# zdebruine/MMVAE

Measured on AMD Instinct MI355X. Metric: cells/sec per MMVAE train step, higher is better.
Workload: dtype f32; 1 GPU; c2: 2-modality MMVAE train step, 20000 genes each, latent 128, K=1, batch 512/GPU, adversarial=False; global_batch=512, parallelism=dp1, exchange=none

## Files before the change

include/mmvae_hip.h:

```cpp
#ifndef MMVAE_HIP_H
#define MMVAE_HIP_H

#include <stddef.h>
#include <stdint.h>

#ifdef __cplusplus
extern "C" {
#endif

typedef void* mmvae_stream_t;

#define MMVAE_OK 0
#define MMVAE_ERR_ARG 1
#define MMVAE_ERR_LAUNCH 2
#define MMVAE_ERR_WORKSPACE 3

#define MMVAE_ABI_VERSION 16
int mmvae_abi_version(void);
const char* mmvae_build_arch(void);

#define MMVAE_GEMM_NT 0
#define MMVAE_GEMM_NN 1
#define MMVAE_GEMM_TN 2

#define MMVAE_GEMM_RELU 1u
#define MMVAE_GEMM_ACCUMULATE 2u
#define MMVAE_GEMM_RAW_SLABS 4u
#define MMVAE_GEMM_OPERAND_SLACK 8u

#define MMVAE_GEMM_PRECISION_F32 0
#define MMVAE_GEMM_PRECISION_BF16X3 1
int mmvae_gemm_set_precision(int mode);
int mmvae_gemm_set_workgroup_cap(int max_workgroups);
int mmvae_gemm_set_x3w(int mode);
int mmvae_gemm_get_x3w(void);
int mmvae_gemm_get_precision(void);

int mmvae_gemm_plan(int layout, int M, int N, int K, int* tile_out, int* splitk_out);
size_t mmvae_gemm_workspace_bytes(int layout, int M, int N, int K, int splitk);

int mmvae_gemm_f32(int layout, int M, int N, int K, float alpha, const float* A, int64_t lda, const float* B,
                   int64_t ldb, float* C, int64_t ldc, const float* bias, unsigned flags, int splitk,
                   float* workspace, size_t workspace_bytes, mmvae_stream_t stream);

typedef struct mmvae_planes {
    uint16_t* p;
    int64_t ld, plane_stride;
} mmvae_planes;
#define MMVAE_RECON_H_KPAD 1u
typedef struct mmvae_recon_args {
    int32_t rows, x_rows, G, H;
    uint32_t flags, reserved;
    const float *h, *W, *bias, *x;
    int64_t ldh, ldw, ldx;
    float *xhat, *dP, *se_part, *col_part;
    int64_t ldxhat, lddp;
    mmvae_planes h_planes, W_planes, dP_planes;
} mmvae_recon_args;
int mmvae_recon_tiles(int G);
int mmvae_recon_row_tiles(int rows);
int mmvae_decoder_recon(const mmvae_recon_args* args, mmvae_stream_t stream);
size_t mmvae_sizeof_planes(void);
size_t mmvae_sizeof_recon_args(void);
size_t mmvae_sizeof_split_job(void);

typedef struct mmvae_bn_params {
    const float* gamma;
    const float* beta;
    float* running_mean;
    float* running_var;
    int64_t* num_batches_tracked;
    float momentum;
    float eps;
} mmvae_bn_params;

size_t mmvae_fc_workspace_bytes(int B, int N);

typedef struct mmvae_split_job {
    int32_t rows, cols;
    const float* src;
    int64_t ld_src;
    mmvae_planes planes;
} mmvae_split_job;

int mmvae_fc_epilogue_fwd(int B, int N, const float* in, int64_t ld_in, int n_slabs, const float* bias,
                          const mmvae_bn_params* bn , int training, int relu,
                          const uint8_t* keep_mask , float dropout_p, float* z_out,
                          float* a_out, float* d_out, int64_t ld_out, float* save_mean, float* save_invstd,
                          float* workspace, size_t workspace_bytes, const mmvae_planes* d_planes ,
                          const mmvae_split_job* split , mmvae_stream_t stream);

int mmvae_fc_epilogue_bwd(int B, int N, const float* din, int64_t ld_in, int n_slabs, const float* addend,
                          const float* addend_a, const float* row_scale, const uint8_t* keep_mask, float dropout_p, int relu,
                          const float* a, const float* z, const float* gamma, const float* save_mean,
                          const float* save_invstd, int has_bn, float* dz_out, int64_t ld_out, float* dbias,
                          float* dgamma, float* dbeta, float* workspace, size_t workspace_bytes,
                          const mmvae_planes* dz_planes , mmvae_stream_t stream);

int mmvae_layernorm_fwd(int B, int N, const float* x, int64_t ldx, float eps, float* y, int64_t ldy, float* save_mean,
                        float* save_invstd, mmvae_stream_t stream);
int mmvae_layernorm_bwd(int B, int N, const float* dy, int64_t lddy, const float* y, int64_t ldy,
                        const float* save_invstd, float* dx, int64_t lddx, mmvae_stream_t stream);

int mmvae_fc_rowtail_fwd(int B, int N, const float* in, int64_t ld_in, int n_slabs, const float* bias ,
                         float eps, int training, int relu, const uint8_t* keep_mask , float dropout_p,
                         float* y_out, float* a_out, float* d_out, int64_t ld_out, float* save_invstd,
                         mmvae_stream_t stream);

int mmvae_fc_rowtail_bwd(int B, int N, const float* din, int64_t ld_in, int n_slabs, const float* addend,
                         const float* row_scale, const uint8_t* keep_mask, float dropout_p, int relu, const float* act,
                         const float* y, const float* save_invstd, float* dz_out, int64_t ld_out, float* dbias,
                         float* workspace, size_t workspace_bytes, mmvae_stream_t stream);

int mmvae_reparam_kl_fwd(int B, int Z, int K, const float* mu, const float* a_raw, const float* eps, float var_eps,
                         float* std_out, float* z_out, float* kl_row, float* stat_row, mmvae_stream_t stream);

int mmvae_reparam_kl_bwd(int B, int Z, int K, const float* mu, const float* std, const float* eps, const float* dz,
                         const float* dmu_extra, const float* dstd_extra, const float* dkl_row,
                         const float* kl_scale_dev, float kl_scale_host, float var_eps, float* dmu, float* da_raw,
                         mmvae_stream_t stream);

int mmvae_mse_sum_fwd_bwd(int B, int G, const float* xhat, int64_t ldxhat, const float* x, int64_t ldx, float* se_row,
                          float* dxhat, int64_t lddx, const float* gscale_dev, float gscale_host,
                          mmvae_stream_t stream);

int mmvae_elbo_finalize(int B, int K, int T, const float* se_part, const float* kl_row, const float* stat_row, int Z,
                        const float* kl_weight_dev, float kl_weight_host, float* out6, float* w_out,
                        float* recon_row , mmvae_stream_t stream);

int mmvae_iwae_logratio(int B, int Z, int K, const float* std, const float* eps, const float* z, float* out,
                        mmvae_stream_t stream);
int mmvae_elbo_finalize_iwae(int B, int K, int T, const float* se_part, const float* logratio, const float* stat_row,
                             int Z, const float* kl_weight_dev, float kl_weight_host, float* out6, float* w_out,
                             float* rows3, mmvae_stream_t stream);
int mmvae_iwae_bwd_terms(int B, int Z, int K, const float* kl_weight_dev, float kl_weight_host, const float* w,
                         const float* z, const float* std, float* dz, float* dstd_extra, mmvae_stream_t stream);

int mmvae_cross_entropy_sum(int B, int C, const float* logits, int64_t ld, const int64_t* labels, float* loss_rows,
                            float* dlogits, int64_t ldd, const float* gscale_dev, float gscale_host,
                            mmvae_stream_t stream);
int mmvae_cross_entropy_heads(int B, int H, int max_classes, const int32_t* col_dev, const int32_t* classes_dev,
                              const float* logits, int64_t ld, const int64_t* labels, float* loss_rows, float* dlogits,
                              int64_t ldd, float gscale, mmvae_stream_t stream);
int mmvae_sum_f32(int64_t n, const float* v, float* out, int accumulate, mmvae_stream_t stream);
int mmvae_sum_rows_f32(int H, int64_t n, const float* v, int64_t ld, float* out_each, float* out_total,
                       mmvae_stream_t stream);

#define MMVAE_ADAM_STATE_FLOATS 8
#define MMVAE_PREPARE_NORM 1u
#define MMVAE_PREPARE_ADVANCE 2u
int64_t mmvae_sqnorm_partials(int64_t n);
int mmvae_grad_sqnorm(int64_t n, const float* grad, float* partials, mmvae_stream_t stream);
int mmvae_adam_prepare(int64_t n_partials, const float* partials, float max_norm, float grad_scale, float beta1,
                       float beta2, float* state, unsigned flags, mmvae_stream_t stream);
int mmvae_adam_set_workgroups(int workgroups);
int mmvae_adam_get_workgroups(void);
int mmvae_grad_sqnorm_ranges_prepare(int n_ranges, const float* const* grads, const int64_t* lens, float* partials,
                                     unsigned* ticket, int64_t n_partials_all, const float* partials_all, float max_norm,
                                     float grad_scale, float beta1, float beta2, float* state, unsigned flags,
                                     mmvae_stream_t stream);
#define MMVAE_ADAM_HYPER_FLOATS 4
int mmvae_adam_step_hp(int64_t n, float* param, const float* grad, float* exp_avg, float* exp_avg_sq, const float* state,
                       const float* hyper, float beta1, float beta2, float eps, float grad_scale, mmvae_stream_t stream);
int mmvae_adam_step_copy_hp(int64_t n, float* param, const float* grad, float* exp_avg, float* exp_avg_sq,
                            const float* state, const float* hyper, float beta1, float beta2, float eps, float grad_scale,
                            int copy_n, const float* copy_src, float* copy_dst, mmvae_stream_t stream);

#define MMVAE_ADAM_JOB_ELEMS 16384
typedef struct {
    int64_t offset;
    int32_t len;
    float bc1, bc2;
    int32_t reserved;
} mmvae_adam_job;
int mmvae_adam_step_jobs_hp(int n_jobs, const mmvae_adam_job* jobs_dev, float* param, const float* grad, float* exp_avg,
                            float* exp_avg_sq, const float* state, const float* hyper, float beta1, float beta2, float eps,
                            float grad_scale, mmvae_stream_t stream);
int mmvae_grad_sqnorm_jobs(int n_jobs, const mmvae_adam_job* jobs_dev, const float* grad, float* partials,
                           mmvae_stream_t stream);
int mmvae_grad_zero_flagged_jobs(int n_jobs, const mmvae_adam_job* jobs_dev, float* grad, mmvae_stream_t stream);
int mmvae_jobs_pack(int n_jobs, const mmvae_adam_job* jobs_dev, const float* arena, float* staging, mmvae_stream_t stream);
int mmvae_jobs_unpack(int n_jobs, const mmvae_adam_job* jobs_dev, float* arena, const float* staging, mmvae_stream_t stream);

int mmvae_philox_keep_mask(int64_t n, float p_drop, uint8_t* mask, uint64_t* rng_state, uint64_t stream_id,
                           int advance, mmvae_stream_t stream);
int mmvae_philox_normal(int64_t n, float* out, uint64_t* rng_state, uint64_t stream_id, int advance,
                        mmvae_stream_t stream);
typedef struct {
    void* out;
    int64_t n;
    uint64_t stream_id;
    float p_drop;
    int32_t kind;
} mmvae_philox_job;
int mmvae_philox_fill_jobs(int n_jobs, const mmvae_philox_job* jobs_dev, int64_t max_n, uint64_t* rng_state,
                           mmvae_stream_t stream);
int mmvae_philox_fill_jobs_advance(int n_jobs, const mmvae_philox_job* jobs_dev, int64_t max_n, uint64_t* rng_state,
                                   uint64_t advance_by, unsigned* ticket, mmvae_stream_t stream);
int mmvae_philox_advance(uint64_t* rng_state, uint64_t by, mmvae_stream_t stream);

typedef struct {
    const float* src;
    float* dst;
    int64_t part_stride, ld_src, ld_dst;
    int32_t n_parts, rows, cols;
    float alpha;
    uint32_t flags;
    uint32_t reserved;
} mmvae_sum_job;
int mmvae_sum_parts_batch(int n_jobs, const mmvae_sum_job* jobs, int64_t max_elems , mmvae_stream_t stream);

int mmvae_gemm_sq_partials(int layout, int M, int N, int K, int operands_regular);

int mmvae_split_planes_f32(int rows, int cols, const float* src, int64_t ld_src, uint16_t* planes,
                           int64_t ld, int64_t plane_stride, mmvae_stream_t stream);
int mmvae_gemm_planes_f32(int layout, int M, int N, int K, float alpha, const float* A, int64_t lda, const uint16_t* Ap,
                          int64_t ldap, int64_t a_plane_stride, const float* B, int64_t ldb, const uint16_t* Bp,
                          int64_t ldbp, int64_t b_plane_stride, float* C, int64_t ldc, const float* bias, unsigned flags,
                          int splitk, float* workspace, size_t workspace_bytes, float* sq_partials, int64_t sq_capacity,
                          mmvae_stream_t stream);
int mmvae_gemm_planes_supported(int layout, int M, int N, int K, int splitk, int a_planes, int b_planes);
typedef struct {
    const float* A;
    const float* B;
    float* C;
    const float* bias;
    int64_t lda, ldb, ldc;
    int32_t layout, M, N, K;
    float alpha;
    uint32_t flags;
    int32_t first_block;
    int32_t n_blocks;
} mmvae_gemm_job;
int mmvae_gemm_batch_job_ok(const mmvae_gemm_job* job);
int mmvae_gemm_batch_prepare(int n_jobs, mmvae_gemm_job* jobs, int* total_blocks);
int mmvae_gemm_batch_f32(int n_jobs, const mmvae_gemm_job* jobs_dev, int total_blocks, mmvae_stream_t stream);

int mmvae_csr_to_dense_f32(int B, int G, int64_t nnz, const int64_t* crow_indices, const int64_t* col_indices,
                           const float* values, float* out, int64_t ldo, mmvae_stream_t stream);
int mmvae_csr_to_dense_i32_f32(int B, int G, int64_t nnz, const int32_t* crow_indices, const int32_t* col_indices,
                               const float* values, float* out, int64_t ldo, mmvae_stream_t stream);

int mmvae_csr_gather_rows_i64(int B, int64_t n_src_rows, int64_t src_nnz, const int64_t* src_crow, const int64_t* src_col,
                              const float* src_val, const int64_t* rows, const int64_t* out_crow, int64_t out_nnz,
                              int64_t* out_col, float* out_val, mmvae_stream_t stream);
int mmvae_csr_gather_rows_i32(int B, int64_t n_src_rows, int64_t src_nnz, const int32_t* src_crow, const int32_t* src_col,
                              const float* src_val, const int64_t* rows, const int32_t* out_crow, int64_t out_nnz,
                              int32_t* out_col, float* out_val, mmvae_stream_t stream);
int mmvae_csr_gather_rows_dense_i64(int B, int G, int64_t n_src_rows, int64_t src_nnz, const int64_t* src_crow,
                                    const int64_t* src_col, const float* src_val, const int64_t* rows, float* out,
                                    int64_t ldo, mmvae_stream_t stream);
int mmvae_csr_gather_rows_dense_i32(int B, int G, int64_t n_src_rows, int64_t src_nnz, const int32_t* src_crow,
                                    const int32_t* src_col, const float* src_val, const int64_t* rows, float* out,
                                    int64_t ldo, mmvae_stream_t stream);

int mmvae_csr_spmm_wt_i32_f32(int B, int N, int G, int64_t nnz, const int32_t* crow_indices, const int32_t* col_indices,
                              const float* values, const float* Wt, int64_t ldwt, const float* bias, float* y,
                              int64_t ldy, mmvae_stream_t stream);

#define MMVAE_COND_DW_CHUNK 32
int mmvae_cond_linear_fwd(int B, int n_in, int n_out, const float* x, int64_t ldx, const float* params,
                          const int64_t* w_off, const int64_t* b_off, const int32_t* cond, const int32_t* rows, float* y,
                          int64_t ldy, mmvae_stream_t stream);
int mmvae_cond_linear_bwd_dx(int B, int n_in, int n_out, const float* dy, int64_t lddy, const float* params,
                             const int64_t* w_off, const int32_t* cond, const int32_t* rows, float* dx, int64_t lddx,
                             int accumulate, mmvae_stream_t stream);
int mmvae_cond_linear_bwd_dw(int n_chunks, const int32_t* chunk_dst, const int32_t* chunk_beg, const int32_t* chunk_end,
                             const int32_t* rows, int n_in, int n_out, const float* dy, int64_t lddy, const float* x,
                             int64_t ldx, float* grads, const int64_t* w_off, const int64_t* b_off, int n_red,
                             const int32_t* red_cond, const int32_t* red_slot, const int32_t* red_n, float* partials,
                             mmvae_stream_t stream);
int mmvae_cond_linear_fwd_multi(int n_pos, int B, int n_in, int n_out, const float* x, int64_t ldx, int64_t x_pos_stride,
                                const float* params, const int64_t* w_off, const int64_t* b_off, const int32_t* cond,
// ... 110 lines not shown
```

mmvae_amd/_lib.py:

```python
from __future__ import annotations

import ctypes as C
import os
from typing import Optional

_HERE = os.path.dirname(os.path.abspath(__file__))
LIB_PATH = os.path.join(_HERE, "csrc", "libmmvae_hip.so")
if os.environ.get("MMVAE_LIB"):
    LIB_PATH = os.environ["MMVAE_LIB"]

OK, ERR_ARG, ERR_LAUNCH, ERR_WORKSPACE = 0, 1, 2, 3
_ERR_NAMES = {1: "MMVAE_ERR_ARG", 2: "MMVAE_ERR_LAUNCH", 3: "MMVAE_ERR_WORKSPACE"}

GEMM_NT, GEMM_NN, GEMM_TN = 0, 1, 2
GEMM_RELU, GEMM_ACCUMULATE, GEMM_RAW_SLABS, GEMM_OPERAND_SLACK = 1, 2, 4, 8
GEMM_PRECISION_F32, GEMM_PRECISION_BF16X3 = 0, 1
ADAM_STATE_FLOATS = 8
ADAM_HYPER_FLOATS = 4
PREPARE_NORM, PREPARE_ADVANCE = 1, 2

_p = C.c_void_p
_i = C.c_int
_l = C.c_int64
_f = C.c_float
_u = C.c_uint
_z = C.c_size_t
_u64 = C.c_uint64


class BnParams(C.Structure):

    _fields_ = [
        ("gamma", _p),
        ("beta", _p),
        ("running_mean", _p),
        ("running_var", _p),
        ("num_batches_tracked", _p),
        ("momentum", _f),
        ("eps", _f),
    ]


class Planes(C.Structure):
    _fields_ = [("p", _p), ("ld", _l), ("plane_stride", _l)]


class ReconArgs(C.Structure):
    _fields_ = [("rows", C.c_int32), ("x_rows", C.c_int32), ("G", C.c_int32), ("H", C.c_int32), ("flags", C.c_uint32),
                ("reserved", C.c_uint32), ("h", _p), ("W", _p), ("bias", _p), ("x", _p), ("ldh", _l), ("ldw", _l),
                ("ldx", _l), ("xhat", _p), ("dP", _p), ("se_part", _p), ("col_part", _p), ("ldxhat", _l), ("lddp", _l),
                ("h_planes", Planes), ("W_planes", Planes), ("dP_planes", Planes)]


class SplitJob(C.Structure):
    _fields_ = [("rows", C.c_int32), ("cols", C.c_int32), ("src", _p), ("ld_src", _l), ("planes", Planes)]


RECON_H_KPAD = 1


PROTOTYPES = {
    "mmvae_abi_version": (_i, []),
    "mmvae_build_arch": (C.c_char_p, []),
    "mmvae_gemm_set_precision": (_i, [_i]),
    "mmvae_gemm_set_workgroup_cap": (_i, [_i]),
    "mmvae_adam_set_workgroups": (_i, [_i]),
    "mmvae_adam_get_workgroups": (_i, []),
    "mmvae_gemm_set_x3w": (_i, [_i]),
    "mmvae_gemm_get_x3w": (_i, []),
    "mmvae_gemm_get_precision": (_i, []),
    "mmvae_gemm_plan": (_i, [_i, _i, _i, _i, C.POINTER(_i), C.POINTER(_i)]),
    "mmvae_gemm_workspace_bytes": (_z, [_i, _i, _i, _i, _i]),
    "mmvae_gemm_f32": (_i, [_i, _i, _i, _i, _f, _p, _l, _p, _l, _p, _l, _p, _u, _i, _p, _z, _p]),
    "mmvae_recon_tiles": (_i, [_i]),
    "mmvae_recon_row_tiles": (_i, [_i]),
    "mmvae_decoder_recon": (_i, [C.POINTER(ReconArgs), _p]),
    "mmvae_sizeof_planes": (_z, []),
    "mmvae_sizeof_recon_args": (_z, []),
    "mmvae_sizeof_split_job": (_z, []),
    "mmvae_fc_workspace_bytes": (_z, [_i, _i]),
    "mmvae_fc_epilogue_fwd": (
        _i,
        [_i, _i, _p, _l, _i, _p, C.POINTER(BnParams), _i, _i, _p, _f, _p, _p, _p, _l, _p, _p, _p, _z,
         C.POINTER(Planes), C.POINTER(SplitJob), _p],
    ),
    "mmvae_fc_epilogue_bwd": (
        _i,
        [_i, _i, _p, _l, _i, _p, _p, _p, _p, _f, _i, _p, _p, _p, _p, _p, _i, _p, _l, _p, _p, _p, _p, _z,
         C.POINTER(Planes), _p],
    ),
    "mmvae_layernorm_fwd": (_i, [_i, _i, _p, _l, _f, _p, _l, _p, _p, _p]),
    "mmvae_layernorm_bwd": (_i, [_i, _i, _p, _l, _p, _l, _p, _p, _l, _p]),
    "mmvae_fc_rowtail_fwd": (_i, [_i, _i, _p, _l, _i, _p, _f, _i, _i, _p, _f, _p, _p, _p, _l, _p, _p]),
    "mmvae_fc_rowtail_bwd": (_i, [_i, _i, _p, _l, _i, _p, _p, _p, _f, _i, _p, _p, _p, _p, _l, _p, _p, _z, _p]),
    "mmvae_reparam_kl_fwd": (_i, [_i, _i, _i, _p, _p, _p, _f, _p, _p, _p, _p, _p]),
    "mmvae_reparam_kl_bwd": (_i, [_i, _i, _i, _p, _p, _p, _p, _p, _p, _p, _p, _f, _f, _p, _p, _p]),
    "mmvae_mse_sum_fwd_bwd": (_i, [_i, _i, _p, _l, _p, _l, _p, _p, _l, _p, _f, _p]),
    "mmvae_elbo_finalize": (_i, [_i, _i, _i, _p, _p, _p, _i, _p, _f, _p, _p, _p, _p]),
    "mmvae_iwae_logratio": (_i, [_i, _i, _i, _p, _p, _p, _p, _p]),
    "mmvae_elbo_finalize_iwae": (_i, [_i, _i, _i, _p, _p, _p, _i, _p, _f, _p, _p, _p, _p]),
    "mmvae_iwae_bwd_terms": (_i, [_i, _i, _i, _p, _f, _p, _p, _p, _p, _p, _p]),
    "mmvae_cross_entropy_sum": (_i, [_i, _i, _p, _l, _p, _p, _p, _l, _p, _f, _p]),
    "mmvae_cross_entropy_heads": (_i, [_i, _i, _i, _p, _p, _p, _l, _p, _p, _p, _l, _f, _p]),
    "mmvae_sum_f32": (_i, [_l, _p, _p, _i, _p]),
    "mmvae_debug_occupy": (_i, [_i, _i, _i, _p, _p]),
    "mmvae_sum_rows_f32": (_i, [_i, _l, _p, _l, _p, _p, _p]),
    "mmvae_sqnorm_partials": (_l, [_l]),
    "mmvae_grad_sqnorm": (_i, [_l, _p, _p, _p]),
    "mmvae_adam_prepare": (_i, [_l, _p, _f, _f, _f, _f, _p, _u, _p]),
    "mmvae_grad_sqnorm_ranges_prepare": (_i, [_i, _p, _p, _p, _p, _l, _p, _f, _f, _f, _f, _p, _u, _p]),
    "mmvae_adam_step_hp": (_i, [_l, _p, _p, _p, _p, _p, _p, _f, _f, _f, _f, _p]),
    "mmvae_adam_step_copy_hp": (_i, [_l, _p, _p, _p, _p, _p, _p, _f, _f, _f, _f, _i, _p, _p, _p]),
    "mmvae_adam_step_jobs_hp": (_i, [_i, _p, _p, _p, _p, _p, _p, _p, _f, _f, _f, _f, _p]),
    "mmvae_grad_sqnorm_jobs": (_i, [_i, _p, _p, _p, _p]),
    "mmvae_grad_zero_flagged_jobs": (_i, [_i, _p, _p, _p]),
    "mmvae_jobs_pack": (_i, [_i, _p, _p, _p, _p]),
    "mmvae_jobs_unpack": (_i, [_i, _p, _p, _p, _p]),
    "mmvae_philox_keep_mask": (_i, [_l, _f, _p, _p, _u64, _i, _p]),
    "mmvae_philox_normal": (_i, [_l, _p, _p, _u64, _i, _p]),
    "mmvae_philox_advance": (_i, [_p, _u64, _p]),
    "mmvae_philox_fill_jobs": (_i, [_i, _p, _l, _p, _p]),
    "mmvae_philox_fill_jobs_advance": (_i, [_i, _p, _l, _p, C.c_uint64, _p, _p]),
    "mmvae_axpby": (_i, [_l, _f, _p, _f, _p, _p]),
    "mmvae_upload_words": (_i, [_l, _p, _p, _p]),
    "mmvae_scale_rows": (_i, [_i, _i, _p, _l, _p, _p, _l, _p]),
    "mmvae_debug_stamp": (_i, [_p, _i, _p]),
    "mmvae_weighted_colsum_chunks": (_i, [_i]),
    "mmvae_weighted_colsum_f32": (_i, [_i, _i, _p, _l, _p, _p, _p]),
    "mmvae_sum_parts_batch": (_i, [_i, _p, _l, _p]),
    "mmvae_gemm_sq_partials": (_i, [_i, _i, _i, _i, _i]),
    "mmvae_split_planes_f32": (_i, [_i, _i, _p, _l, _p, _l, _l, _p]),
    "mmvae_gemm_planes_f32": (
        _i,
        [_i, _i, _i, _i, _f, _p, _l, _p, _l, _l, _p, _l, _p, _l, _l, _p, _l, _p, _u, _i, _p, _z, _p, _l, _p],
    ),
    "mmvae_gemm_planes_supported": (_i, [_i, _i, _i, _i, _i, _i, _i]),
    "mmvae_csr_to_dense_f32": (_i, [_i, _i, _l, _p, _p, _p, _p, _l, _p]),
    "mmvae_csr_to_dense_i32_f32": (_i, [_i, _i, _l, _p, _p, _p, _p, _l, _p]),
    "mmvae_csr_gather_rows_i64": (_i, [_i, _l, _l, _p, _p, _p, _p, _p, _l, _p, _p, _p]),
    "mmvae_csr_gather_rows_i32": (_i, [_i, _l, _l, _p, _p, _p, _p, _p, _l, _p, _p, _p]),
    "mmvae_csr_gather_rows_dense_i64": (_i, [_i, _i, _l, _l, _p, _p, _p, _p, _p, _l, _p]),
    "mmvae_csr_gather_rows_dense_i32": (_i, [_i, _i, _l, _l, _p, _p, _p, _p, _p, _l, _p]),
    "mmvae_csr_spmm_wt_i32_f32": (_i, [_i, _i, _i, _l, _p, _p, _p, _p, _l, _p, _p, _l, _p]),
    "mmvae_cond_linear_fwd": (_i, [_i, _i, _i, _p, _l, _p, _p, _p, _p, _p, _p, _l, _p]),
    "mmvae_cond_linear_bwd_dx": (_i, [_i, _i, _i, _p, _l, _p, _p, _p, _p, _p, _l, _i, _p]),
    "mmvae_cond_linear_bwd_dw": (_i, [_i, _p, _p, _p, _p, _i, _i, _p, _l, _p, _l, _p, _p, _p, _i, _p, _p, _p, _p, _p]),
    "mmvae_cond_linear_fwd_multi": (_i, [_i, _i, _i, _i, _p, _l, _l, _p, _p, _p, _p, _p, _l, _p, _l, _l, _p]),
    "mmvae_cond_linear_bwd_dx_multi": (_i, [_i, _i, _i, _i, _p, _l, _l, _p, _p, _p, _l, _p, _l, _i, _p]),
    "mmvae_cond_linear_bwd_dw_multi": (_i, [_i, _i, _p, _p, _p, _p, _l, _i, _i, _p, _l, _l, _p, _l, _l, _p, _p, _p, _i, _p,
                                            _p, _p, _p, _l, _p]),
    "mmvae_gemm_batch_job_ok": (_i, [_p]),
    "mmvae_gemm_batch_prepare": (_i, [_i, _p, C.POINTER(_i)]),
    "mmvae_gemm_batch_f32": (_i, [_i, _p, _i, _p]),
    "mmvae_adv_pass_plan": (_i, [_p, _i, C.POINTER(_i), C.POINTER(_z), C.POINTER(_l), C.POINTER(_i)]),
    "mmvae_adv_pass_f32": (_i, [_i, _p, _i, _i, _i, _i, _z, _p]),
    "mmvae_adv_dw_prepare": (_i, [_i, _p, C.POINTER(_i), C.POINTER(_i)]),
    "mmvae_adv_dw_f32": (_i, [_i, _p, _i, _i, _p, _p, _p, _i, _p, _i, _p]),
    "mmvae_adam_step_multi_hp": (_i, [_i, _p, _l, _p]),
    "mmvae_ell_from_dense_f32": (_i, [_i, _i, _p, _l, _i, _p, _p, _p, _p]),
    "mmvae_dw_sparse_ell_f32": (_i, [_i, _i, _i, _p, _l, _p, _p, _p, _i, _p, _l, _p]),
    "mmvae_col_pearson_workspace_bytes": (_z, [_i, _i]),
    "mmvae_col_pearson_f32": (_i, [_i, _i, _p, _l, _p, _l, _p, _p, _z, _p]),
}


class SumJob(C.Structure):
    _fields_ = [("src", C.c_void_p), ("dst", C.c_void_p), ("part_stride", C.c_int64), ("ld_src", C.c_int64),
                ("ld_dst", C.c_int64), ("n_parts", C.c_int32), ("rows", C.c_int32), ("cols", C.c_int32),
                ("alpha", C.c_float), ("flags", C.c_uint32), ("reserved", C.c_uint32)]


class PhiloxJob(C.Structure):
    _fields_ = [("out", C.c_void_p), ("n", C.c_int64), ("stream_id", C.c_uint64), ("p_drop", C.c_float),
                ("kind", C.c_int32)]


class GemmJob(C.Structure):
    _fields_ = [("A", C.c_void_p), ("B", C.c_void_p), ("C", C.c_void_p), ("bias", C.c_void_p), ("lda", C.c_int64),
                ("ldb", C.c_int64), ("ldc", C.c_int64), ("layout", C.c_int32), ("M", C.c_int32), ("N", C.c_int32),
                ("K", C.c_int32), ("alpha", C.c_float), ("flags", C.c_uint32), ("first_block", C.c_int32),
                ("n_blocks", C.c_int32)]


ADV_MAX_LAYERS, ADV_MAX_HEADS = 4, 8


class AdvJob(C.Structure):
    _fields_ = [("x", _p), ("ldx", _l), ("W", _p * ADV_MAX_LAYERS), ("b", _p * ADV_MAX_LAYERS),
                ("mask", _p * ADV_MAX_LAYERS), ("act", _p * ADV_MAX_LAYERS), ("dz", _p * ADV_MAX_LAYERS), ("Wh", _p),
                ("bh", _p), ("labels", _p), ("logits", _p), ("lse", _p), ("loss_rows", _p), ("gx", _p), ("partials", _p),
                ("loss_each", _p), ("loss_total", _p), ("total_loss", _p), ("total_scale", _f),
                ("gscale", _f), ("p_drop", _f * ADV_MAX_LAYERS), ("relu", C.c_int32 * ADV_MAX_LAYERS),
                ("width", C.c_int32 * (ADV_MAX_LAYERS + 1)), ("n_layers", C.c_int32), ("H", C.c_int32),
                ("Ct", C.c_int32), ("B", C.c_int32), ("col", C.c_int32 * ADV_MAX_HEADS),
                ("classes", C.c_int32 * ADV_MAX_HEADS), ("seg_lo", (C.c_int16 * ADV_MAX_HEADS) * 8),
                ("seg_hi", (C.c_int16 * ADV_MAX_HEADS) * 8)]


class AdvDwJob(C.Structure):
    _fields_ = [("dz", _p), ("ld_dz", _l), ("inp", _p), ("ld_inp", _l), ("gW", _p), ("gb", _p), ("lse", _p),
                ("labels", _p), ("gscale", _f), ("M", C.c_int32), ("N", C.c_int32), ("B", C.c_int32), ("H", C.c_int32),
                ("opt", C.c_int32), ("col", C.c_int32 * ADV_MAX_HEADS), ("classes", C.c_int32 * ADV_MAX_HEADS),
                ("first_block", C.c_int32), ("n_blocks", C.c_int32)]


class AdvOpt(C.Structure):
    _fields_ = [("state", _p), ("norm_out", _p), ("max_norm", _f), ("grad_scale", _f), ("beta1", _f), ("beta2", _f),
                ("flags", C.c_uint32), ("reserved", C.c_uint32)]


class AdamArenaHp(C.Structure):
    _fields_ = [("p", _p), ("g", _p), ("m", _p), ("v", _p), ("state", _p), ("hyper", _p), ("n", _l), ("beta1", _f),
                ("beta2", _f), ("eps", _f), ("grad_scale", _f)]


class HipLibraryError(RuntimeError):
    pass


_lib: Optional[C.CDLL] = None


def load() -> C.CDLL:
    global _lib
    if _lib is not None:
        return _lib
    import torch

    if not os.path.exists(LIB_PATH):
        raise HipLibraryError(
            f"{LIB_PATH} not found: build it with `make -C mmvae_amd/csrc` (or __graft_entry__.build()). "
            "mmvae_amd has no non-HIP execution path for device tensors."
        )
    try:
        lib = C.CDLL(LIB_PATH)
    except OSError as e:
        raise HipLibraryError(f"could not load {LIB_PATH}: {e}") from e
    for name, (res, args) in PROTOTYPES.items():
        try:
            fn = getattr(lib, name)
        except AttributeError as e:
            raise HipLibraryError(f"{LIB_PATH} does not export {name}") from e
        fn.restype = res
        fn.argtypes = args
    _lib = lib
    return lib


def check(rc: int, what: str) -> None:
# ... 3 lines not shown
```

mmvae_amd/csrc/elbo_optim.hip:

```cpp
#include "common.h"

namespace {

__global__ __launch_bounds__(256) void reparam_kl_fwd_kernel(int B, int Z, int K, const float* __restrict__ mu,
                                                             const float* __restrict__ a_raw,
                                                             const float* __restrict__ eps, float var_eps,
                                                             float* __restrict__ std_out, float* __restrict__ z_out,
                                                             float* __restrict__ kl_row, float* __restrict__ stat_row) {
    const int lane = threadIdx.x & 63;
    const int b = blockIdx.x * 4 + (threadIdx.x >> 6);
    if (b >= B) return;
    float kl = 0.f, smu = 0.f, svar = 0.f;
    for (int j = lane; j < Z; j += 64) {
        const int64_t o = (int64_t)b * Z + j;
        const float m = mu[o];
        const float v = expf(a_raw[o]) + var_eps;
        const float s = sqrtf(v);
        if (std_out) std_out[o] = s;
        const float vr = s * s;
        kl += 0.5f * (vr + m * m - 1.f - logf(vr));
        smu += m;
        svar += vr;
        if (z_out)
            for (int k = 0; k < K; ++k) {
                const int64_t ok = ((int64_t)k * B + b) * Z + j;
                z_out[ok] = m + s * eps[ok];
            }
    }
    kl = wave_sum(kl);
    smu = wave_sum(smu);
    svar = wave_sum(svar);
    if (lane == 0) {
        if (kl_row) kl_row[b] = kl;
        if (stat_row) {
            stat_row[b] = smu;
            stat_row[B + b] = svar;
        }
    }
}

__global__ __launch_bounds__(256) void reparam_kl_bwd_kernel(int B, int Z, int K, const float* __restrict__ mu,
                                                             const float* __restrict__ sd,
                                                             const float* __restrict__ eps, const float* __restrict__ dz,
                                                             const float* __restrict__ dmu_extra,
                                                             const float* __restrict__ dstd_extra,
                                                             const float* __restrict__ dkl_row,
                                                             const float* __restrict__ kl_scale_dev, float kl_scale_host,
                                                             float var_eps, float* __restrict__ dmu,
                                                             float* __restrict__ da_raw) {
    const int64_t n = (int64_t)B * Z;
    const float cs = (kl_scale_dev ? *kl_scale_dev : 1.f) * kl_scale_host;
    for (int64_t o = (int64_t)blockIdx.x * blockDim.x + threadIdx.x; o < n; o += (int64_t)gridDim.x * blockDim.x) {
        const int b = (int)(o / Z);
        const float c = cs * (dkl_row ? dkl_row[b] : 1.f);
        const float m = mu[o], s = sd[o];
        const float v = s * s;
        float gm = dmu_extra ? dmu_extra[o] : 0.f;
        float gs = dstd_extra ? dstd_extra[o] : 0.f;
        if (dz)
            for (int k = 0; k < K; ++k) {
                const int64_t ok = (int64_t)k * n + o;
                const float g = dz[ok];
                gm += g;
                gs += g * eps[ok];
            }
        dmu[o] = gm + c * m;
        da_raw[o] = (gs / (2.f * s) + c * 0.5f * (1.f - 1.f / v)) * (v - var_eps);
    }
}

__global__ __launch_bounds__(256) void mse_rows_kernel(int B, int G, const float* __restrict__ xhat, int64_t ldxhat,
                                                       const float* __restrict__ x, int64_t ldx,
                                                       float* __restrict__ se_row, float* __restrict__ dxhat,
                                                       int64_t lddx, const float* __restrict__ gscale_dev,
                                                       float gscale_host) {
    __shared__ float red[4];
    const int b = blockIdx.x;
    const float gs = 2.f * gscale_host * (gscale_dev ? *gscale_dev : 1.f);
    const float* xh = xhat + (int64_t)b * ldxhat;
    const float* xr = x + (int64_t)b * ldx;
    float* dr = dxhat ? dxhat + (int64_t)b * lddx : nullptr;
    float s = 0.f;
    for (int j = threadIdx.x; j < G; j += 256) {
        const float d = xh[j] - xr[j];
        s += d * d;
        if (dr) dr[j] = gs * d;
    }
    s = wave_sum(s);
    if ((threadIdx.x & 63) == 0) red[threadIdx.x >> 6] = s;
    __syncthreads();
    if (threadIdx.x == 0 && se_row) se_row[b] = (red[0] + red[1]) + (red[2] + red[3]);
}

constexpr int ELBO_MAXK = 64;
__global__ __launch_bounds__(256) void elbo_rows_kernel(int B, int K, int T, const float* __restrict__ se_part,
                                                        float* __restrict__ recon_row, float* __restrict__ w_out) {
    __shared__ float se_s[4][ELBO_MAXK];
    const int lane = threadIdx.x & 63, wv = threadIdx.x >> 6;
    const int b = blockIdx.x * 4 + wv;
    if (b >= B) return;
    const int64_t KB = (int64_t)K * B;
    if (K == 1) {
        float s = 0.f;
        for (int t = lane; t < T; t += 64) s += se_part[(int64_t)t * KB + b];
        s = wave_sum(s);
        if (lane == 0) {
            recon_row[b] = s;
            if (w_out) w_out[b] = 1.f;
        }
        return;
    }
    for (int k = 0; k < K; ++k) {
        float s = 0.f;
        for (int t = lane; t < T; t += 64) s += se_part[(int64_t)t * KB + (int64_t)k * B + b];
        s = wave_sum(s);
        if (lane == 0) se_s[wv][k] = s;
    }
    __builtin_amdgcn_wave_barrier();
    float v = (lane < K) ? -se_s[wv][lane] : -INFINITY;
    const float mx = wave_max(v);
    const float ex = (lane < K) ? expf(v - mx) : 0.f;
    const float sum = wave_sum(ex);
    const float lse = mx + logf(sum);
    if (lane == 0) recon_row[b] = -(lse - logf((float)K));
    if (w_out && lane < K) w_out[(int64_t)lane * B + b] = ex / sum;
}

__global__ __launch_bounds__(256) void iwae_logratio_kernel(int B, int Z, int K, const float* __restrict__ std,
                                                            const float* __restrict__ eps, const float* __restrict__ z,
                                                            float* __restrict__ out) {
    const int lane = threadIdx.x & 63, row = blockIdx.x * 4 + (threadIdx.x >> 6);
    if (row >= K * B) return;
    const int b = row % B;
    const float* sr = std + (int64_t)b * Z;
    const float* er = eps + (int64_t)row * Z;
    const float* zr = z + (int64_t)row * Z;
    float s = 0.f;
    for (int j = lane; j < Z; j += 64) s += -logf(sr[j]) - 0.5f * er[j] * er[j] + 0.5f * zr[j] * zr[j];
    s = wave_sum(s);
    if (lane == 0) out[row] = s;
}

__global__ __launch_bounds__(256) void elbo_rows_iwae_kernel(int B, int K, int T, const float* __restrict__ se_part,
                                                             const float* __restrict__ logratio,
                                                             const float* __restrict__ klw_dev, float c_host,
                                                             float* __restrict__ rows3, float* __restrict__ w_out) {
    __shared__ float se_s[4][ELBO_MAXK];
    const int lane = threadIdx.x & 63, wv = threadIdx.x >> 6;
    const int b = blockIdx.x * 4 + wv;
    if (b >= B) return;
    const int64_t KB = (int64_t)K * B;
    const float c = (klw_dev ? *klw_dev : 1.f) * c_host;
    for (int k = 0; k < K; ++k) {
        float s = 0.f;
        for (int t = lane; t < T; t += 64) s += se_part[(int64_t)t * KB + (int64_t)k * B + b];
        s = wave_sum(s);
        if (lane == 0) se_s[wv][k] = s;
    }
    __builtin_amdgcn_wave_barrier();
    const float se = (lane < K) ? se_s[wv][lane] : 0.f;
    const float r = (lane < K) ? logratio[(int64_t)lane * B + b] : 0.f;
    const float v = (lane < K) ? -se - c * r : -INFINITY;
    const float mx = wave_max(v);
    const float ex = (lane < K) ? expf(v - mx) : 0.f;
    const float sum = wave_sum(ex);
    const float lse = mx + logf(sum);
    const float w = ex / sum;
    const float wse = wave_sum(w * se), wr = wave_sum(w * r);
    if (lane == 0) {
        rows3[b] = -(lse - logf((float)K));
        rows3[B + b] = wse;
        rows3[2 * (int64_t)B + b] = wr;
    }
    if (w_out && lane < K) w_out[(int64_t)lane * B + b] = w;
}

__global__ __launch_bounds__(256) void elbo_reduce_iwae_kernel(int B, const float* __restrict__ rows3,
                                                               const float* __restrict__ stat_row, int Z,
                                                               const float* __restrict__ klw_dev, float klw_host,
                                                               float* __restrict__ out6) {
    __shared__ double red[5][256];
    const int tid = threadIdx.x;
    double a0 = 0.0, a1 = 0.0, a2 = 0.0, smu = 0.0, svar = 0.0;
    for (int b = tid; b < B; b += 256) {
        a0 += (double)rows3[b];
        a1 += (double)rows3[B + b];
        a2 += (double)rows3[2 * (int64_t)B + b];
        if (stat_row) {
            smu += (double)stat_row[b];
            svar += (double)stat_row[B + b];
        }
    }
    red[0][tid] = a0;
    red[1][tid] = a1;
    red[2][tid] = a2;
    red[3][tid] = smu;
    red[4][tid] = svar;
    __syncthreads();
    if (tid == 0) {
        double t[5] = {0, 0, 0, 0, 0};
        for (int i = 0; i < 256; ++i)
            for (int q = 0; q < 5; ++q) t[q] += red[q][i];
// ... 426 lines not shown
                   nullptr, nullptr);
}

inline int grid_for(int64_t n, int per_block, int cap);
constexpr int STREAM_GRID_CAP = 1 << 22;
static int g_adam_workgroups = 0;

extern "C" int mmvae_adam_set_workgroups(int workgroups) {
    if (workgroups < 0 || workgroups > 256) return MMVAE_ERR_ARG;
    g_adam_workgroups = workgroups;
    return MMVAE_OK;
}

extern "C" int mmvae_adam_get_workgroups(void) { return g_adam_workgroups; }

static int launch_adam_step(int64_t n, float* param, const float* grad, float* exp_avg, float* exp_avg_sq,
                            const float* state, const float* hyper, float beta1, float beta2, float eps,
                            float grad_scale, int copy_n, const float* copy_src, float* copy_dst, hipStream_t stream) {
    const int vec = aligned16(param) && aligned16(grad) && aligned16(exp_avg) && aligned16(exp_avg_sq);
    if (g_adam_workgroups > 0) {
        static bool attr = false;
        if (!attr) {
            if (hipFuncSetAttribute(reinterpret_cast<const void*>(adam_step_wide_hp_kernel),
                                    hipFuncAttributeMaxDynamicSharedMemorySize, ADAM_WIDE_LDS) != hipSuccess)
                return MMVAE_ERR_LAUNCH;
            attr = true;
        }
        MMVAE_LAUNCH(adam_step_wide_hp_kernel, dim3(g_adam_workgroups), dim3(1024), (size_t)ADAM_WIDE_LDS, stream, n, param,
                     grad, exp_avg, exp_avg_sq, state, hyper, beta1, beta2, eps, grad_scale, vec, copy_n, copy_src,
                     copy_dst);
    } else {
        MMVAE_LAUNCH(adam_step_hp_kernel, dim3(grid_for(n, 1024, STREAM_GRID_CAP)), dim3(256), 0, stream, n, param, grad,
                     exp_avg, exp_avg_sq, state, hyper, beta1, beta2, eps, grad_scale, vec, copy_n, copy_src, copy_dst);
    }
    MMVAE_LAUNCH_CHECK();
    return MMVAE_OK;
}

__device__ __forceinline__ void adam_step_jobs_body(const mmvae_adam_job* __restrict__ jobs, float* __restrict__ p,
                                                    const float* __restrict__ g, float* __restrict__ m,
                                                    float* __restrict__ v, const float* __restrict__ state,
                                                    const float* __restrict__ hyper, float b1, float b2, float eps,
                                                    float grad_scale) {
    const mmvae_adam_job job = jobs[blockIdx.x];
    if ((job.reserved & 3) == 2) return;
    float lr, wd, decay;
    adam_hyper(hyper, lr, wd, decay);
    const float gmul = state[2] * grad_scale;
    const float step_size = lr / job.bc1;
    const float inv_bc2_sqrt = 1.f / sqrtf(job.bc2);
    const float cv = state[5];
    const int64_t o = job.offset;
    const int n = job.len;
    if ((o & 3) == 0) {
        const int nv = n >> 2;
        f32x4* pv = reinterpret_cast<f32x4*>(p + o);
        const f32x4* gv = reinterpret_cast<const f32x4*>(g + o);
        f32x4* mv = reinterpret_cast<f32x4*>(m + o);
        f32x4* vv = reinterpret_cast<f32x4*>(v + o);
        for (int i = threadIdx.x; i < nv; i += 256) {
            f32x4 pp = pv[i], gg = gv[i], mm = mv[i], vw = vv[i];
#pragma unroll
            for (int e = 0; e < 4; ++e) {
                float pe = pp[e], me = mm[e], ve = vw[e];
                adam_elem(pe, gg[e], me, ve, gmul, wd, decay, b1, b2, step_size, inv_bc2_sqrt, eps, cv);
                pp[e] = pe;
                mm[e] = me;
                vw[e] = ve;
            }
            pv[i] = pp;
            mv[i] = mm;
            vv[i] = vw;
        }
        for (int i = 4 * nv + threadIdx.x; i < n; i += 256)
            adam_elem(p[o + i], g[o + i], m[o + i], v[o + i], gmul, wd, decay, b1, b2, step_size, inv_bc2_sqrt, eps, cv);
    } else {
        for (int i = threadIdx.x; i < n; i += 256)
            adam_elem(p[o + i], g[o + i], m[o + i], v[o + i], gmul, wd, decay, b1, b2, step_size, inv_bc2_sqrt, eps, cv);
    }
}

__global__ __launch_bounds__(256) void adam_step_jobs_hp_kernel(const mmvae_adam_job* __restrict__ jobs,
                                                                float* __restrict__ p, const float* __restrict__ g,
                                                                float* __restrict__ m, float* __restrict__ v,
                                                                const float* __restrict__ state,
                                                                const float* __restrict__ hyper, float b1, float b2,
                                                                float eps, float grad_scale) {
    adam_step_jobs_body(jobs, p, g, m, v, state, hyper, b1, b2, eps, grad_scale);
}

__global__ __launch_bounds__(256) void sqnorm_jobs_kernel(const mmvae_adam_job* __restrict__ jobs,
                                                          const float* __restrict__ g, float* __restrict__ partials) {
    __shared__ float red[4];
    const mmvae_adam_job job = jobs[blockIdx.x];
    const int64_t o = job.offset;
    const int n = (job.reserved & 3) == 2 ? 0 : job.len;
    float s = 0.f;
    if ((o & 3) == 0) {
        const int nv = n >> 2;
        const f32x4* gv = reinterpret_cast<const f32x4*>(g + o);
        float s0 = 0.f, s1 = 0.f, s2 = 0.f, s3 = 0.f;
        for (int i = threadIdx.x; i < nv; i += 256) {
            const f32x4 v = gv[i];
            s0 += v.x * v.x;
            s1 += v.y * v.y;
            s2 += v.z * v.z;
            s3 += v.w * v.w;
        }
        s = (s0 + s1) + (s2 + s3);
        for (int i = 4 * nv + threadIdx.x; i < n; i += 256) s += g[o + i] * g[o + i];
    } else {
        for (int i = threadIdx.x; i < n; i += 256) s += g[o + i] * g[o + i];
    }
    s = wave_sum(s);
    if ((threadIdx.x & 63) == 0) red[threadIdx.x >> 6] = s;
    __syncthreads();
    if (threadIdx.x == 0) partials[blockIdx.x] = (red[0] + red[1]) + (red[2] + red[3]);
}

__global__ __launch_bounds__(256) void zero_flagged_jobs_kernel(const mmvae_adam_job* __restrict__ jobs,
                                                                float* __restrict__ g) {
    const mmvae_adam_job job = jobs[blockIdx.x];
    if ((job.reserved & 3) != 1 && (job.reserved & 3) != 2) return;
    for (int i = threadIdx.x; i < job.len; i += 256) g[job.offset + i] = 0.f;
}

template <bool PACK>
__global__ __launch_bounds__(256) void jobs_pack_kernel(const mmvae_adam_job* __restrict__ jobs, float* __restrict__ arena,
                                                        float* __restrict__ staging) {
    const mmvae_adam_job job = jobs[blockIdx.x];
    float* a = arena + job.offset;
    float* s = staging + (int64_t)((unsigned)job.reserved >> 2) * 128;
    const int n = job.len, padded = (n + 127) & ~127;
    for (int i = threadIdx.x; i < n; i += 256) {
        if (PACK)
            s[i] = a[i];
        else
            a[i] = s[i];
    }
    if (PACK)
        for (int i = n + threadIdx.x; i < padded; i += 256) s[i] = 0.f;
}

__global__ __launch_bounds__(256) void occupy_kernel(long long ticks, float* __restrict__ sink) {
    extern __shared__ float hold[];
    hold[threadIdx.x] = (float)threadIdx.x;
    __syncthreads();
    const long long t0 = wall_clock64();
    float acc = hold[(threadIdx.x + 1) & 255];
    while (wall_clock64() - t0 < ticks) acc = acc * 1.0000001f + 1e-7f;
    if (acc == -1.f && sink) sink[0] = acc;
}

struct u32x4 {
    uint32_t x, y, z, w;
};
__device__ __forceinline__ u32x4 philox4x32_10(uint64_t counter, uint64_t stream_id, uint64_t seed) {
    uint32_t c0 = (uint32_t)counter, c1 = (uint32_t)(counter >> 32), c2 = (uint32_t)stream_id,
             c3 = (uint32_t)(stream_id >> 32);
    uint32_t k0 = (uint32_t)seed, k1 = (uint32_t)(seed >> 32);
#pragma unroll
    for (int i = 0; i < 10; ++i) {
        const uint64_t p0 = (uint64_t)0xD2511F53u * c0;
        const uint64_t p1 = (uint64_t)0xCD9E8D57u * c2;
        const uint32_t n0 = (uint32_t)(p1 >> 32) ^ c1 ^ k0;
        const uint32_t n1 = (uint32_t)p1;
        const uint32_t n2 = (uint32_t)(p0 >> 32) ^ c3 ^ k1;
        const uint32_t n3 = (uint32_t)p0;
        c0 = n0;
        c1 = n1;
        c2 = n2;
        c3 = n3;
        k0 += 0x9E3779B9u;
        k1 += 0xBB67AE85u;
    }
    return {c0, c1, c2, c3};
}
__device__ __forceinline__ float u01(uint32_t x) { return ((float)(x >> 8) + 0.5f) * (1.0f / 16777216.0f); }

__global__ __launch_bounds__(256) void philox_mask_kernel(int64_t n, float p_drop, uint8_t* __restrict__ mask,
                                                          const uint64_t* __restrict__ rng, uint64_t stream_id) {
    const uint64_t seed = rng[0], off = rng[1];
    const int64_t nq = (n + 3) / 4;
    for (int64_t q = (int64_t)blockIdx.x * blockDim.x + threadIdx.x; q < nq; q += (int64_t)gridDim.x * blockDim.x) {
        const u32x4 r = philox4x32_10(off + (uint64_t)q, stream_id, seed);
        const uint32_t rv[4] = {r.x, r.y, r.z, r.w};
#pragma unroll
        for (int j = 0; j < 4; ++j) {
            const int64_t i = q * 4 + j;
            if (i < n) mask[i] = (u01(rv[j]) >= p_drop) ? 1 : 0;
        }
    }
}

__global__ __launch_bounds__(256) void philox_normal_kernel(int64_t n, float* __restrict__ out,
                                                            const uint64_t* __restrict__ rng, uint64_t stream_id) {
    const uint64_t seed = rng[0], off = rng[1];
    const int64_t nq = (n + 3) / 4;
    for (int64_t q = (int64_t)blockIdx.x * blockDim.x + threadIdx.x; q < nq; q += (int64_t)gridDim.x * blockDim.x) {
        const u32x4 r = philox4x32_10(off + (uint64_t)q, stream_id, seed);
        const float u0 = u01(r.x), u1 = u01(r.y), u2 = u01(r.z), u3 = u01(r.w);
        const float r0 = sqrtf(-2.f * logf(u0)), r1 = sqrtf(-2.f * logf(u2));
        float s0, c0, s1, c1;
        sincosf(6.283185307179586f * u1, &s0, &c0);
        sincosf(6.283185307179586f * u3, &s1, &c1);
        const float nv[4] = {r0 * c0, r0 * s0, r1 * c1, r1 * s1};
#pragma unroll
        for (int j = 0; j < 4; ++j) {
            const int64_t i = q * 4 + j;
            if (i < n) out[i] = nv[j];
        }
    }
}

__global__ void philox_advance_kernel(uint64_t* rng, uint64_t by) { rng[1] += by; }

__global__ __launch_bounds__(256) void philox_fill_jobs_kernel(const mmvae_philox_job* __restrict__ jobs, uint64_t* rng,
                                                               uint64_t advance_by, unsigned* ticket) {
    const mmvae_philox_job job = jobs[blockIdx.y];
    const uint64_t seed = rng[0], off = rng[1];
    const int64_t n = job.n, nq = (n + 3) / 4;
    for (int64_t q = (int64_t)blockIdx.x * blockDim.x + threadIdx.x; q < nq; q += (int64_t)gridDim.x * blockDim.x) {
        const u32x4 r = philox4x32_10(off + (uint64_t)q, job.stream_id, seed);
        if (job.kind == 0) {
            uint8_t* mask = static_cast<uint8_t*>(job.out);
            const uint32_t rv[4] = {r.x, r.y, r.z, r.w};
#pragma unroll
            for (int j = 0; j < 4; ++j) {
                const int64_t i = q * 4 + j;
                if (i < n) mask[i] = (u01(rv[j]) >= job.p_drop) ? 1 : 0;
            }
        } else {
            float* out = static_cast<float*>(job.out);
            const float u0 = u01(r.x), u1 = u01(r.y), u2 = u01(r.z), u3 = u01(r.w);
            const float r0 = sqrtf(-2.f * logf(u0)), r1 = sqrtf(-2.f * logf(u2));
            float s0, c0, s1, c1;
            sincosf(6.283185307179586f * u1, &s0, &c0);
            sincosf(6.283185307179586f * u3, &s1, &c1);
            const float nv[4] = {r0 * c0, r0 * s0, r1 * c1, r1 * s1};
#pragma unroll
            for (int j = 0; j < 4; ++j) {
                const int64_t i = q * 4 + j;
                if (i < n) out[i] = nv[j];
            }
        }
    }
    if (advance_by && ticket) {
        __syncthreads();
        if (threadIdx.x == 0 && atomicAdd(ticket, 1u) == gridDim.x * gridDim.y - 1) {
            *ticket = 0u;
            rng[1] = off + advance_by;
        }
    }
}

__global__ __launch_bounds__(256) void axpby_kernel(int64_t n, float alpha, const float* __restrict__ x, float beta,
                                                    float* __restrict__ y) {
    for (int64_t i = (int64_t)blockIdx.x * blockDim.x + threadIdx.x; i < n; i += (int64_t)gridDim.x * blockDim.x)
        y[i] = alpha * x[i] + (beta != 0.f ? beta * y[i] : 0.f);
}

__global__ __launch_bounds__(256) void axpby4_kernel(int64_t n4, float alpha, const float4* __restrict__ x, float beta,
                                                     float4* __restrict__ y) {
    for (int64_t i = (int64_t)blockIdx.x * blockDim.x + threadIdx.x; i < n4; i += (int64_t)gridDim.x * blockDim.x) {
        const float4 a = x[i];
        float4 r = make_float4(alpha * a.x, alpha * a.y, alpha * a.z, alpha * a.w);
        if (beta != 0.f) {
            const float4 b = y[i];
            r.x += beta * b.x, r.y += beta * b.y, r.z += beta * b.z, r.w += beta * b.w;
        }
        y[i] = r;
    }
}

__global__ __launch_bounds__(256) void sum_parts_batch_kernel(const mmvae_sum_job* __restrict__ jobs) {
    const mmvae_sum_job j = jobs[blockIdx.y];
    const bool acc = j.flags & MMVAE_GEMM_ACCUMULATE;
    const bool vec = j.cols % 4 == 0;
    if (vec) {
        const int c4n = j.cols / 4;
        const int64_t total = (int64_t)j.rows * c4n;
        for (int64_t i = (int64_t)blockIdx.x * blockDim.x + threadIdx.x; i < total; i += (int64_t)gridDim.x * blockDim.x) {
            const int r = (int)(i / c4n), c = (int)(i - (int64_t)r * c4n) * 4;
            const float* sp = j.src + (int64_t)r * j.ld_src + c;
            f32x4 s = {0.f, 0.f, 0.f, 0.f};
            int p = 0;
            for (; p + 8 <= j.n_parts; p += 8) {
                f32x4 t[8];
#pragma unroll
                for (int u = 0; u < 8; ++u) t[u] = *reinterpret_cast<const f32x4*>(sp + (int64_t)(p + u) * j.part_stride);
#pragma unroll
                for (int u = 0; u < 8; ++u) s += t[u];
            }
            for (; p < j.n_parts; ++p) s += *reinterpret_cast<const f32x4*>(sp + (int64_t)p * j.part_stride);
            f32x4 v = s * j.alpha;
            float* dp = j.dst + (int64_t)r * j.ld_dst + c;
            if (acc) v += *reinterpret_cast<const f32x4*>(dp);
            *reinterpret_cast<f32x4*>(dp) = v;
        }
    } else {
        const int64_t total = (int64_t)j.rows * j.cols;
        for (int64_t i = (int64_t)blockIdx.x * blockDim.x + threadIdx.x; i < total; i += (int64_t)gridDim.x * blockDim.x) {
            const int r = (int)(i / j.cols), c = (int)(i - (int64_t)r * j.cols);
            const float* sp = j.src + (int64_t)r * j.ld_src + c;
            float s = 0.f;
            for (int p = 0; p < j.n_parts; ++p) s += sp[(int64_t)p * j.part_stride];
            float v = s * j.alpha;
            float* dp = j.dst + (int64_t)r * j.ld_dst + c;
            if (acc) v += *dp;
            *dp = v;
        }
    }
}

__global__ __launch_bounds__(256) void scale_rows_kernel(int B, int N, const float* __restrict__ x, int64_t ldx,
                                                         const float* __restrict__ rs, float* __restrict__ y,
                                                         int64_t ldy) {
    const int64_t total = (int64_t)B * N;
    for (int64_t i = (int64_t)blockIdx.x * blockDim.x + threadIdx.x; i < total; i += (int64_t)gridDim.x * blockDim.x) {
        const int b = (int)(i / N), j = (int)(i - (int64_t)b * N);
        y[(int64_t)b * ldy + j] = x[(int64_t)b * ldx + j] * rs[b];
    }
}

inline int grid_for(int64_t n, int per_block, int cap) {
    int64_t b = (n + per_block - 1) / per_block;
    if (b < 1) b = 1;
    if (b > cap) b = cap;
    return (int)b;
}

}

extern "C" int mmvae_abi_version(void) { return MMVAE_ABI_VERSION; }
extern "C" const char* mmvae_build_arch(void) { return "gfx950"; }

extern "C" int mmvae_reparam_kl_fwd(int B, int Z, int K, const float* mu, const float* a_raw, const float* eps,
                                    float var_eps, float* std_out, float* z_out, float* kl_row, float* stat_row,
                                    mmvae_stream_t stream) {
    if (B <= 0 || Z <= 0 || K < 1 || !mu || !a_raw) return MMVAE_ERR_ARG;
    if (z_out && !eps) return MMVAE_ERR_ARG;
    MMVAE_LAUNCH(reparam_kl_fwd_kernel, dim3(ceil_div_i(B, 4)), dim3(256), 0, (hipStream_t)stream, B, Z, K, mu,
                       a_raw, eps, var_eps, std_out, z_out, kl_row, stat_row);
    MMVAE_LAUNCH_CHECK();
    return MMVAE_OK;
}

extern "C" int mmvae_reparam_kl_bwd(int B, int Z, int K, const float* mu, const float* sd, const float* eps,
                                    const float* dz, const float* dmu_extra, const float* dstd_extra,
                                    const float* dkl_row, const float* kl_scale_dev, float kl_scale_host, float var_eps,
                                    float* dmu, float* da_raw, mmvae_stream_t stream) {
    if (B <= 0 || Z <= 0 || K < 1 || !mu || !sd || !dmu || !da_raw) return MMVAE_ERR_ARG;
    if (dz && !eps) return MMVAE_ERR_ARG;
    const int64_t n = (int64_t)B * Z;
    MMVAE_LAUNCH(reparam_kl_bwd_kernel, dim3(grid_for(n, 256, 2048)), dim3(256), 0, (hipStream_t)stream, B, Z, K,
                       mu, sd, eps, dz, dmu_extra, dstd_extra, dkl_row, kl_scale_dev, kl_scale_host, var_eps, dmu,
                       da_raw);
    MMVAE_LAUNCH_CHECK();
    return MMVAE_OK;
}

extern "C" int mmvae_mse_sum_fwd_bwd(int B, int G, const float* xhat, int64_t ldxhat, const float* x, int64_t ldx,
                                     float* se_row, float* dxhat, int64_t lddx, const float* gscale_dev,
                                     float gscale_host, mmvae_stream_t stream) {
    if (B <= 0 || G <= 0 || !xhat || !x || ldxhat < G || ldx < G) return MMVAE_ERR_ARG;
    if (!se_row && !dxhat) return MMVAE_ERR_ARG;
    if (dxhat && lddx < G) return MMVAE_ERR_ARG;
    MMVAE_LAUNCH(mse_rows_kernel, dim3(B), dim3(256), 0, (hipStream_t)stream, B, G, xhat, ldxhat, x, ldx, se_row,
                       dxhat, lddx, gscale_dev, gscale_host);
    MMVAE_LAUNCH_CHECK();
    return MMVAE_OK;
}

extern "C" int mmvae_elbo_finalize(int B, int K, int T, const float* se_part, const float* kl_row,
                                   const float* stat_row, int Z, const float* kl_weight_dev, float kl_weight_host,
                                   float* out6, float* w_out, float* recon_row, mmvae_stream_t stream) {
    if (B <= 0 || K < 1 || K > ELBO_MAXK || T < 1 || !se_part || !out6 || !recon_row) return MMVAE_ERR_ARG;
    MMVAE_LAUNCH(elbo_rows_kernel, dim3(ceil_div_i(B, 4)), dim3(256), 0, (hipStream_t)stream, B, K, T, se_part,
                       recon_row, w_out);
    MMVAE_LAUNCH_CHECK();
    MMVAE_LAUNCH(elbo_reduce_kernel, dim3(1), dim3(256), 0, (hipStream_t)stream, B, recon_row, kl_row, stat_row, Z,
                       kl_weight_dev, kl_weight_host, out6);
    MMVAE_LAUNCH_CHECK();
    return MMVAE_OK;
}

extern "C" int mmvae_iwae_logratio(int B, int Z, int K, const float* std, const float* eps, const float* z, float* out,
                                   mmvae_stream_t stream) {
    if (B <= 0 || Z <= 0 || K < 1 || K > ELBO_MAXK || !std || !eps || !z || !out) return MMVAE_ERR_ARG;
    MMVAE_LAUNCH(iwae_logratio_kernel, dim3(ceil_div_i(K * B, 4)), dim3(256), 0, (hipStream_t)stream, B, Z, K, std, eps, z,
                 out);
    MMVAE_LAUNCH_CHECK();
    return MMVAE_OK;
}

extern "C" int mmvae_elbo_finalize_iwae(int B, int K, int T, const float* se_part, const float* logratio,
                                        const float* stat_row, int Z, const float* kl_weight_dev, float kl_weight_host,
                                        float* out6, float* w_out, float* rows3, mmvae_stream_t stream) {
    if (B <= 0 || K < 1 || K > ELBO_MAXK || T < 1 || !se_part || !logratio || !out6 || !rows3) return MMVAE_ERR_ARG;
    MMVAE_LAUNCH(elbo_rows_iwae_kernel, dim3(ceil_div_i(B, 4)), dim3(256), 0, (hipStream_t)stream, B, K, T, se_part,
                 logratio, kl_weight_dev, kl_weight_host / (float)B, rows3, w_out);
    MMVAE_LAUNCH_CHECK();
    MMVAE_LAUNCH(elbo_reduce_iwae_kernel, dim3(1), dim3(256), 0, (hipStream_t)stream, B, rows3, stat_row, Z,
                 kl_weight_dev, kl_weight_host, out6);
    MMVAE_LAUNCH_CHECK();
    return MMVAE_OK;
}

extern "C" int mmvae_iwae_bwd_terms(int B, int Z, int K, const float* kl_weight_dev, float kl_weight_host, const float* w,
                                    const float* z, const float* std, float* dz, float* dstd_extra,
                                    mmvae_stream_t stream) {
    if (B <= 0 || Z <= 0 || K < 1 || !w || !z || !std || !dz || !dstd_extra) return MMVAE_ERR_ARG;
    MMVAE_LAUNCH(iwae_bwd_terms_kernel, dim3(grid_for((int64_t)K * B * Z, 256, 2048)), dim3(256), 0, (hipStream_t)stream,
                 B, Z, K, kl_weight_dev, kl_weight_host / (float)B, w, z, std, dz, dstd_extra);
    MMVAE_LAUNCH_CHECK();
    return MMVAE_OK;
}

extern "C" int mmvae_cross_entropy_sum(int B, int C, const float* logits, int64_t ld, const int64_t* labels,
                                       float* loss_rows, float* dlogits, int64_t ldd, const float* gscale_dev,
                                       float gscale_host, mmvae_stream_t stream) {
    if (B <= 0 || C <= 0 || !logits || !labels || ld < C) return MMVAE_ERR_ARG;
    if (!loss_rows && !dlogits) return MMVAE_ERR_ARG;
    if (dlogits && ldd < C) return MMVAE_ERR_ARG;
    if (C >= 1024 && C <= 256 * 4 * 8)
        MMVAE_LAUNCH(ce_rows_block_kernel<8>, dim3(B), dim3(256), 0, (hipStream_t)stream, B, C, logits, ld, labels,
                     loss_rows, dlogits, ldd, gscale_dev, gscale_host);
    else
        MMVAE_LAUNCH(ce_rows_kernel, dim3(ceil_div_i(B, 4)), dim3(256), 0, (hipStream_t)stream, B, C, logits, ld,
                     labels, loss_rows, dlogits, ldd, gscale_dev, gscale_host);
    MMVAE_LAUNCH_CHECK();
    return MMVAE_OK;
}

extern "C" int mmvae_cross_entropy_heads(int B, int H, int max_classes, const int32_t* col_dev, const int32_t* classes_dev,
                                         const float* logits, int64_t ld, const int64_t* labels, float* loss_rows,
                                         float* dlogits, int64_t ldd, float gscale, mmvae_stream_t stream) {
    if (B <= 0 || H <= 0 || H > 65535 || max_classes <= 0 || max_classes > 256 * 4 * 8 || !col_dev || !classes_dev ||
        !logits || !labels || (!loss_rows && !dlogits))
        return MMVAE_ERR_ARG;
    MMVAE_LAUNCH(ce_heads_kernel<8>, dim3(B, H), dim3(256), 0, (hipStream_t)stream, B, col_dev, classes_dev, logits, ld,
                 labels, loss_rows, dlogits, ldd, gscale);
    MMVAE_LAUNCH_CHECK();
    return MMVAE_OK;
}

__global__ void debug_stamp_kernel(long long* __restrict__ buf, int slot) { buf[slot] = wall_clock64(); }
extern "C" int mmvae_debug_stamp(long long* buf, int slot, mmvae_stream_t stream) {
    if (!buf || slot < 0) return MMVAE_ERR_ARG;
    MMVAE_LAUNCH(debug_stamp_kernel, dim3(1), dim3(1), 0, (hipStream_t)stream, buf, slot);
    MMVAE_LAUNCH_CHECK();
    return MMVAE_OK;
}

extern "C" int mmvae_debug_occupy(int workgroups, int lds_bytes, int micros, float* sink, mmvae_stream_t stream) {
    if (workgroups <= 0 || workgroups > 256 || lds_bytes < 1024 || lds_bytes > 160 * 1024 || micros <= 0 ||
        micros > 20000)
        return MMVAE_ERR_ARG;
    if (lds_bytes > 64 * 1024 &&
        hipFuncSetAttribute(reinterpret_cast<const void*>(occupy_kernel), hipFuncAttributeMaxDynamicSharedMemorySize,
                            lds_bytes) != hipSuccess)
        return MMVAE_ERR_LAUNCH;
    MMVAE_LAUNCH(occupy_kernel, dim3(workgroups), dim3(256), (size_t)lds_bytes, (hipStream_t)stream,
                 (long long)micros * 100, sink);
    MMVAE_LAUNCH_CHECK();
    return MMVAE_OK;
}

extern "C" int mmvae_sum_f32(int64_t n, const float* v, float* out, int accumulate, mmvae_stream_t stream) {
    if (n < 0 || (n > 0 && !v) || !out) return MMVAE_ERR_ARG;
    MMVAE_LAUNCH(sum_kernel, dim3(1), dim3(1024), 0, (hipStream_t)stream, n, v, out, accumulate);
    MMVAE_LAUNCH_CHECK();
    return MMVAE_OK;
}

extern "C" int mmvae_sum_rows_f32(int H, int64_t n, const float* v, int64_t ld, float* out_each, float* out_total,
                                  mmvae_stream_t stream) {
    if (H <= 0 || n < 0 || (n > 0 && !v) || ld < n || (!out_each && !out_total)) return MMVAE_ERR_ARG;
    MMVAE_LAUNCH(sum_rows_kernel, dim3(1), dim3(1024), 0, (hipStream_t)stream, H, n, v, ld, out_each, out_total);
    MMVAE_LAUNCH_CHECK();
    return MMVAE_OK;
}

extern "C" int64_t mmvae_sqnorm_partials(int64_t n) { return n > 0 ? ceil_div_l(n, SQN_CHUNK) : 0; }

extern "C" int mmvae_grad_sqnorm(int64_t n, const float* grad, float* partials, mmvae_stream_t stream) {
    if (n <= 0 || !grad || !partials) return MMVAE_ERR_ARG;
    MMVAE_LAUNCH(sqnorm_kernel, dim3((unsigned)mmvae_sqnorm_partials(n)), dim3(256), 0, (hipStream_t)stream, n,
                       grad, partials);
    MMVAE_LAUNCH_CHECK();
    return MMVAE_OK;
}

extern "C" int mmvae_adam_prepare(int64_t n_partials, const float* partials, float max_norm, float grad_scale,
                                  float beta1, float beta2, float* state, unsigned flags, mmvae_stream_t stream) {
    if (n_partials < 0 || !state) return MMVAE_ERR_ARG;
    if ((flags & MMVAE_PREPARE_NORM) && n_partials > 0 && !partials) return MMVAE_ERR_ARG;
    MMVAE_LAUNCH(adam_prepare_kernel, dim3(1), dim3(256), 0, (hipStream_t)stream, n_partials, partials, max_norm,
                       grad_scale, beta1, beta2, state, flags);
    MMVAE_LAUNCH_CHECK();
    return MMVAE_OK;
}

extern "C" int mmvae_grad_sqnorm_ranges_prepare(int n_ranges, const float* const* grads, const int64_t* lens,
                                                float* partials, unsigned* ticket, int64_t n_partials_all,
                                                const float* partials_all, float max_norm, float grad_scale,
                                                float beta1, float beta2, float* state, unsigned flags,
                                                mmvae_stream_t stream) {
    if (n_ranges < 1 || n_ranges > 4 || !grads || !lens || !partials || !ticket || !partials_all || !state ||
        n_partials_all <= 0)
// ... 482 lines not shown
```

mmvae_amd/csrc/fc_epilogue.hip:

```cpp
#include "common.h"

namespace {

constexpr int CW = 64;
constexpr int RPC = 32;
constexpr int RPW = 8;
constexpr int CT = 256;

struct FwdArgs {
    const float* in;
    int64_t ld_in, slab_stride;
    int n_slabs;
    const float* bias;
    const float* gamma;
    const float* beta;
    float* running_mean;
    float* running_var;
    int64_t* nbt;
    float momentum, eps;
    int training, relu;
    const uint8_t* mask;
    float keep_scale;
    float* z_out;
    float* a_out;
    float* d_out;
    int64_t ld_out;
    float* save_mean;
    float* save_invstd;
    float* ws;
    int B, N, RC;
    unsigned short* d_planes;
    int64_t ldp, pstride;
    const float* sp_src;
    unsigned short* sp_planes;
    int64_t sp_ld_src, sp_ld, sp_pstride;
    int sp_rows, sp_groups, sp_cols;
};

__device__ __forceinline__ void split_rows_job(const FwdArgs& a, int wg, int nwg) {
    const int64_t total = (int64_t)a.sp_rows * a.sp_groups;
    for (int64_t idx = (int64_t)wg * CT + threadIdx.x; idx < total; idx += (int64_t)nwg * CT) {
        const int row = (int)(idx / a.sp_groups), gq = (int)(idx - (int64_t)row * a.sp_groups);
        const float* sp = a.sp_src + (int64_t)row * a.sp_ld_src + 8 * gq;
        f32x4 v0, v1;
        if (8 * gq + 8 <= a.sp_cols) {
            v0 = *reinterpret_cast<const f32x4*>(sp);
            v1 = *reinterpret_cast<const f32x4*>(sp + 4);
        } else {
            const int left = a.sp_cols - 8 * gq;
#pragma unroll
            for (int j = 0; j < 4; ++j) {
                v0[j] = j < left ? sp[j] : 0.f;
                v1[j] = 4 + j < left ? sp[4 + j] : 0.f;
            }
        }
        unsigned q[8][3];
#pragma unroll
        for (int j = 0; j < 4; ++j) {
            x3_split(v0[j], q[j][0], q[j][1], q[j][2]);
            x3_split(v1[j], q[4 + j][0], q[4 + j][1], q[4 + j][2]);
        }
        unsigned short* dp = a.sp_planes + (int64_t)row * a.sp_ld + 8 * gq;
#pragma unroll
        for (int p = 0; p < 3; ++p)
            *reinterpret_cast<uint4*>(dp + p * a.sp_pstride) =
                make_uint4((q[0][p] >> 16) | (q[1][p] & 0xFFFF0000u), (q[2][p] >> 16) | (q[3][p] & 0xFFFF0000u),
                           (q[4][p] >> 16) | (q[5][p] & 0xFFFF0000u), (q[6][p] >> 16) | (q[7][p] & 0xFFFF0000u));
    }
}

__device__ __forceinline__ float block_colsum(float v, float (*red)[CW], int w, int lane) {
    __syncthreads();
    red[w][lane] = v;
    __syncthreads();
    return (red[0][lane] + red[1][lane]) + (red[2][lane] + red[3][lane]);
}

__device__ __forceinline__ void slab_sum_rows(float (&acc)[RPW], const float* __restrict__ in, int64_t ld,
                                              int64_t slab_stride, int n_slabs, int r0, int B, int c) {
    const float* p[RPW];
#pragma unroll
    for (int i = 0; i < RPW; ++i) p[i] = in + (int64_t)min(r0 + i, B - 1) * ld + c;
    int s = 0;
    for (; s + 4 <= n_slabs; s += 4) {
        float t[4][RPW];
#pragma unroll
        for (int u = 0; u < 4; ++u)
#pragma unroll
            for (int i = 0; i < RPW; ++i) t[u][i] = p[i][(int64_t)(s + u) * slab_stride];
#pragma unroll
        for (int u = 0; u < 4; ++u)
#pragma unroll
            for (int i = 0; i < RPW; ++i) acc[i] += t[u][i];
    }
    for (; s < n_slabs; ++s) {
        float t[RPW];
#pragma unroll
        for (int i = 0; i < RPW; ++i) t[i] = p[i][(int64_t)s * slab_stride];
#pragma unroll
        for (int i = 0; i < RPW; ++i) acc[i] += t[i];
    }
}

__global__ __launch_bounds__(CT) void fc_fwd_stats_kernel(const FwdArgs a) {
    __shared__ float red[4][CW];
    const int lane = threadIdx.x & 63, w = threadIdx.x >> 6;
    const int c = blockIdx.x * CW + lane;
    const int chunk = blockIdx.y;
    const bool cv = c < a.N;
    const float bias = (cv && a.bias) ? a.bias[c] : 0.f;
    const int r0 = chunk * RPC + w * RPW;
    float zv[RPW];
    float s = 0.f;
#pragma unroll
    for (int i = 0; i < RPW; ++i) zv[i] = bias;
    slab_sum_rows(zv, a.in, a.ld_in, a.slab_stride, a.n_slabs, r0, a.B, cv ? c : a.N - 1);
#pragma unroll
    for (int i = 0; i < RPW; ++i) {
        const int r = r0 + i;
        if (cv && r < a.B) {
            a.z_out[(int64_t)r * a.ld_out + c] = zv[i];
            s += zv[i];
        } else {
            zv[i] = 0.f;
        }
    }
    const int nb = min(RPC, a.B - chunk * RPC);
    const float mean = block_colsum(s, red, w, lane) / (float)nb;
    float m2 = 0.f;
#pragma unroll
    for (int i = 0; i < RPW; ++i)
        if (r0 + i < a.B) {
            const float d = zv[i] - mean;
            m2 += d * d;
        }
    m2 = block_colsum(m2, red, w, lane);
    if (w == 0 && cv) {
        a.ws[(int64_t)chunk * a.N + c] = mean;
        a.ws[(int64_t)(a.RC + chunk) * a.N + c] = m2;
    }
}

template <bool HAS_BN>
__global__ __launch_bounds__(CT) void fc_fwd_apply_kernel(const FwdArgs a) {
    if ((int)blockIdx.y >= a.RC) {
        split_rows_job(a, ((int)blockIdx.y - a.RC) * gridDim.x + blockIdx.x, ((int)gridDim.y - a.RC) * gridDim.x);
        return;
    }
    const int lane = threadIdx.x & 63, w = threadIdx.x >> 6;
    const int c = blockIdx.x * CW + lane;
    const int chunk = blockIdx.y;
    if (c >= a.N) return;
    const float bias = a.bias ? a.bias[c] : 0.f;
    float mean = 0.f, invstd = 1.f, gam = 1.f, bet = 0.f;
    const bool stats = HAS_BN && a.training;
    const int r0 = chunk * RPC + w * RPW;
    float zs[RPW];
    unsigned char mk[RPW];
    if (stats || a.mask) {
#pragma unroll
        for (int i = 0; i < RPW; ++i) {
            const int rc = min(r0 + i, a.B - 1);
            if (stats) zs[i] = a.z_out[(int64_t)rc * a.ld_out + c];
            mk[i] = a.mask ? a.mask[(int64_t)rc * a.N + c] : (unsigned char)1;
        }
    }
    if (HAS_BN) {
        gam = a.gamma ? a.gamma[c] : 1.f;
        bet = a.beta ? a.beta[c] : 0.f;
        if (stats) {
            float n = 0.f, M2 = 0.f;
            for (int ch0 = 0; ch0 < a.RC; ch0 += 8) {
                float mb[8], m2b[8];
#pragma unroll
                for (int u = 0; u < 8; ++u) {
                    const int ch = min(ch0 + u, a.RC - 1);
                    mb[u] = a.ws[(int64_t)ch * a.N + c];
                    m2b[u] = a.ws[(int64_t)(a.RC + ch) * a.N + c];
                }
#pragma unroll
                for (int u = 0; u < 8; ++u) {
                    const int ch = ch0 + u;
                    if (ch < a.RC) {
                        const float nb = (float)min(RPC, a.B - ch * RPC);
                        const float delta = mb[u] - mean;
                        const float nn = n + nb;
                        mean += delta * (nb / nn);
                        M2 += m2b[u] + delta * delta * (n * nb / nn);
                        n = nn;
                    }
                }
            }
            const float var = M2 / (float)a.B;
            invstd = 1.0f / sqrtf(var + a.eps);
            if (chunk == 0 && w == 0) {
                if (a.save_mean) a.save_mean[c] = mean;
                if (a.save_invstd) a.save_invstd[c] = invstd;
                if (a.running_mean) a.running_mean[c] = (1.f - a.momentum) * a.running_mean[c] + a.momentum * mean;
                if (a.running_var) {
                    const float unb = a.B > 1 ? var * ((float)a.B / (float)(a.B - 1)) : var;
                    a.running_var[c] = (1.f - a.momentum) * a.running_var[c] + a.momentum * unb;
                }
                if (blockIdx.x == 0 && lane == 0 && a.nbt) *a.nbt += 1;
            }
        } else {
            mean = a.running_mean[c];
            invstd = 1.0f / sqrtf(a.running_var[c] + a.eps);
        }
    }
    if (!stats) {
#pragma unroll
        for (int i = 0; i < RPW; ++i) zs[i] = bias;
        slab_sum_rows(zs, a.in, a.ld_in, a.slab_stride, a.n_slabs, r0, a.B, c);
    }
#pragma unroll
    for (int i = 0; i < RPW; ++i) {
        const int r = r0 + i;
        if (r >= a.B) break;
        const int64_t o = (int64_t)r * a.ld_out + c;
        const float z = zs[i];
        if (!stats && a.z_out) a.z_out[o] = z;
        float y = z;
        if (HAS_BN) y = (z - mean) * invstd * gam + bet;
        if (a.relu) y = fmaxf(y, 0.f);
        if (a.a_out) a.a_out[o] = y;
        if (a.d_out) {
            float d = y;
            if (a.mask) d = mk[i] ? y * a.keep_scale : 0.f;
            a.d_out[o] = d;
            if (a.d_planes) store_planes_lanepair(a.d_planes, a.ldp, a.pstride, r, c, d, lane);
        }
    }
}

struct BwdArgs {
    const float* din;
    int64_t ld_in, slab_stride;
    int n_slabs;
    const float* addend;
    const float* addend_a;
    const float* row_scale;
    const uint8_t* mask;
    float keep_scale;
    int relu;
    const float* a;
    const float* z;
    const float* gamma;
    const float* save_mean;
    const float* save_invstd;
    float* dz_out;
    int64_t ld_out;
    float* dbias;
    float* dgamma;
    float* dbeta;
    float* ws;
    int B, N, RC;
    unsigned short* dz_planes;
    int64_t ldp, pstride;
};

struct BwdRowOps {
    float addend[RPW], row_scale[RPW], addend_a[RPW], act[RPW], z[RPW];
    unsigned char mask[RPW];
};
template <bool HAS_BN>
__device__ __forceinline__ void bwd_load_rows(const BwdArgs& a, int r0, int c, BwdRowOps& o) {
#pragma unroll
    for (int i = 0; i < RPW; ++i) {
        const int r = min(r0 + i, a.B - 1);
        const int64_t oo = (int64_t)r * a.ld_out + c;
        o.addend[i] = a.addend ? a.addend[oo] : 0.f;
        o.row_scale[i] = a.row_scale ? a.row_scale[r] : 1.f;
        o.mask[i] = a.mask ? a.mask[(int64_t)r * a.N + c] : (unsigned char)1;
        o.addend_a[i] = a.addend_a ? a.addend_a[oo] : 0.f;
        o.act[i] = a.relu ? a.a[oo] : 1.f;
        o.z[i] = HAS_BN ? a.z[oo] : 0.f;
    }
}
__device__ __forceinline__ float bwd_dy(const BwdArgs& a, const BwdRowOps& o, int i, float g) {
    if (a.addend) g += o.addend[i];
    if (a.row_scale) g *= o.row_scale[i];
    if (a.mask) g = o.mask[i] ? g * a.keep_scale : 0.f;
    if (a.addend_a) g += o.addend_a[i];
    if (a.relu) g = (o.act[i] > 0.f) ? g : 0.f;
    return g;
}

template <bool HAS_BN>
__global__ __launch_bounds__(CT) void fc_bwd_stats_kernel(const BwdArgs a) {
    __shared__ float red[4][CW];
    const int lane = threadIdx.x & 63, w = threadIdx.x >> 6;
    const int c = blockIdx.x * CW + lane;
    const int chunk = blockIdx.y;
    const bool cv = c < a.N;
    float mean = 0.f, invstd = 1.f;
    if (HAS_BN && cv) {
        mean = a.save_mean[c];
        invstd = a.save_invstd[c];
    }
    const int r0 = chunk * RPC + w * RPW;
    float s1 = 0.f, s2 = 0.f, s3 = 0.f;
    float gs[RPW];
#pragma unroll
    for (int i = 0; i < RPW; ++i) gs[i] = 0.f;
    BwdRowOps ops;
    bwd_load_rows<HAS_BN>(a, r0, cv ? c : a.N - 1, ops);
    slab_sum_rows(gs, a.din, a.ld_in, a.slab_stride, a.n_slabs, r0, a.B, cv ? c : a.N - 1);
#pragma unroll
    for (int i = 0; i < RPW; ++i) {
        const int r = r0 + i;
        if (cv && r < a.B) {
            const float dy = bwd_dy(a, ops, i, gs[i]);
            const int64_t oo = (int64_t)r * a.ld_out + c;
            if (a.dz_out) a.dz_out[oo] = dy;
            if (!HAS_BN && a.dz_planes) store_planes_lanepair(a.dz_planes, a.ldp, a.pstride, r, c, dy, lane);
            s1 += dy;
            if (HAS_BN) {
                const float xh = (ops.z[i] - mean) * invstd;
                s2 += dy * xh;
                s3 += xh;
            }
        }
    }
    if (!a.ws) return;
    s1 = block_colsum(s1, red, w, lane);
    if (HAS_BN) {
        s2 = block_colsum(s2, red, w, lane);
        s3 = block_colsum(s3, red, w, lane);
    }
    if (w == 0 && cv) {
        a.ws[(int64_t)chunk * a.N + c] = s1;
        if (HAS_BN) {
            a.ws[(int64_t)(a.RC + chunk) * a.N + c] = s2;
            a.ws[(int64_t)(2 * a.RC + chunk) * a.N + c] = s3;
        }
    }
}

__global__ __launch_bounds__(CT) void fc_bwd_apply_kernel(const BwdArgs a) {
    const int lane = threadIdx.x & 63, w = threadIdx.x >> 6;
    const int c = blockIdx.x * CW + lane;
    const int chunk = blockIdx.y;
    if (c >= a.N) return;
    const int r0 = chunk * RPC + w * RPW;
    float dys[RPW], zsv[RPW];
#pragma unroll
    for (int i = 0; i < RPW; ++i) {
        const int64_t oc = (int64_t)min(r0 + i, a.B - 1) * a.ld_out + c;
        dys[i] = a.dz_out[oc];
        zsv[i] = a.z[oc];
    }
    float S1 = 0.f, S2 = 0.f, S3 = 0.f;
    for (int ch0 = 0; ch0 < a.RC; ch0 += 8) {
        float t1[8], t2[8], t3[8];
#pragma unroll
        for (int u = 0; u < 8; ++u) {
            const int ch = min(ch0 + u, a.RC - 1);
            t1[u] = a.ws[(int64_t)ch * a.N + c];
            t2[u] = a.ws[(int64_t)(a.RC + ch) * a.N + c];
            t3[u] = a.ws[(int64_t)(2 * a.RC + ch) * a.N + c];
        }
#pragma unroll
        for (int u = 0; u < 8; ++u)
            if (ch0 + u < a.RC) {
                S1 += t1[u];
                S2 += t2[u];
                S3 += t3[u];
            }
    }
    const float mean = a.save_mean[c], invstd = a.save_invstd[c];
    const float gam = a.gamma ? a.gamma[c] : 1.f;
    const float invB = 1.f / (float)a.B;
    const float m1 = S1 * invB, m2 = S2 * invB;
    if (chunk == 0 && w == 0) {
        if (a.dbeta) a.dbeta[c] = S1;
        if (a.dgamma) a.dgamma[c] = S2;
        if (a.dbias) a.dbias[c] = -gam * invstd * m2 * S3;
    }
#pragma unroll
    for (int i = 0; i < RPW; ++i) {
        const int r = r0 + i;
// ... 105 lines not shown
        v[k] = (c < a.N && a.bias) ? a.bias[c] : 0.f;
    }
    for (int s = 0; s < a.n_slabs; ++s) {
        const float* xs = xr + (int64_t)s * a.slab_stride;
#pragma unroll
        for (int k = 0; k < NV; ++k) {
            const int c = lane + 64 * k;
            if (c < a.N) v[k] += xs[c];
        }
    }
    float s1 = 0.f;
#pragma unroll
    for (int k = 0; k < NV; ++k) s1 += v[k];
    const float mean = wave_sum(s1) / (float)a.N;
    float s2 = 0.f;
#pragma unroll
    for (int k = 0; k < NV; ++k) {
        v[k] = (lane + 64 * k < a.N) ? v[k] - mean : 0.f;
        s2 += v[k] * v[k];
    }
    const float invstd = 1.0f / sqrtf(wave_sum(s2) / (float)a.N + a.eps);
#pragma unroll
    for (int k = 0; k < NV; ++k) {
        const int c = lane + 64 * k;
        if (c < a.N) rowtail_store(a, row, c, v[k] * invstd);
    }
    if (lane == 0 && a.save_invstd) a.save_invstd[row] = invstd;
}

__global__ __launch_bounds__(256) void fc_rowtail_fwd_loop_kernel(const RowFwdArgs a) {
    const int lane = threadIdx.x & 63;
    const int row = blockIdx.x * 4 + (threadIdx.x >> 6);
    if (row >= a.B) return;
    const float* xr = a.in + (int64_t)row * a.ld_in;
    float* dr = a.d_out + (int64_t)row * a.ld_out;
    float s1 = 0.f;
    for (int c = lane; c < a.N; c += 64) {
        float v = a.bias ? a.bias[c] : 0.f;
        for (int s = 0; s < a.n_slabs; ++s) v += xr[(int64_t)s * a.slab_stride + c];
        dr[c] = v;
        s1 += v;
    }
    const float mean = wave_sum(s1) / (float)a.N;
    float s2 = 0.f;
    for (int c = lane; c < a.N; c += 64) {
        const float d = dr[c] - mean;
        s2 += d * d;
    }
    const float invstd = 1.0f / sqrtf(wave_sum(s2) / (float)a.N + a.eps);
    for (int c = lane; c < a.N; c += 64) rowtail_store(a, row, c, (dr[c] - mean) * invstd);
    if (lane == 0 && a.save_invstd) a.save_invstd[row] = invstd;
}

struct RowBwdArgs {
    const float* din;
    int64_t ld_in, slab_stride;
    int n_slabs;
    const float* addend;
    const float* row_scale;
    const uint8_t* mask;
    float keep_scale;
    int relu;
    const float* act;
    const float* y;
    const float* save_invstd;
    float* dz_out;
    int64_t ld_out;
    float* ws;
    int B, N;
};

__device__ __forceinline__ float rowtail_dy(const RowBwdArgs& a, int row, int c, float rs) {
    const float* gp = a.din + (int64_t)row * a.ld_in + c;
    float g = 0.f;
    for (int s = 0; s < a.n_slabs; ++s) g += gp[(int64_t)s * a.slab_stride];
    const int64_t o = (int64_t)row * a.ld_out + c;
    g *= rs;
    if (a.mask) g = a.mask[(int64_t)row * a.N + c] ? g * a.keep_scale : 0.f;
    if (a.addend) g += a.addend[o];
    if (a.relu) g = (a.act[o] > 0.f) ? g : 0.f;
    return g;
}

template <int NV>
__global__ __launch_bounds__(256) void fc_rowtail_bwd_kernel(const RowBwdArgs a) {
    __shared__ float red[4][64 * NV];
    const int lane = threadIdx.x & 63, w = threadIdx.x >> 6;
    const int chunk = blockIdx.x;
    float col[NV];
#pragma unroll
    for (int k = 0; k < NV; ++k) col[k] = 0.f;
#pragma unroll 2
    for (int i = 0; i < RPW; ++i) {
        const int row = chunk * RPC + w * RPW + i;
        if (row >= a.B) break;
        const float rs = a.row_scale ? a.row_scale[row] : 1.f;
        float g[NV], yv[NV];
        float s1 = 0.f, s2 = 0.f;
#pragma unroll
        for (int k = 0; k < NV; ++k) {
            const int c = lane + 64 * k;
            const bool cv = c < a.N;
            g[k] = cv ? rowtail_dy(a, row, c, rs) : 0.f;
            yv[k] = cv ? a.y[(int64_t)row * a.ld_out + c] : 0.f;
            s1 += g[k];
            s2 += g[k] * yv[k];
        }
        const float m1 = wave_sum(s1) / (float)a.N, m2 = wave_sum(s2) / (float)a.N;
        const float invstd = a.save_invstd[row];
#pragma unroll
        for (int k = 0; k < NV; ++k) {
            const int c = lane + 64 * k;
            if (c < a.N) {
                const float dz = invstd * (g[k] - m1 - yv[k] * m2);
                a.dz_out[(int64_t)row * a.ld_out + c] = dz;
                col[k] += dz;
            }
        }
    }
    if (!a.ws) return;
#pragma unroll
    for (int k = 0; k < NV; ++k) red[w][lane + 64 * k] = col[k];
    __syncthreads();
    for (int c = threadIdx.x; c < a.N; c += 256)
        a.ws[(int64_t)chunk * a.N + c] = (red[0][c] + red[1][c]) + (red[2][c] + red[3][c]);
}

__global__ __launch_bounds__(256) void fc_rowtail_bwd_loop_kernel(const RowBwdArgs a) {
    const int lane = threadIdx.x & 63;
    const int row = blockIdx.x * 4 + (threadIdx.x >> 6);
    if (row >= a.B) return;
    const float rs = a.row_scale ? a.row_scale[row] : 1.f;
    const float* yr = a.y + (int64_t)row * a.ld_out;
    float* dr = a.dz_out + (int64_t)row * a.ld_out;
    float s1 = 0.f, s2 = 0.f;
    for (int c = lane; c < a.N; c += 64) {
        const float g = rowtail_dy(a, row, c, rs);
        dr[c] = g;
        s1 += g;
        s2 += g * yr[c];
    }
    const float m1 = wave_sum(s1) / (float)a.N, m2 = wave_sum(s2) / (float)a.N;
    const float invstd = a.save_invstd[row];
    for (int c = lane; c < a.N; c += 64) dr[c] = invstd * (dr[c] - m1 - yr[c] * m2);
}

}

extern "C" size_t mmvae_fc_workspace_bytes(int B, int N) {
    if (B <= 0 || N <= 0) return 0;
    return (size_t)3 * (size_t)ceil_div_i(B, RPC) * (size_t)N * sizeof(float);
}

extern "C" int mmvae_fc_epilogue_fwd(int B, int N, const float* in, int64_t ld_in, int n_slabs, const float* bias,
                                     const mmvae_bn_params* bn, int training, int relu, const uint8_t* keep_mask,
                                     float dropout_p, float* z_out, float* a_out, float* d_out, int64_t ld_out,
                                     float* save_mean, float* save_invstd, float* workspace, size_t workspace_bytes,
                                     const mmvae_planes* d_pl, const mmvae_split_job* split, mmvae_stream_t stream) {
    if ((d_pl && d_pl->p && split) || (split && !split->planes.p)) return MMVAE_ERR_ARG;
    static const mmvae_planes no_planes = {nullptr, 0, 0};
    const mmvae_planes dp = d_pl ? *d_pl : no_planes, sp = split ? split->planes : no_planes;
    uint16_t *const d_planes = dp.p, *const sp_planes = sp.p;
    const int64_t ldp = dp.ld, pstride = dp.plane_stride, sp_ld = sp.ld, sp_pstride = sp.plane_stride;
    const int sp_rows = split ? split->rows : 0, sp_cols = split ? split->cols : 0;
    const float* sp_src = split ? split->src : nullptr;
    const int64_t sp_ld_src = split ? split->ld_src : 0;
    if (d_planes && (!d_out || N % 2 != 0 || ldp < N || ldp % 2 != 0 || pstride < (int64_t)B * ldp)) return MMVAE_ERR_ARG;
    if (sp_planes && (sp_rows <= 0 || sp_cols <= 0 || !sp_src || sp_ld_src < sp_cols || sp_ld < (sp_cols + 7) / 8 * 8 ||
                      sp_ld % 8 != 0 || sp_pstride % 8 != 0 || sp_pstride < (int64_t)sp_rows * sp_ld ||
                      (reinterpret_cast<uintptr_t>(sp_planes) & 15u)))
        return MMVAE_ERR_ARG;
    if (B <= 0 || N <= 0 || !in || n_slabs < 1 || ld_in < N || ld_out < N) return MMVAE_ERR_ARG;
    if (!a_out && !d_out) return MMVAE_ERR_ARG;
    if (keep_mask && (dropout_p < 0.f || dropout_p >= 1.f || !d_out)) return MMVAE_ERR_ARG;
    if (bn && training && (!z_out || !save_mean || !save_invstd)) return MMVAE_ERR_ARG;
    if (bn && !training && (!bn->running_mean || !bn->running_var)) return MMVAE_ERR_ARG;
    const bool stats = bn && training;
    if (stats && (!workspace || workspace_bytes < mmvae_fc_workspace_bytes(B, N))) return MMVAE_ERR_WORKSPACE;
    FwdArgs a = {};
    a.in = in;
    a.ld_in = ld_in;
    a.slab_stride = (int64_t)B * ld_in;
    a.n_slabs = n_slabs;
    a.bias = bias;
    if (bn) {
        a.gamma = bn->gamma;
        a.beta = bn->beta;
        a.running_mean = bn->running_mean;
        a.running_var = bn->running_var;
        a.nbt = bn->num_batches_tracked;
        a.momentum = bn->momentum;
        a.eps = bn->eps;
    }
    a.training = training;
    a.relu = relu;
    a.mask = keep_mask;
    a.keep_scale = keep_mask ? 1.0f / (1.0f - dropout_p) : 1.f;
    a.z_out = z_out;
    a.a_out = a_out;
    a.d_out = d_out;
    a.ld_out = ld_out;
    a.save_mean = save_mean;
    a.save_invstd = save_invstd;
    a.ws = workspace;
    a.B = B;
    a.N = N;
    a.RC = ceil_div_i(B, RPC);
    a.d_planes = reinterpret_cast<unsigned short*>(d_planes);
    a.ldp = ldp;
    a.pstride = pstride;
    const dim3 grid(ceil_div_i(N, CW), a.RC);
    dim3 grid_apply = grid;
    if (sp_planes) {
        a.sp_src = sp_src;
        a.sp_planes = reinterpret_cast<unsigned short*>(sp_planes);
        a.sp_ld_src = sp_ld_src;
        a.sp_ld = sp_ld;
        a.sp_pstride = sp_pstride;
        a.sp_rows = sp_rows;
        a.sp_groups = (sp_cols + 7) / 8;
        a.sp_cols = sp_cols;
        grid_apply.y = a.RC + ceil_div_i(768, (int)grid.x);
    }
    hipStream_t s = (hipStream_t)stream;
    if (stats) {
        MMVAE_LAUNCH(fc_fwd_stats_kernel, grid, dim3(CT), 0, s, a);
        MMVAE_LAUNCH_CHECK();
    }
    if (bn)
        MMVAE_LAUNCH(fc_fwd_apply_kernel<true>, grid_apply, dim3(CT), 0, s, a);
    else
        MMVAE_LAUNCH(fc_fwd_apply_kernel<false>, grid_apply, dim3(CT), 0, s, a);
    MMVAE_LAUNCH_CHECK();
    return MMVAE_OK;
}

extern "C" int mmvae_fc_epilogue_bwd(int B, int N, const float* din, int64_t ld_in, int n_slabs, const float* addend,
                                     const float* addend_a, const float* row_scale, const uint8_t* keep_mask,
                                     float dropout_p, int relu, const float* a_act, const float* z, const float* gamma,
                                     const float* save_mean, const float* save_invstd, int has_bn, float* dz_out,
                                     int64_t ld_out, float* dbias, float* dgamma, float* dbeta, float* workspace,
                                     size_t workspace_bytes, const mmvae_planes* dz_pl, mmvae_stream_t stream) {
    uint16_t* const dz_planes = dz_pl ? dz_pl->p : nullptr;
    const int64_t ldp = dz_pl ? dz_pl->ld : 0, pstride = dz_pl ? dz_pl->plane_stride : 0;
    if (dz_planes && (!dz_out || N % 2 != 0 || ldp < N || ldp % 2 != 0 || pstride < (int64_t)B * ldp)) return MMVAE_ERR_ARG;
    if (B <= 0 || N <= 0 || !din || n_slabs < 1 || ld_in < N || ld_out < N) return MMVAE_ERR_ARG;
    if (relu && !a_act) return MMVAE_ERR_ARG;
    if (keep_mask && (dropout_p < 0.f || dropout_p >= 1.f)) return MMVAE_ERR_ARG;
    if (has_bn && (!z || !save_mean || !save_invstd || !dz_out)) return MMVAE_ERR_ARG;
    if (!dz_out && !dbias && !workspace) return MMVAE_ERR_ARG;
    const bool need_ws = has_bn || dbias || workspace;
    if (need_ws && (!workspace || workspace_bytes < mmvae_fc_workspace_bytes(B, N))) return MMVAE_ERR_WORKSPACE;
    BwdArgs a = {};
    a.din = din;
    a.ld_in = ld_in;
    a.slab_stride = (int64_t)B * ld_in;
    a.n_slabs = n_slabs;
    a.addend = addend;
    a.addend_a = addend_a;
    a.row_scale = row_scale;
    a.mask = keep_mask;
    a.keep_scale = keep_mask ? 1.0f / (1.0f - dropout_p) : 1.f;
    a.relu = relu;
    a.a = a_act;
    a.z = z;
    a.gamma = gamma;
    a.save_mean = save_mean;
    a.save_invstd = save_invstd;
    a.dz_out = dz_out;
    a.ld_out = ld_out;
    a.dbias = dbias;
    a.dgamma = dgamma;
    a.dbeta = dbeta;
    a.ws = need_ws ? workspace : nullptr;
    a.B = B;
    a.N = N;
    a.RC = ceil_div_i(B, RPC);
    a.dz_planes = reinterpret_cast<unsigned short*>(dz_planes);
    a.ldp = ldp;
    a.pstride = pstride;
    const dim3 grid(ceil_div_i(N, CW), a.RC);
    hipStream_t s = (hipStream_t)stream;
    if (has_bn) {
        MMVAE_LAUNCH(fc_bwd_stats_kernel<true>, grid, dim3(CT), 0, s, a);
        MMVAE_LAUNCH_CHECK();
        MMVAE_LAUNCH(fc_bwd_apply_kernel, grid, dim3(CT), 0, s, a);
    } else {
        MMVAE_LAUNCH(fc_bwd_stats_kernel<false>, grid, dim3(CT), 0, s, a);
        MMVAE_LAUNCH_CHECK();
        if (dbias)
            MMVAE_LAUNCH(fc_colsum_finish_kernel, dim3(ceil_div_i(N, 256)), dim3(256), 0, s, workspace, a.RC, N,
                               dbias);
    }
    MMVAE_LAUNCH_CHECK();
    return MMVAE_OK;
}

extern "C" int mmvae_layernorm_fwd(int B, int N, const float* x, int64_t ldx, float eps, float* y, int64_t ldy,
                                   float* save_mean, float* save_invstd, mmvae_stream_t stream) {
    if (B <= 0 || N <= 0 || !x || !y || ldx < N || ldy < N) return MMVAE_ERR_ARG;
    MMVAE_LAUNCH(layernorm_fwd_kernel, dim3(ceil_div_i(B, 4)), dim3(256), 0, (hipStream_t)stream, B, N, x, ldx,
                       eps, y, ldy, save_mean, save_invstd);
    MMVAE_LAUNCH_CHECK();
    return MMVAE_OK;
}

extern "C" int mmvae_layernorm_bwd(int B, int N, const float* dy, int64_t lddy, const float* y, int64_t ldy,
                                   const float* save_invstd, float* dx, int64_t lddx, mmvae_stream_t stream) {
    if (B <= 0 || N <= 0 || !dy || !y || !save_invstd || !dx || lddy < N || ldy < N || lddx < N) return MMVAE_ERR_ARG;
    MMVAE_LAUNCH(layernorm_bwd_kernel, dim3(ceil_div_i(B, 4)), dim3(256), 0, (hipStream_t)stream, B, N, dy,
                       lddy, y, ldy, save_invstd, dx, lddx);
    MMVAE_LAUNCH_CHECK();
    return MMVAE_OK;
}

extern "C" int mmvae_fc_rowtail_fwd(int B, int N, const float* in, int64_t ld_in, int n_slabs, const float* bias, float eps,
                                    int training, int relu, const uint8_t* keep_mask, float dropout_p, float* y_out,
                                    float* a_out, float* d_out, int64_t ld_out, float* save_invstd,
                                    mmvae_stream_t stream) {
    if (B <= 0 || N <= 0 || !in || !d_out || n_slabs < 1 || ld_in < N || ld_out < N || !(eps >= 0.f)) return MMVAE_ERR_ARG;
    if (keep_mask && (!training || dropout_p < 0.f || dropout_p >= 1.f)) return MMVAE_ERR_ARG;
    if (training && !save_invstd) return MMVAE_ERR_ARG;
    RowFwdArgs a = {};
    a.in = in;
    a.ld_in = ld_in;
    a.slab_stride = (int64_t)B * ld_in;
    a.n_slabs = n_slabs;
    a.bias = bias;
    a.eps = eps;
    a.relu = relu;
    a.mask = keep_mask;
    a.keep_scale = keep_mask ? 1.0f / (1.0f - dropout_p) : 1.f;
    a.y_out = training ? y_out : nullptr;
    a.a_out = training ? a_out : nullptr;
    a.d_out = d_out;
    a.ld_out = ld_out;
    a.save_invstd = training ? save_invstd : nullptr;
    a.B = B;
    a.N = N;
    const dim3 grid(ceil_div_i(B, 4)), block(256);
    hipStream_t s = (hipStream_t)stream;
    if (N <= 256)
        MMVAE_LAUNCH(fc_rowtail_fwd_kernel<4>, grid, block, 0, s, a);
    else if (N <= 512)
        MMVAE_LAUNCH(fc_rowtail_fwd_kernel<8>, grid, block, 0, s, a);
    else if (N <= 768)
        MMVAE_LAUNCH(fc_rowtail_fwd_kernel<12>, grid, block, 0, s, a);
    else if (N <= 1024)
        MMVAE_LAUNCH(fc_rowtail_fwd_kernel<16>, grid, block, 0, s, a);
    else
        MMVAE_LAUNCH(fc_rowtail_fwd_loop_kernel, grid, block, 0, s, a);
    MMVAE_LAUNCH_CHECK();
    return MMVAE_OK;
}

extern "C" int mmvae_fc_rowtail_bwd(int B, int N, const float* din, int64_t ld_in, int n_slabs, const float* addend,
                                    const float* row_scale, const uint8_t* keep_mask, float dropout_p, int relu,
                                    const float* act, const float* y, const float* save_invstd, float* dz_out,
                                    int64_t ld_out, float* dbias, float* workspace, size_t workspace_bytes,
                                    mmvae_stream_t stream) {
    if (B <= 0 || N <= 0 || !din || !y || !save_invstd || !dz_out || n_slabs < 1 || ld_in < N || ld_out < N)
        return MMVAE_ERR_ARG;
    if (relu && !act) return MMVAE_ERR_ARG;
    if (keep_mask && (dropout_p < 0.f || dropout_p >= 1.f)) return MMVAE_ERR_ARG;
    const int RC = ceil_div_i(B, RPC);
    if (dbias && !workspace) return MMVAE_ERR_WORKSPACE;
    if (workspace && workspace_bytes < (size_t)RC * (size_t)N * sizeof(float)) return MMVAE_ERR_WORKSPACE;
    RowBwdArgs a = {};
    a.din = din;
    a.ld_in = ld_in;
    a.slab_stride = (int64_t)B * ld_in;
    a.n_slabs = n_slabs;
    a.addend = addend;
    a.row_scale = row_scale;
    a.mask = keep_mask;
    a.keep_scale = keep_mask ? 1.0f / (1.0f - dropout_p) : 1.f;
    a.relu = relu;
    a.act = act;
    a.y = y;
    a.save_invstd = save_invstd;
    a.dz_out = dz_out;
    a.ld_out = ld_out;
    a.ws = workspace;
    a.B = B;
    a.N = N;
    const dim3 grid(RC), block(256);
    hipStream_t s = (hipStream_t)stream;
// ... 34 lines not shown
```

mmvae_amd/engine.py:

```python
from __future__ import annotations

import os
from dataclasses import dataclass
from typing import Dict, List, Optional

import torch

from . import _lib, dist as mdist, rng
from .constants import REGISTRY_KEYS as RK
from .engine_adv import PlanAdversaries
from .engine_common import ACC, NN, NT, RELU, SQ_FUSED_SLOTS, TN, _LayerRef, _PlaneBuf, _block_decline, _p
from .engine_cond import CondProgram
from .engine_emit import PlanEmit
from .engine_run import PlanRun
from .modules.base.components import Adversarial, FCBlock, _identity
from .optim import HipAdam

MAX_POINTER_PLANS = 8
SIDE_MAX_ROWS = 640
ADV_DW_CAP = 170


@dataclass(frozen=True)
class EngineSettings:
    conditionals: bool = True
    graphs: bool = True
    planes: bool = True
    side_dw: int = 125
    side_dw2: int = 185
    side_dw_dp: int = 125
    side_dw_any: bool = False
    prefetch_adv: int = 86
    cond_batched: bool = True
    prefetch: int = 128
    adv_fused: bool = True
    adv_aside: int = 2
    dp_overlap: Optional[bool] = None
    dp_shard: bool = True
    dp_kernels: str = "auto"
    dp_sim_world: int = 0
    dp_autotune_force: bool = False
    stamps: bool = False

    @staticmethod
    def from_env() -> "EngineSettings":
        e = os.environ.get
        ov = e("MMVAE_DP_OVERLAP", "")
        kernels = e("MMVAE_DP_KERNELS", "auto")
        if kernels not in ("auto", "dynamic", "persistent"):
            raise _lib.HipLibraryError(f"MMVAE_DP_KERNELS={kernels!r}: dynamic | persistent | auto")
        return EngineSettings(
            conditionals=e("MMVAE_ENGINE_CONDITIONALS", "1") != "0", graphs=e("MMVAE_NO_GRAPH", "0") == "0",
            planes=e("MMVAE_PLANES", "1") != "0", side_dw=int(e("MMVAE_SIDE_DW", "125")),
            side_dw2=int(e("MMVAE_SIDE_DW2", "185")), side_dw_dp=int(e("MMVAE_SIDE_DW_DP", "125")),
            side_dw_any=e("MMVAE_SIDE_DW_ANY", "0") != "0", prefetch=int(e("MMVAE_PREFETCH", "128")),
            cond_batched=e("MMVAE_COND_BATCHED", "1") != "0", prefetch_adv=int(e("MMVAE_PREFETCH_ADV", "86")),
            adv_fused=e("MMVAE_ADV_FUSED", "1") != "0",
            adv_aside=int(e("MMVAE_ADV_ASIDE", "2")),
            dp_overlap=None if ov == "" else ov != "0", dp_shard=e("MMVAE_DP_SHARD", "1") != "0", dp_kernels=kernels,
            dp_sim_world=int(e("MMVAE_DP_SIM_WORLD", "0")), dp_autotune_force=e("MMVAE_DP_AUTOTUNE_FORCE", "0") != "0",
            stamps=e("MMVAE_STAMPS", "0") == "1")


FORK_VALIDATED_RUNTIMES = ("7.0.",)


def concurrent_streams(device, n: int, pool: int = 12) -> list:
    main = torch.cuda.current_stream(device)
    spin = 400_000
    out = []
    for _ in range(pool):
        c = torch.cuda.Stream(device=device)
        torch.cuda.synchronize(device)
        t0, t1, m0, m1 = (torch.cuda.Event(enable_timing=True) for _ in range(4))
        ev = torch.cuda.Event()
        with torch.cuda.stream(c):
            t0.record()
        m0.record(main)
        torch.cuda._sleep(spin)
        ev.record(main)
        torch.cuda._sleep(spin)
        m1.record(main)
        with torch.cuda.stream(c):
            c.wait_event(ev)
            torch.cuda._sleep(2_000)
            t1.record()
        torch.cuda.synchronize(device)
        side_us, both_us = t0.elapsed_time(t1) * 1e3, m0.elapsed_time(m1) * 1e3
        if side_us < 0.8 * both_us:
            out.append(c)
            if len(out) == n:
                break
    return out


def forks_allowed(settings: "EngineSettings", runtime: Optional[str] = None) -> bool:
    v = (torch.version.hip or "") if runtime is None else runtime
    return bool(settings.side_dw_any) or any(v.startswith(p) for p in FORK_VALIDATED_RUNTIMES)


@dataclass(frozen=True)
class _Layout:
    big: bool
    side_dw: int
    early: bool
    late: bool
    late_cap: int
    adv_aside: bool
    adv_dw2: bool
    adv_lane: bool
    dp_dw: int
    prefetch: bool
    prefetch_cap: int
    prefetch_side2: bool


def plan_layout(st: EngineSettings, *, fork_ok: bool, side_stream: bool, side_stream2: bool, lane_stream: bool,
                overlap: bool, world: int, mode: str, B: int, K: int, R: int, G: int, n_in_last: int, iwae: bool,
                has_adv: bool, has_cond: bool, adv_reducer: bool) -> _Layout:
    train = mode == "train"
    dw_flops = 2.0 * G * n_in_last * R
    big = dw_flops >= 5e9
    measured = big and (0.75 * 2.1e10 <= dw_flops <= 1.25 * 2.1e10 or st.side_dw_any)
    in_order = not overlap and world == 1 and K == 1
    side_dw = st.side_dw if fork_ok else 0
    side_dw = side_dw if (train and side_stream and in_order and R <= SIDE_MAX_ROWS and not has_adv and measured) else 0
    late = bool(side_dw or (st.side_dw2 and side_stream and train and has_adv and in_order and R <= SIDE_MAX_ROWS
                            and measured and st.adv_aside))
    adv_fused = has_adv and train and st.adv_fused
    adv_dp = overlap or adv_reducer
    adv_aside = bool(adv_fused and not adv_dp and st.adv_aside and side_stream and in_order and measured and not has_cond)
    adv_forks = bool(adv_fused and st.adv_aside >= 2 and side_stream2 and in_order and measured and not has_cond
                     and not adv_reducer)
    dp_dw = st.side_dw_dp if fork_ok else 0
    dp_dw = dp_dw if (overlap and side_stream and train and K == 1 and not has_adv and measured and not has_cond) else 0
    return _Layout(
        big=big, side_dw=side_dw, early=bool(side_dw and not iwae), late=late, late_cap=st.side_dw2,
        adv_aside=adv_aside, adv_dw2=bool(adv_aside and side_stream2 and st.adv_aside >= 2),
        adv_lane=bool(adv_fused and adv_dp and st.adv_aside and lane_stream and K == 1 and not has_cond), dp_dw=dp_dw,
        prefetch=bool(train and (side_dw or adv_forks)),
        prefetch_cap=st.prefetch_adv if adv_forks else st.prefetch, prefetch_side2=adv_forks)


def _key_pointer(key: tuple) -> int:
    return key[-2]


def _key_target(key: tuple):
    t = key[6] if str(key[0]).startswith("train") else None
    return t if (t is not None and t[1] != 0) else None


class StepEngine:
    @staticmethod
    def decline_reason(model) -> Optional[str]:
        m = model.module
        if m.vae.encoder.z_transformation is not _identity:
            return ('the latent distribution is not "normal" (distribution="ln": a '
                    f"{type(m.vae.encoder.z_transformation).__name__} over the latent sample)")
        blocks = [("the shared VAE's encoder", m.vae.encoder.fc), ("the shared VAE's decoder", m.vae.decoder)]
        for eid, e in m.experts.items():
            blocks += [(f"the encoder of expert {eid!r}", e.encoder), (f"the decoder of expert {eid!r}", e.decoder)]
        for where, b in blocks:
            why = _block_decline(b)
            if why is not None:
                return f"{where}: {why}"
        for eid, e in m.experts.items():
            if hasattr(e.encoder.fc_layers[0], "ln"):
                return (f"the encoder of expert {eid!r}: LayerNorm on its first (gene-wide) layer, whose product is "
                        "pipelined across steps and whose weight gradient reads pre-split planes")
            if hasattr(e.decoder.fc_layers[-1], "ln"):
                return (f"the decoder of expert {eid!r}: LayerNorm on its last (gene-wide) layer, which is fused with the "
                        "reconstruction epilogue")
        for i, adv in enumerate(m.adversarials, start=1):
            why = _block_decline(adv.encoder, layer_norm=False)
            if why is not None:
                return f"the encoder of adversary {i}: {why} (the adversaries' programs have no row tail)"
            for c, h in adv.heads.items():
                if len(h.fc_layers) != 1 or len(list(h.fc_layers[0].children())) != 1:
                    return f"head {c!r} of adversary {i} is not a single Linear"
        cl = getattr(m.vae, "conditionals", None)
        if cl is not None and not EngineSettings.from_env().conditionals:
            return "conditional layers with MMVAE_ENGINE_CONDITIONALS=0"
        opts = model.optimizers()
        if not all(isinstance(o, HipAdam) and o._hip for o in opts):
            return ("an optimiser that is not the HIP Adam (mmvae_amd.optim.HipAdam on device arenas, coupled or "
                    "decoupled weight decay)")
        if cl is not None:
            if not CondProgram.supported(cl, model.get_optimizers()["vae"], m.vae.encoder.mean_encoder.out_features):
                return ("conditional blocks that are not one Linear (+ LayerNorm) of the latent width each, all in the "
                        "shared VAE's optimiser")
        return None

    @staticmethod
    def try_build(model, on_decline=None) -> Optional["StepEngine"]:
        why = StepEngine.decline_reason(model)
        if why is None:
            return StepEngine(model)
        if on_decline is not None:
            on_decline(why)
        return None

    def __init__(self, model, settings: Optional[EngineSettings] = None):
        self.model = model
        self.settings = settings if settings is not None else EngineSettings.from_env()
        self.lib = _lib.load()
        self.device = next(model.parameters()).device
        self.opts = model.get_optimizers()
        self._grad_of: Dict[int, torch.Tensor] = {}
        for opt in model.optimizers():
            for i, p in enumerate(opt.arena.params):
                self._grad_of[id(p)] = opt.arena.grad_view(i)
        self._pool: Dict[tuple, torch.Tensor] = {}
        self._plans: Dict[tuple, "_Plan"] = {}
        self._state_slot: Dict[int, int] = {}
        opts_list = list(model.optimizers())
        if len(opts_list) <= 8:
            metrics = self.buf("metrics", (256,))
            for i, opt in enumerate(opts_list):
                view = metrics[192 + 8 * i:200 + 8 * i]
                if opt.state_dev.data_ptr() != view.data_ptr():
                    view.copy_(opt.state_dev)
                    opt.state_dev = view
                self._state_slot[id(opt)] = 192 + 8 * i
        self._ptr_seen: Dict[tuple, int] = {}
        self.stamps = self.settings.stamps
        self.eager_only = False
        self.klw_dev = torch.ones(1, dtype=torch.float32, device=self.device)
        self._klw_host = None
        st = self.settings
        self.planes = st.planes
        self.side_dw = st.side_dw
        self.fork_ok = forks_allowed(st)
        if not self.fork_ok and (st.side_dw or st.side_dw_dp):
            import warnings

            warnings.warn(f"mmvae_amd.engine: HIP runtime {torch.version.hip} is not one the forked step programs were "
                          f"validated on {FORK_VALIDATED_RUNTIMES}: single-stream programs (MMVAE_SIDE_DW_ANY=1 overrides)")
            self.side_dw = 0
        self.side_dw_dp = st.side_dw_dp if self.fork_ok else 0
        self.side_stream = torch.cuda.Stream(device=self.device) if (self.side_dw or self.side_dw_dp) else None
        self.side_stream2 = torch.cuda.Stream(device=self.device) if (self.side_dw and st.adv_aside >= 2 and st.adv_fused) else None
        self.comm_stream = self.small_stream = self.lane_stream = None
        self._tune = None
        self.dp_tuned: Dict[str, float] = {}
        self._configure_parallel()
        self._sig = self._signature()
        self._sig_changes = 0
        self._cond_lookup: Dict[tuple, dict] = {}
        self._cond_prev_union = None
        self._pending: Dict[str, torch.cuda.Event] = {}
        import weakref

        me = weakref.ref(self)
        for opt in opts_list:
            opt.settle = lambda me=me: me() is not None and me().flush()
        self._prefetched: Optional[dict] = None
        self.prefetch_stats = {"issued": 0, "consumed": 0, "discarded": 0, "staged_ahead": 0}
        self._next_seen: Dict[tuple, int] = {}
        self._staged: Optional[tuple] = None
        self.last_forward_key: Optional[tuple] = None

    def _configure_parallel(self) -> None:
        self.world = mdist.world_size()
        st = self.settings
        self.overlap = mdist.collectives_active() if st.dp_overlap is None else bool(st.dp_overlap)
        self.shard = mdist.collectives_active() and st.dp_shard
        self.shard_sim_world = st.dp_sim_world if self.world == 1 else 0
        self.dp_kernels = st.dp_kernels
        if "MMVAE_X3W" not in os.environ:
            if not mdist.collectives_active():
                self.lib.mmvae_gemm_set_x3w(-1)
            else:
                choice = self.dp_kernels if self.dp_kernels != "auto" else (self.dp_tuned.get("choice") or "dynamic")
                tune = (self.dp_kernels == "auto" and "choice" not in self.dp_tuned
                        and (mdist.world_size() > 1 or st.dp_autotune_force))
                if tune and self._tune is None:
                    self._tune = dict(kind="dynamic", step=0, ev=None)
                elif tune:
                    self._tune.update(step=0, ev=None)
                    choice = self._tune["kind"]
                self.lib.mmvae_gemm_set_x3w(1 if choice == "persistent" else 0)
        if self.overlap and self.comm_stream is None:
            got = concurrent_streams(self.device, 3)
            self.streams_probe = {"wanted": 3, "observed_concurrent": len(got)}
            self.comm_stream, self.small_stream, self.lane_stream = (got + [torch.cuda.Stream(device=self.device)
                                                                            for _ in range(3)])[:3]

    def _signature(self) -> tuple:
        ac = self.model.autograd_config
        clip = lambda c: (float(c.val), c.algorithm or "norm") if (c and c.val) else (0.0, "norm")
        per_opt = tuple((g["eps"], tuple(g["betas"]), o.reducer is not None, o.grad_scale)
                        for o in self.model.optimizers() for g in o.param_groups[:1])
        return (per_opt, clip(ac.vae_gradient_clip), clip(ac.expert_gradient_clip), clip(ac.adversarial_gradient_clip),
# ... 335 lines not shown
        self._check_signature()
        x_arg = x
        x = self._dense_f32(x)
        enc_mod = model.module.vae.encoder
        expert = model.module.experts[expert_id]
        explicit = enc_mod.explicit_eps is not None or expert.encoder.explicit_masks is not None
        K = int(enc_mod.n_samples)
        if enc_mod.explicit_eps is not None and enc_mod.explicit_eps.dim() == 3:
            K = enc_mod.explicit_eps.shape[0]
        B = x.shape[0]
        iwae = getattr(enc_mod, "elbo_mode", "analytic") == "iwae"
        l0 = expert.encoder.fc_layers[0]
        planes = self._enc_planes(l0.lin.in_features, l0.lin.out_features, hasattr(l0, "bn"), B, K, True, iwae)
        ahead = self._take_prefetched(expert_id, x) if x is x_arg else None
        if x is not x_arg:
            self._drop_lookahead()
        staged, self._staged = self._staged, None
        target = self._prefetch_target(expert_id, B, K, iwae, next_batch)
        hinted = target[1] if target else None
        key, x_in, x_t = self._select_input(x, ("train-iwae" if iwae else "train", expert_id, B, K, explicit,
                                                ahead.data_ptr() if ahead is not None else 0),
                                            needs_slack=not planes, target=target, staged=staged)
        if target is not None:
            target = (target[0], x_t)
        plan = self._plans.get(key)
        if plan is None:
            plan = _Plan(self, expert_id, B, K, explicit, x_in, iwae=iwae, slabs_ahead=ahead, prefetch=target)
            self._plans[key] = plan
        if target is not None and plan.prefetch_slabs is None:
            target = None
        self._set_kl_weight()
        if explicit:
            plan.load_explicit_noise(enc_mod, expert)
        if plan.has_adv:
            plan.load_labels(metadata)
        if plan.cond is not None:
            plan.cond.load(metadata)
        ev = self._pending.pop(expert_id, None)
        if ev is not None:
            torch.cuda.current_stream().wait_event(ev)
        self._sync_hyper(expert_id)
        self.last_plan = plan
        ev = plan.run()
        if ev is not None:
            self._pending[expert_id] = ev
        if target is not None:
            x_n = hinted
            w_n = model.module.experts[target[0]].encoder.fc_layers[0].lin.weight
            self._prefetched = dict(eid=target[0], x=x_n, sig=self._batch_sig(x_n), w_version=w_n._version,
                                    slabs=plan.prefetch_slabs)
            self.prefetch_stats["issued"] += 1
        if plan.cond is not None:
            plan.cond.commit()
        model.kl_annealing_fn.step()
        plan.log(model, expert_id)
        if self._tune is not None:
            self._dp_autotune(plan)


class _Plan(PlanEmit, PlanAdversaries, PlanRun):
    def __init__(self, eng: StepEngine, eid: str, B: int, K: int, explicit: bool, x: torch.Tensor, mode: str = "train",
                 iwae: bool = False, slabs_ahead: Optional[torch.Tensor] = None, prefetch=None, targets: tuple = ()):
        self.eng, self.eid, self.B, self.K, self.explicit = eng, eid, B, K, explicit
        self.mode = mode
        self.targets = tuple(targets)
        self.xhat: Dict[str, torch.Tensor] = {}
        self.slabs_ahead, self.prefetch, self.prefetch_slabs = slabs_ahead, prefetch, None
        self.iwae = bool(iwae) and mode == "train"
        self.x, self.ldx = x, x.stride(0) if x.shape[0] > 1 else x.shape[1]
        self.R = B * K
        model = eng.model
        m = model.module
        self.lib = eng.lib
        g = eng.grad_of
        exp = m.experts[eid]

        refs = self._layer_refs
        self.enc_layers = refs(exp.encoder) + refs(m.vae.encoder.fc)
        self.n_expert_enc = len(exp.encoder.fc_layers)
        self.dec_layers = refs(m.vae.decoder) + refs(exp.decoder)
        self.G = exp.decoder.config.layers[-1]
        self.Z = m.vae.encoder.mean_encoder.out_features
        self.var_eps = float(m.vae.encoder.var_eps)
        self.hidden_z = bool(m.vae.encoder.hidden_z)
        self.mean_enc, self.var_enc = m.vae.encoder.mean_encoder, m.vae.encoder.var_encoder
        self.advs = list(m.adversarials)
        self.has_adv = len(self.advs) > 0
        self.adv_weight = float(model.adv_weight)
        self.opt_vae = eng.opts["vae"]
        self.opt_exp = eng.opts["experts"][eid]
        self.opt_adv = list(eng.opts.get("adversarials", {}).values()) if self.has_adv else []
        ac = model.autograd_config
        def clip_rule(c):
            val = float(c.val) if (c and c.val) else 0.0
            if val and (c.algorithm or "norm") == "value":
                return 0.0, val
            if val and (c.algorithm or "norm") != "norm":
                raise _lib.HipLibraryError(f"engine: gradient_clip_algorithm {c.algorithm!r} (config.py:8 allows 'norm' / 'value')")
            return val, 0.0

        (self.clip_vae, cv_vae), (self.clip_exp, cv_exp), (self.clip_adv, cv_adv) = (
            clip_rule(ac.vae_gradient_clip), clip_rule(ac.expert_gradient_clip), clip_rule(ac.adversarial_gradient_clip))
        for opt, cv in [(self.opt_vae, cv_vae), (self.opt_exp, cv_exp)] + [(o, cv_adv) for o in self.opt_adv]:
            opt.set_clip_value(cv or None)
            if not cv:
                opt.state_dev[5] = 0.0
        self.conditions = list(Adversarial.labels.keys()) if self.has_adv else []
        self.metric_slots: Dict[str, int] = {}
        self.segments: List = []
        self._cur: List = []
        self.stamp_names: List[str] = []
        self._dirty: List = []
        self._sq_used: Dict[int, int] = {}
        self._sq_cover: Dict[int, list] = {}
        self._mask_layers: List = []
        self._gemm_jobs: List = []
        self._sum_jobs: List = []
        self._sum_keep: List = []
        self._job_tables: List = []
        self._ws_bytes = 0
        self._slab_floats = 0
        self._graphs: Optional[list] = None
        self._probe_next = None
        self.probe = None
        self.probe_meta: Dict[str, dict] = {}
        self._forked = False
        self._events: List = []
        self._runs = 0
        self.exp_norm_log = None
        self._x_split_jobs: List = []
        self._defer_next_dw = False
        self._deferred_dw = None
        self._fcws_bytes = 0
        self._defer_id = 0
        self.x_fp32_dw1 = False
        self.adv_grad_into: Dict[int, torch.Tensor] = {}
        self.n_adv = 0
        self._label_ring = None
        self._log_cache: Dict[tuple, list] = {}
        self.metrics = eng.buf("metrics", (256,))
        self.rng_state = rng.state(eng.device)
        cl = getattr(m.vae, "conditionals", None)
        self.cond = None
        if cl is not None and mode != "embed":
            if K != 1:
                raise _lib.HipLibraryError("engine: conditional layers with the K-sample extension are not supported")
            self.cond = CondProgram(self, cl, eid, train=(mode == "train"))
        self.layout = plan_layout(
            eng.settings, fork_ok=eng.fork_ok, side_stream=eng.side_stream is not None,
            side_stream2=eng.side_stream2 is not None, lane_stream=eng.lane_stream is not None, overlap=eng.overlap,
            world=eng.world, mode=mode, B=B, K=K, R=self.R, G=self.G, n_in_last=self.dec_layers[-1].n_in, iwae=self.iwae,
            has_adv=self.has_adv, has_cond=self.cond is not None,
            adv_reducer=any(o.reducer is not None for o in self.opt_adv))
        self._build()

    def _layer_refs(self, block: FCBlock) -> list:
        g = self.eng.grad_of
        return [_LayerRef(seq, g, block.config.return_hidden[i], block, i) for i, seq in enumerate(block.fc_layers)]

    def _build(self):
        self.eps = self.eng.buf("eps", (self.K, self.B, self.Z))
        self._mark("step begins (behind the noise fill)")
        self._plan_operand_planes()
        self._emit_encoder_forward()
        self._emit_heads()
        if self.mode == "embed":
            return self._finish_forward_only()
        if self.mode == "generate":
            self._emit_generate()
            return self._finish_forward_only()
        adv = self._emit_adversaries()
        loss_calls = self._emit_decoder_forward()
        if self.mode != "train":
            return self._finish_forward_only()
        self._emit_adversaries_inline(adv)
        self._emit_decoder_backward(adv, loss_calls)
        self._emit_encoder_backward()
        self._emit_optimisers()
        self._finish(self._mask_layers)

    def _plan_operand_planes(self):
        eng, lib = self.eng, self.lib
        B, R, G, train = self.B, self.R, self.G, self.mode == "train"
        x, ldx = self.x, self.ldx
        l0, lastl = self.enc_layers[0], self.dec_layers[-1]
        pl_on = bool(eng.planes and train and not self.iwae and lib.mmvae_gemm_get_precision() == 1)
        self.pl_enc = eng._enc_planes(l0.n_in, l0.n_out, l0.bn is not None, B, self.K, train, self.iwae)
        self.xp = _PlaneBuf(eng, f"xp.{l0.n_in}", B, l0.n_in) if self.pl_enc else None
        self.dYp = _PlaneBuf(eng, f"dYp.{l0.n_out}", B, l0.n_out) if self.pl_enc else None
        self.pl_dec_h = bool(pl_on and lastl.n_in % 8 == 0 and len(self.dec_layers) >= 2
                             and lib.mmvae_gemm_planes_supported(TN, G, lastl.n_in, self.kpad(R), 1, 0, 1))
        self.hp = _PlaneBuf(eng, f"hp.{lastl.n_in}", R, lastl.n_in) if self.pl_dec_h else None
        self.pl_dec_w = bool(pl_on and R >= 2048 and lastl.n_in % 8 == 0
                             and lib.mmvae_gemm_planes_supported(NN, R, lastl.n_in, (G + 31) // 32 * 32, 0, 0, 1))
        self.wp = _PlaneBuf(eng, f"wp.{G}.{lastl.n_in}", G, lastl.n_in) if self.pl_dec_w else None
        self.x_fp32_dw1 = bool(self.pl_enc and not eng._x_planes(l0.n_in, B))
        if self.x_fp32_dw1:
            self.xp = None
        if self.pl_enc and not self.x_fp32_dw1:
            per = (B + 2) // 3
            xpp, xld, xps = self.xp.args()
            self._x_split_jobs = [(min(per, B - r0), l0.n_in, _p(x) + 4 * r0 * ldx, ldx, xpp + 2 * r0 * xld, xld, xps)
                                  for r0 in range(0, B, per)]
        if self.pl_dec_w:
            per = (G + 2) // 3
            wpp, wld, wps = self.wp.args()
            self._x_split_jobs = [(min(per, G - r0), lastl.n_in, _p(lastl.W) + 4 * r0 * lastl.n_in, lastl.n_in,
                                   wpp + 2 * r0 * wld, wld, wps) for r0 in range(0, G, per)] + self._x_split_jobs

    def _emit_prefetch(self):
        L, eng = self.layout, self.eng
        if self.prefetch is None or not L.prefetch:
            return
        eid_n, x_n = self.prefetch
        ln = _LayerRef(eng.model.module.experts[eid_n].encoder.fc_layers[0], eng.grad_of, False)
        Bn = x_n.shape[0]
        sk_n = self._plan_gemm(NT, Bn, ln.n_out, ln.n_in)
        if ln.bn is None or 2.0 * Bn * ln.n_out * ln.n_in < 5e9:
            return
        self.prefetch_slabs = eng.buf(f"prefetch.slabs.{eid_n}", (sk_n, Bn, ln.n_out))
        self._probe_next = "enc_l1_fwd"
        self._gemm_launch(NT, Bn, ln.n_out, ln.n_in, 1.0, x_n, x_n.stride(0), ln.W, ln.n_in, self.prefetch_slabs, ln.n_out,
                          None, _lib.GEMM_RAW_SLABS, sk=sk_n, cap=L.prefetch_cap,
                          stream=eng.side_stream2 if L.prefetch_side2 else eng.side_stream)
        self._probe_next = None

    def _emit_encoder_forward(self):
        B, train = self.B, self.mode == "train"
        cur, ld = self.x, self.ldx
        if self.slabs_ahead is not None:
            self._emit_prefetch()
        for i, l in enumerate(self.enc_layers):
            ahead = self.slabs_ahead if i == 0 else None
            if ahead is not None and tuple(ahead.shape) != (self._plan_gemm(NT, B, l.n_out, l.n_in), B, l.n_out):
                raise _lib.HipLibraryError("engine: slabs computed ahead do not fit this step's first layer")
            self._probe_next = "enc_l1_fwd" if (i == 0 and ahead is None) else None
            cur = self.fwd_layer(f"{self.eid}.enc{i}" if i < self.n_expert_enc else f"vae.enc{i}", l, cur, ld, B,
                                 training=train, mask_stream=i, split_job=self._next_x_split_job(l, B), slabs_from=ahead)
            self._probe_next = None
            ld = l.n_out
            if i == 0:
                self._mark("enc L1 forward done")
                if self.slabs_ahead is None:
                    self._emit_prefetch()

    def _emit_heads(self):
        eng, lib = self.eng, self.lib
        B, K, Z = self.B, self.K, self.Z
        q, HV = self.enc_layers[-1].d, self.enc_layers[-1].n_out
        self.mu = eng.buf("mu", (B, Z))
        self.a_raw = eng.buf("a_raw", (B, Z))
        self.std = eng.buf("std", (B, Z))
        self.z = eng.buf("z", (K, B, Z))
        self.kl_row = eng.buf("kl_row", (B,))
        self.stat = eng.buf("stat", (2, B))
        if not self._gemm_group([
                (NT, B, Z, HV, q, HV, self.mean_enc.weight, HV, self.mu, Z, self.mean_enc.bias, 0, 1.0),
                (NT, B, Z, HV, q, HV, self.var_enc.weight, HV, self.a_raw, Z, self.var_enc.bias, 0, 1.0)]):
            self.gemm(NT, B, Z, HV, q, HV, self.mean_enc.weight, HV, self.mu, Z, bias=self.mean_enc.bias)
            self.gemm(NT, B, Z, HV, q, HV, self.var_enc.weight, HV, self.a_raw, Z, bias=self.var_enc.bias)
        self._emit(lib.mmvae_reparam_kl_fwd, B, Z, K, _p(self.mu), _p(self.a_raw), _p(self.eps), self.var_eps,
                   _p(self.std), _p(self.z), _p(self.kl_row), _p(self.stat))
        self._mark("reparameterised (fork point)")
        if self.iwae:
            self.logratio = eng.buf("iwae.logratio", (K, B))
            self._emit(lib.mmvae_iwae_logratio, B, Z, K, _p(self.std), _p(self.eps), _p(self.z), _p(self.logratio))

    def _emit_adversaries(self):
        L, eng = self.layout, self.eng
        hidden = [l.a if l.a is not None else l.d for l in self.enc_layers if l.return_hidden]
        if self.hidden_z:
            hidden.append(self.z)
        adv_calls, adv_aside, adv_lane = None, False, False
        if L.adv_lane:
            main_segments, main_cur = self.segments, self._cur
            self.segments, self._cur = [], []
            slot_before = dict(self.metric_slots)
            self._mark("adversaries' lane: first launch")
            built = self._build_adversaries_fused(hidden)
            self._mark("adversaries' lane: done")
            lane = [it for it in self.segments + [self._cur] if isinstance(it, tuple) or it]
            self.segments, self._cur = main_segments, main_cur
            if built:
                self._host_marker(("lane", eng.lane_stream, lane))
                adv_lane = True
            else:
                self.metric_slots = slot_before
        if self.has_adv and self.mode == "train" and eng.settings.adv_fused and not self._adv_dp():
            start = len(self._cur)
            if self._build_adversaries_fused(hidden):
                adv_calls = self._take(start)
                adv_calls = [c for c in [self._mark_call("adversaries: first launch")] if c] + adv_calls + \
                            [c for c in [self._mark_call("adversaries: done")] if c]
                adv_aside = L.adv_aside
                if adv_aside:
                    self._fork()
        return hidden, adv_calls, adv_aside, adv_lane

    def _adv_dp(self) -> bool:
        return self.eng.overlap or any(o.reducer is not None for o in self.opt_adv)

    def _emit_decoder_forward(self) -> list:
        eng, lib, L = self.eng, self.lib, self.layout
        B, K, R, Z, G, train = self.B, self.K, self.R, self.Z, self.G, self.mode == "train"
        cur, ld = self.z, Z
        if self.cond is not None:
            cur, ld = self.cond.emit_forward(self.z)
        for i, l in enumerate(self.dec_layers[:-1]):
            to_planes = self.hp is not None and K == 1 and i == len(self.dec_layers) - 2
            cur = self.fwd_layer(f"{self.eid}.dec{i}.K{K}", l, cur, ld, R, training=train,
                                 mask_stream=len(self.enc_layers) + i, planes_out=self.hp if to_planes else None,
                                 split_job=None if to_planes else self._next_x_split_job(l, R))
            ld = l.n_out
        for job in self._x_split_jobs:
            self._emit(lib.mmvae_split_planes_f32, *job)
        self._x_split_jobs = []
        last = self.dec_layers[-1]
        if not (last.relu and last.bn is None and last.ln is None and last.p == 0):
            raise _lib.HipLibraryError("engine: the last decoder layer must be Linear+ReLU (fused recon epilogue)")
        last.inp, last.ld_inp, last.rows = cur, ld, R
        T = lib.mmvae_recon_tiles(G)
        Gp = (G + 31) // 32 * 32
        if not (train and Gp != G and L.big and lib.mmvae_gemm_get_precision() == 1
                and (Gp - G) * last.n_in <= last.b.numel() + 32
                and last.b.data_ptr() == last.W.data_ptr() + 4 * last.W.numel()):
            Gp = G
        self.ldp = Gp
        self.dP = eng.buf(f"dP.{G}", (R, Gp))[:, :G] if train else None
        self.se_part = eng.buf(f"se_part.{G}", (T, R))
        self.w = eng.buf("w", (R,))
        self.dp_colpart = None
        if train and K == 1:
            nrt = lib.mmvae_recon_row_tiles(R)
            self.dp_colpart = eng.buf(f"dP.colpart.{G}", (nrt, G))
            self._defer_sum(self.dp_colpart, nrt, G, 1, G, G, last.gb, G)
        h_in, ld_h, kpad = cur, ld, False
        if last.n_in % 32 != 0 and lib.mmvae_gemm_get_precision() == 1:
            Kp = (last.n_in + 31) // 32 * 32
            hpad = eng.buf(f"hpad.{R}.{last.n_in}", (R, Kp))
            pending, self._sum_jobs, pending_g, self._gemm_jobs = self._sum_jobs, [], self._gemm_jobs, []
            self._defer_sum(cur, 1, 0, R, last.n_in, ld, hpad, Kp)
            self._flush_sums()
            self._sum_jobs, self._gemm_jobs = pending, pending_g
            h_in, ld_h, kpad = hpad, Kp, True
        self._recon_args = _lib.ReconArgs(
            rows=R, x_rows=B, G=G, H=last.n_in, flags=_lib.RECON_H_KPAD if kpad else 0, h=_p(h_in), ldh=ld_h,
            W=_p(last.W), ldw=last.n_in, bias=_p(last.b), x=_p(self.x), ldx=self.ldx, dP=_p(self.dP), lddp=self.ldp,
            se_part=_p(self.se_part), col_part=_p(self.dp_colpart))
        self._emit(lib.mmvae_decoder_recon, self._recon_args, probe=("dec_l2_recon", 2.0 * R * G * last.n_in))
        self.probe_meta["dec_l2_recon"].update(bound="mfma", cus=0, planes="",
                                               shape=f"NT {R}x{G}x{last.n_in} + reconstruction epilogue")
        self._mark("reconstruction done")
        self.recon_row = eng.buf("recon_row", (B,))
        if self.iwae:
            self.rows3 = eng.buf("iwae.rows3", (3, B))
            self._emit(lib.mmvae_elbo_finalize_iwae, B, K, T, _p(self.se_part), _p(self.logratio), _p(self.stat), Z,
                       _p(eng.klw_dev), 1.0, _p(self.metrics), _p(self.w), _p(self.rows3))
            return []
        start = len(self._cur)
        self._emit(lib.mmvae_elbo_finalize, B, K, T, _p(self.se_part), _p(self.kl_row), _p(self.stat), Z,
                   _p(eng.klw_dev), 1.0, _p(self.metrics), _p(self.w), _p(self.recon_row))
        return self._take(start) if (L.early and not self.has_adv) else []

    def _emit_generate(self):
        eng = self.eng
        m = eng.model.module
        R, Z = self.R, self.Z
        cur, ld = self.z, Z
        if self.cond is not None:
            cur, ld = self.cond.emit_forward(self.z)
        self.z_out = cur if self.cond is not None else self.z[0]

        n_shared = len(m.vae.decoder.fc_layers)
        for i, l in enumerate(self.dec_layers[:n_shared]):
            cur = self.fwd_layer(f"gen.vae.dec{i}", l, cur, ld, R, training=False)
            ld = l.n_out
        for t in self.targets:
            t_cur, t_ld = cur, ld
            layers = self.dec_layers[n_shared:] if t == self.eid else self._layer_refs(m.experts[t].decoder)
            for i, l in enumerate(layers[:-1]):
                t_cur = self.fwd_layer(f"gen.{t}.dec{i}", l, t_cur, t_ld, R, training=False)
                t_ld = l.n_out
            last = layers[-1]
            if not (last.relu and last.bn is None and last.ln is None and last.p == 0):
                raise _lib.HipLibraryError("engine: the last decoder layer must be Linear+ReLU (fused recon epilogue)")
            G = last.n_out
            ldx = (G + 3) // 4 * 4
            out = eng.buf(f"xhat.{t}", (R, ldx))
            self.gemm(NT, R, G, last.n_in, t_cur, t_ld, last.W, last.n_in, out, ldx, bias=last.b, flags=RELU)
            self.xhat[t] = out[:, :G]
        self._mark("generated")

    def _emit_adversaries_inline(self, adv):
        hidden, adv_calls, adv_aside, adv_lane = adv
        eng, lib = self.eng, self.lib
        total = lambda beta: self._emit(lib.mmvae_axpby, 1, 1.0, _p(self.metrics), beta, self.mptr("total_loss"))
        self.dz_lat = eng.buf("dz_lat", (self.R, self.Z))
        if not self.has_adv:
            self.metric_slots["total_loss"] = 0
        elif adv_lane:
            pass
        elif adv_calls is None and eng.settings.adv_fused and self._adv_dp() and self._build_adversaries_fused(hidden):
            total(1.0)
        elif adv_calls is None:
            total(0.0)
            self._build_adversaries(hidden)
        elif adv_aside:
            self._branch(eng.side_stream, adv_calls)
        else:
            self._cur.extend(adv_calls)
            total(1.0)

    def _emit_decoder_backward(self, adv, loss_calls):
        eng, lib, L = self.eng, self.lib, self.layout
        B, K, R, Z, G = self.B, self.K, self.R, self.Z, self.G
        _, _, adv_aside, adv_lane = adv
        last = self.dec_layers[-1]
        dw_inp, dw_ld, w_rows = last.inp, last.ld_inp, None
        if K > 1:
            w_rows = self.w
            nch = lib.mmvae_weighted_colsum_chunks(R)
            parts = eng.buf(f"wcolsum.{G}", (nch, G))
            self._emit(lib.mmvae_weighted_colsum_f32, R, G, _p(self.dP), self.ldp, _p(self.w), _p(parts))
            self._defer_sum(parts, nch, G, 1, G, G, last.gb, G)
            dw_inp = eng.buf(f"h_weighted.{last.n_in}", (R, last.n_in))
            dw_ld = last.n_in
            self._emit(lib.mmvae_scale_rows, R, last.n_in, _p(last.inp), last.ld_inp, _p(self.w), _p(dw_inp), dw_ld)
            if self.hp is not None:
                self._emit(lib.mmvae_split_planes_f32, R, last.n_in, _p(dw_inp), dw_ld, *self.hp.args())
        late_dw = adv_aside and L.adv_dw2
        if late_dw:
            S = self._emit_dec_dx()
            self._mark("decoder dX done")
        elif L.side_dw:
            S = self._emit_dec_dx()
            self._emit_dec_dw(last.inp, last.ld_inp, cap=L.side_dw)
            self._mark("decoder dX done")
            if L.early:
                self._fork()
                self._branch(eng.side_stream, loss_calls + [c for c in [self._mark_call("decoder dW + loss words done (branch)")] if c])
        elif L.dp_dw and self._plan_gemm(TN, G, last.n_in, self.kpad(R)) == 1:
            S = self._emit_dec_dx()
            self._emit_dec_dw(last.inp, last.ld_inp, cap=L.dp_dw, exchange=True)
        else:
            self._emit_dec_dw(dw_inp, dw_ld, probe=L.big)
            S = self._emit_dec_dx(probe=L.big, planes=(None, self.wp) if self.pl_dec_w else None)
        rest = self.dec_layers[:-1]
        for j in range(len(rest) - 1, -1, -1):
            l = rest[j]
            rs = w_rows if j == len(rest) - 1 else None
            if j > 0:
                S = self.bwd_layer(l, None, S, need_dx="raw", row_scale=rs)
            else:
                self.bwd_layer(l, None, S, need_dx="full", row_scale=rs,
                               dx_out=self.dz_lat if self.cond is None else self.cond.d_out)
        if self.cond is not None:
            self.cond.emit_backward(self.dz_lat)
            if mdist.collectives_active():
                self._emit(lib.mmvae_grad_zero_flagged_jobs, self.cond.max_jobs, self.cond.jobs_ptr,
                           _p(self.cond.opt.arena.grad))
        if not rest:
            raise _lib.HipLibraryError("engine: decoder needs at least two layers")
        if adv_lane or adv_aside:
            self._mark("chain reaches the adversaries' join")
            if adv_lane:
                self._host_marker(("lane_join", eng.lane_stream))
            else:
                self._join(only=eng.side_stream)
            self._mark("adversaries joined")
            if late_dw:
                self._emit_dec_dw(last.inp, last.ld_inp, cap=ADV_DW_CAP, stream=eng.side_stream2)
                c = self._mark_call("decoder dW done (second branch)")
                if c is not None:
                    self._branch(eng.side_stream2, [c])
            self._emit(lib.mmvae_axpby, 1, 1.0, _p(self.metrics), 1.0, self.mptr("total_loss"))
        zi = self.adv_grad_into.get(id(self.z))
        if zi is not None:
            self._emit(lib.mmvae_axpby, B * Z, 1.0, _p(zi), 1.0, _p(self.dz_lat))

    def _emit_dec_dx(self, probe: bool = True, planes=None) -> int:
        last = self.dec_layers[-1]
        self._probe_next = "dec_l2_dx" if probe else None
        S = self.gemm_raw(NN, self.R, last.n_in, self.ldp, self.dP, self.ldp, last.W, last.n_in, planes=planes)
        self._probe_next = None
        return S

    def _emit_dec_dw(self, inp, ld_inp, cap: int = 0, stream=None, exchange: bool = False, probe: bool = True):
        last = self.dec_layers[-1]
        args = (TN, self.G, last.n_in, self.kpad(self.R))
        ops = (self.dP, self.ldp, inp, ld_inp, last.gW, last.n_in)
        planes = (None, self.hp) if self.pl_dec_h else None
        self._probe_next = "dec_l2_dw" if probe else None
        if exchange:
            self._gemm_launch(*args, 1.0, *ops, None, 0, planes=planes, cap=cap, stream=self.eng.side_stream)
        elif not (cap and self._fuse_sqnorm(*args, 1.0, *ops, None, 0, side_cap=cap, planes=planes, stream=stream)):
            self.gemm(*args, *ops, side=True, planes=planes)
        self._probe_next = None

    def _emit_encoder_backward(self):
        eng, lib = self.eng, self.lib
        B, K, Z = self.B, self.K, self.Z
        q, HV = self.enc_layers[-1].d, self.enc_layers[-1].n_out
        dm = eng.buf("dmu_da", (2, B, Z))
        self.dmu, self.da = dm[0], dm[1]
        dq2 = eng.buf("dq", (2, B, HV))
        self.dq = dq2[0]
        if self.iwae:
            self.dstd_extra = eng.buf("iwae.dstd", (B, Z))
            self._emit(lib.mmvae_iwae_bwd_terms, B, Z, K, _p(eng.klw_dev), 1.0, _p(self.w), _p(self.z), _p(self.std),
                       _p(self.dz_lat), _p(self.dstd_extra))
            self._emit(lib.mmvae_reparam_kl_bwd, B, Z, K, _p(self.mu), _p(self.std), _p(self.eps), _p(self.dz_lat), None,
                       _p(self.dstd_extra), None, _p(eng.klw_dev), 0.0, self.var_eps, _p(self.dmu), _p(self.da))
        else:
            self._emit(lib.mmvae_reparam_kl_bwd, B, Z, K, _p(self.mu), _p(self.std), _p(self.eps), _p(self.dz_lat), None,
                       None, None, _p(eng.klw_dev), 1.0 / B, self.var_eps, _p(self.dmu), _p(self.da))
        if B % 32 == 0:
            self._emit_colsum_pair(B, Z, dm, eng.grad_of(self.mean_enc.bias), eng.grad_of(self.var_enc.bias))
        else:
            for dy, lin in ((self.dmu, self.mean_enc), (self.da, self.var_enc)):
                self._emit_fc_bwd(B, Z, dy, None, None, None, eng.grad_of(lin.bias))
        for dy, lin in ((self.dmu, self.mean_enc), (self.da, self.var_enc)):
            self.gemm(TN, Z, HV, self.kpad(B), dy, Z, q, HV, eng.grad_of(lin.weight), HV, side=True)
        if self._gemm_group([(NN, B, HV, Z, self.dmu, Z, self.mean_enc.weight, HV, dq2[0], HV, None, 0, 1.0),
                             (NN, B, HV, Z, self.da, Z, self.var_enc.weight, HV, dq2[1], HV, None, 0, 1.0)]):
            din, S = dq2, 2
        else:
            self.gemm(NN, B, HV, Z, self.dmu, Z, self.mean_enc.weight, HV, self.dq, HV)
            self.gemm(NN, B, HV, Z, self.da, Z, self.var_enc.weight, HV, self.dq, HV, flags=ACC)
            din, S = self.dq, 1
        early = eng.overlap
        if early and len(self.enc_layers) == self.n_expert_enc:
            self._begin_exchange(self.opt_vae)
        for j in range(len(self.enc_layers) - 1, -1, -1):
            l = self.enc_layers[j]
            hid = l.a if l.a is not None else l.d
            addend = self.adv_grad_into.get(id(hid)) if l.return_hidden else None
            if j == 0 and self.layout.late:
                self._defer_next_dw = True
            S_next = self.bwd_layer(l, din, S, addend=addend, need_dx="raw" if j > 0 else "none",
                                    dz_planes=self.dYp if (j == 0 and self.pl_enc) else None,
                                    inp_planes=self.xp if (j == 0 and self.pl_enc) else None)
            din, S = None, S_next
            if early and j == self.n_expert_enc:
                self._begin_exchange(self.opt_vae)
        self._mark("backward chain done")

    def _emit_optimisers(self):
        eng, lib, L = self.eng, self.lib, self.layout
        self.log_buf = torch.zeros(256, dtype=torch.float32, device=eng.device)

        def emit_log_copy():
            self._emit(lib.mmvae_axpby, 256, 1.0, _p(self.metrics), 0.0, _p(self.log_buf))

        early = eng.overlap
        deferred, self._deferred_dw = self._deferred_dw, None
        late_branch = bool(L.late and deferred is not None and self.cond is None)
        start = len(self._cur)
        self.optimizer(self.opt_vae, self.clip_vae, exchange="wait" if early else "inline", join=not late_branch)
        self.log_norm(self.opt_vae, "grad_norms/vae")
        if late_branch:
            calls = self._take(start)
            self._fork()
            (layout, M, N, Kk, A, lda, Bm, ldb, Cm, ldc), dwp = deferred
            self._probe_next = "enc_l1_dw"
            if not self._fuse_sqnorm(layout, M, N, Kk, 1.0, A, lda, Bm, ldb, Cm, ldc, None, 0, side_cap=L.late_cap,
                                     on_side=False, planes=dwp):
                self.gemm(*deferred[0], side=True, planes=dwp)
            self._probe_next = None
            self._branch(eng.side_stream, calls + [c for c in [self._mark_call("VAE optimiser done (branch)")] if c])
        elif deferred is not None:
            self._probe_next = "enc_l1_dw" if L.big else None
            self.gemm(*deferred[0], side=True, planes=deferred[1])
            self._probe_next = None
        if early:
            emit_log_copy()
        self._mark("encoder dW done / VAE optimiser branch emitted")
        ride = (not early and self.cond is None
                and eng._state_slot.get(id(self.opt_exp)) is not None
                and not (eng.shard and self.opt_exp.reducer is not None))
        self.optimizer(self.opt_exp, self.clip_exp, exchange="deferred" if early else "inline",
                       tail_copy=(256, self.metrics, self.log_buf) if ride else None)
        self._mark("expert optimiser done")
        if early:
            self.exp_norm_log = torch.zeros(1, dtype=torch.float32, device=eng.device)
        else:
            self.log_norm(self.opt_exp, "grad_norms/expert")
            if not ride:
                emit_log_copy()

    def _finish_forward_only(self):
        self.exp_norm_log = None
        self.has_adv = False
        self._finish([])

    def _finish(self, masks):
        eng, lib = self.eng, self.lib
        self.segments.append(self._cur)
        self._cur = []
        if not self.explicit:
            n_max = self.K * self.B * self.Z
            fills = []
            for l, stream in masks:
                n_max = max(n_max, l.mask.numel())
                fills.append(_lib.PhiloxJob(_p(l.mask), l.mask.numel(), rng.STREAM_DROPOUT + stream, l.p, 0))
            fills.append(_lib.PhiloxJob(_p(self.eps), self.K * self.B * self.Z, rng.STREAM_NORMAL, 0.0, 1))
            jobs = self._upload_table((_lib.PhiloxJob * len(fills))(*fills))
            ticket = eng.buf("philox.ticket", (1,), torch.int32)
            self._emit(lib.mmvae_philox_fill_jobs_advance, len(fills), jobs, n_max, _p(self.rng_state), (n_max + 3) // 4,
                       _p(ticket))
            self.segments[0] = self._cur + self.segments[0]
            self._cur = []
        self._size_workspaces()

    def _size_workspaces(self):
        eng = self.eng
        self.fcws = eng.buf("fc_ws", (max(self._fcws_bytes // 4, 1),))
        for key, t in eng._pool.items():
            if key[0] == "fc_ws" and t.numel() > self.fcws.numel():
                self.fcws = t
        self.ws = eng.buf("gemm_ws", (max(self._ws_bytes // 4, 1),))
        self.slab = eng.buf("gemm_slabs", (max(self._slab_floats, 1),))
        for key, t in eng._pool.items():
            if key[0] == "gemm_ws" and t.numel() > self.ws.numel():
                self.ws = t
            if key[0] == "gemm_slabs" and t.numel() > self.slab.numel():
                self.slab = t
```

mmvae_amd/engine_emit.py:

```python
from __future__ import annotations

import ctypes as C
from typing import Optional

import torch

from . import _lib, dist as mdist
from .engine_common import ACC, NN, NT, RAW, RELU, SLACK, SQ_FUSED_SLOTS, TN, _LayerRef, _NOPL, _PlaneBuf, _p, _planes_desc, _s
from .optim import HipAdam


class PlanEmit:
    def _emit(self, fn, *args, probe=None):
        lib_fn = fn

        def call():
            rc = lib_fn(*args, _s())
            if rc != 0:
                raise _lib.HipLibraryError(f"{lib_fn.__name__} failed with code {rc}")

        self._cur.append(self._probed(probe[0], probe[1], call) if probe else call)

    def _mark_call(self, name: str):
        if not self.eng.stamps:
            return None
        slot = len(self.stamp_names)
        self.stamp_names.append(name)
        buf = self.eng.buf("debug.stamps", (256,), torch.int64)
        lib = self.lib

        def call():
            lib.mmvae_debug_stamp(buf.data_ptr(), slot, _s())

        return call

    def _mark(self, name: str):
        c = self._mark_call(name)
        if c is not None:
            self._cur.append(c)

    def _probed(self, tag, work, call, **meta):
        if tag is None:
            return call
        plan = self
        self.probe_meta[tag] = dict(meta, work=work)

        def wrapped():
            pr = plan.probe
            if pr is None:
                return call()
            st = torch.cuda.current_stream()
            e0, e1, e2 = (torch.cuda.Event(enable_timing=True) for _ in range(3))
            e0.record(st)
            call()
            e1.record(st)
            e2.record(st)
            pr.setdefault(tag, []).append((e0, e1, work, e2))

        return wrapped

    def _cut(self, marker):
        self._join()
        self.segments.append(self._cur)
        self.segments.append(marker)
        self._cur = []

    def _host_marker(self, marker):
        self._join()
        if self._cur:
            self.segments.append(self._cur)
            self._cur = []
        self.segments.append(marker)

    def slot(self, name: str) -> int:
        if name not in self.metric_slots:
            self.metric_slots[name] = 8 + sum(1 for v in self.metric_slots.values() if 8 <= v < 192)
            assert self.metric_slots[name] < 192
        return self.metric_slots[name]

    def mptr(self, name: str) -> int:
        return self.metrics.data_ptr() + 4 * self.slot(name)

    @staticmethod
    def kpad(rows: int) -> int:
        return (rows + 31) // 32 * 32

    def _plan_tile(self, layout, M, N, K):
        tile, sk = C.c_int(0), C.c_int(0)
        self.lib.mmvae_gemm_plan(layout, M, N, K, C.byref(tile), C.byref(sk))
        return tile.value, sk.value

    def _plan_gemm(self, layout, M, N, K):
        return self._plan_tile(layout, M, N, K)[1]

    def _fuse_sqnorm(self, layout, M, N, K, alpha, A, lda, Bm, ldb, Cm, ldc, bias, flags, side_cap: int = 0,
                     on_side: bool = True, planes=None, stream=None) -> bool:
        eng = self.eng
        if eng.overlap or eng.world > 1 or ldc != N or (flags & ~ACC):
            return False
        regular = int(_p(A) % 16 == 0 and _p(Bm) % 16 == 0 and lda % 4 == 0 and ldb % 4 == 0)
        self.lib.mmvae_gemm_set_workgroup_cap(side_cap)
        n_part = self.lib.mmvae_gemm_sq_partials(layout, M, N, K, regular)
        self.lib.mmvae_gemm_set_workgroup_cap(0)
        if n_part <= 0:
            return False
        hit = eng.locate_grad(Cm)
        if hit is None:
            return False
        opt, off = hit
        if opt.reducer is not None or (self.cond is not None and opt is self.opt_vae):
            return False
        buf = eng.sq_buffer(opt)
        base = self._sq_used.get(id(opt), 0)
        if base + n_part > SQ_FUSED_SLOTS:
            return False
        self._sq_used[id(opt)] = base + n_part
        self._sq_cover.setdefault(id(opt), []).append((off, M * N))
        side = (stream if stream is not None else eng.side_stream) if on_side else None
        self._gemm_launch(layout, M, N, K, alpha, A, lda, Bm, ldb, Cm, ldc, bias, flags, planes=planes,
                          sq=(buf.data_ptr() + 4 * base, n_part), cap=side_cap, stream=side)
        return True

    def _gemm_launch(self, layout, M, N, K, alpha, A, lda, Bm, ldb, Cm, ldc, bias, flags, sk: int = 1, planes=None,
                     use_ws: bool = False, sq=None, cap: int = 0, stream=None) -> None:
        plan, lib = self, self.lib
        ap, bp = (planes[0].args() if planes and planes[0] else _NOPL), (planes[1].args() if planes and planes[1] else _NOPL)
        tag, self._probe_next = self._probe_next, None
        sq_args = sq if sq else (None, 0)

        def launch_gemm():
            ws = (plan.ws.data_ptr(), plan.ws.numel() * 4) if use_ws else (None, 0)
            c_ptr = _p(Cm) if Cm is not None else plan.slab.data_ptr()
            rc = lib.mmvae_gemm_planes_f32(layout, M, N, K, alpha, _p(A), lda, *ap, _p(Bm), ldb, *bp, c_ptr, ldc,
                                           _p(bias), flags | SLACK, sk, *ws, *sq_args, _s())
            if rc != 0:
                raise _lib.HipLibraryError(f"GEMM launch failed with code {rc} (layout {layout}, {M}x{N}x{K})")

        launch = self._probed(tag, 2.0 * M * N * K, launch_gemm, bound="mfma", cus=cap, planes=_planes_desc(planes),
                              shape=f"{('NT', 'NN', 'TN')[layout]} {M}x{N}x{K}" + (f" split-K {sk}" if sk > 1 else ""))
        if not cap:
            self._cur.append(launch)
            return
        if stream is not None:
            self._fork(stream)

        def call():
            lib.mmvae_gemm_set_workgroup_cap(cap)
            try:
                if stream is not None:
                    with torch.cuda.stream(stream):
                        launch()
                else:
                    launch()
            finally:
                lib.mmvae_gemm_set_workgroup_cap(0)

        self._cur.append(call)

    def _queue_gemm(self, layout, M, N, K, alpha, A, lda, Bm, ldb, Cm, ldc, bias, flags) -> bool:
        if self._plan_tile(layout, M, N, K)[0] != 2:
# ... 5 lines not shown
            n_sl = (K + 511) // 512
            slabs = self.eng.buf(f"dwslabs.{self._next_defer_id()}", (n_sl, M, N))
            ok = True
            sub = []
            for i in range(n_sl):
                k0 = 512 * i
                kk = min(512, K - k0)
                j = _lib.GemmJob(_p(A) + 4 * k0 * lda, _p(Bm) + 4 * k0 * ldb, _p(slabs[i]), None, lda, ldb, N, layout, M, N,
                                 kk, 1.0, 0, 0, 0)
                ok = ok and bool(self.lib.mmvae_gemm_batch_job_ok(C.addressof(j)))
                sub.append(j)
            if ok:
                self._gemm_jobs.extend(sub)
                self._sum_keep.append((A, Bm, Cm, slabs))
                self._defer_sum(slabs, n_sl, M * N, M, N, N, Cm, ldc, alpha, flags & ACC)
                return True
        self._gemm_jobs.append(job)
        self._sum_keep.append((A, Bm, Cm, bias))
        return True

    def _gemm_group(self, jobs) -> bool:
        arr = []
        for layout, M, N, K, A, lda, Bm, ldb, Cm, ldc, bias, flags, alpha in jobs:
            tile = self._plan_tile(layout, M, N, K)[0]
            job = _lib.GemmJob(_p(A), _p(Bm), _p(Cm), _p(bias), lda, ldb, ldc, layout, M, N, K, float(alpha), int(flags), 0, 0)
            if tile != 2 or not self.lib.mmvae_gemm_batch_job_ok(C.addressof(job)):
                return False
            arr.append(job)
            self._sum_keep.append((A, Bm, Cm, bias))
        self._emit_gemm_batch(arr)
        return True

    def _flush_gemms(self):
        if self._gemm_jobs:
            self._emit_gemm_batch(self._gemm_jobs)
            self._gemm_jobs = []

    def _emit_gemm_batch(self, jobs):
        table = (_lib.GemmJob * len(jobs))(*jobs)
        total = C.c_int(0)
        _lib.check(self.lib.mmvae_gemm_batch_prepare(len(jobs), C.addressof(table), C.byref(total)), "mmvae_gemm_batch_prepare")
        self._emit(self.lib.mmvae_gemm_batch_f32, len(jobs), self._upload_table(table), total.value)

    def _upload_table(self, table) -> int:
        t = torch.frombuffer(bytearray(bytes(table)), dtype=torch.uint8).to(self.eng.device)
        self._job_tables.append(t)
        return t.data_ptr()

    def gemm(self, layout, M, N, K, A, lda, Bm, ldb, Cm, ldc, bias=None, flags=0, alpha=1.0, side=False, planes=None):
        if side and self._queue_gemm(layout, M, N, K, alpha, A, lda, Bm, ldb, Cm, ldc, bias, flags):
            return
        sk = self._plan_gemm(layout, M, N, K)
        if side and sk > 1 and not (flags & ~ACC) and bias is None:
            slabs = self.eng.buf(f"dwslabs.{self._next_defer_id()}", (sk, M, N))
            self._gemm_launch(layout, M, N, K, 1.0, A, lda, Bm, ldb, slabs, N, None, RAW, sk=sk, planes=planes)
            self._defer_sum(slabs, sk, M * N, M, N, N, Cm, ldc, alpha, flags & ACC)
            return
        if side and sk == 1 and self._fuse_sqnorm(layout, M, N, K, alpha, A, lda, Bm, ldb, Cm, ldc, bias, flags, planes=planes):
            return
        nbytes = self.lib.mmvae_gemm_workspace_bytes(layout, M, N, K, sk)
        self._ws_bytes = max(self._ws_bytes, nbytes)
        self._gemm_launch(layout, M, N, K, alpha, A, lda, Bm, ldb, Cm, ldc, bias, flags, sk=sk, planes=planes, use_ws=True)

    def _edge(self, src, dst):
        ev = torch.cuda.Event()
        self._events.append(ev)

        def call():
            s = src if src is not None else torch.cuda.current_stream()
            d = dst if dst is not None else torch.cuda.current_stream()
            ev.record(s)
            d.wait_event(ev)

        self._cur.append(call)

    def _next_x_split_job(self, l: _LayerRef, rows: int):
        if not self._x_split_jobs:
            return None
        p_drop = l.p if self.mode == "train" else 0.0
        if l.ln is not None and l.bn is None:
            return None
        if l.bn is None and p_drop == 0 and self._plan_gemm(NT, rows, l.n_out, l.n_in) == 1:
            return None
        job = self._x_split_jobs.pop(0)
        return _lib.SplitJob(*job[:4], _lib.Planes(*job[4:]))

    def _fork(self, stream=None):
        side = stream if stream is not None else self.eng.side_stream
        self._edge(None, side)
        self._forked = True
        if side not in self._dirty:
            self._dirty.append(side)

    def _join(self, only=None):
        for side in self._dirty:
            if only is None or side is only:
                self._edge(side, None)
        self._dirty = [] if only is None else [s for s in self._dirty if s is not only]

    def _take(self, start: int) -> list:
        calls = self._cur[start:]
        del self._cur[start:]
        return calls

    def _branch(self, stream, calls):
        if not calls:
            return

        def call():
            with torch.cuda.stream(stream):
                for c in calls:
                    c()

        self._cur.append(call)
        if stream not in self._dirty:
            self._dirty.append(stream)

    def _next_defer_id(self) -> int:
        self._defer_id += 1
        return self._defer_id

    def _defer_sum(self, src, n_parts, part_stride, rows, cols, ld_src, dst, ld_dst, alpha=1.0, flags=0):
        self._sum_jobs.append(_lib.SumJob(_p(src), _p(dst), part_stride, ld_src, ld_dst, n_parts, rows, cols, float(alpha),
                                          int(flags), 0))
        self._sum_keep.append((src, dst))

    def _flush_sums(self):
        self._flush_gemms()
        if not self._sum_jobs:
            return
        arr = (_lib.SumJob * len(self._sum_jobs))(*self._sum_jobs)
        self._emit(self.lib.mmvae_sum_parts_batch, len(self._sum_jobs), self._upload_table(arr),
                   max(int(j.rows) * int(j.cols) for j in self._sum_jobs))
        self._sum_jobs = []

    def gemm_raw(self, layout, M, N, K, A, lda, Bm, ldb, planes=None) -> int:
        sk = self._plan_gemm(layout, M, N, K)
        self._slab_floats = max(self._slab_floats, sk * M * N)
        self._gemm_launch(layout, M, N, K, 1.0, A, lda, Bm, ldb, None, N, None, RAW, sk=sk, planes=planes)
        return sk

    def fwd_layer(self, tag: str, l: _LayerRef, cur: torch.Tensor, ld_cur: int, rows: int, training: bool = True,
                  mask_tag: Optional[str] = None, mask_stream: Optional[int] = None, planes_out: Optional[_PlaneBuf] = None,
                  split_job=None, slabs_from: Optional[torch.Tensor] = None):
        eng = self.eng
        l.inp, l.ld_inp, l.rows = cur, ld_cur, rows
        l.d = eng.buf(f"{tag}.d", (rows, l.n_out))
        l.z = eng.buf(f"{tag}.z", (rows, l.n_out)) if l.bn is not None else None
        l.mean = eng.buf(f"{tag}.mean", (l.n_out,)) if l.bn is not None else None
        l.invstd = eng.buf(f"{tag}.invstd", (l.n_out,)) if l.bn is not None else None
        l.mask = eng.buf(f"{mask_tag or tag}.mask", (rows, l.n_out), torch.uint8) if (l.p > 0 and training) else None
        if l.mask is not None:
            self._mask_layers.append((l, mask_stream if mask_stream is not None else len(self._mask_layers)))
        l.a = eng.buf(f"{tag}.a", (rows, l.n_out)) if (l.p > 0 and l.return_hidden and training) else None
        l.dz = eng.buf(f"{tag}.dz", (rows, l.n_out)) if training else None
        p_drop = l.p if training else 0.0
        self._fcws_bytes = max(self._fcws_bytes, self.lib.mmvae_fc_workspace_bytes(rows, l.n_out))
        sk = self._plan_gemm(NT, rows, l.n_out, l.n_in)
        l.y = l.ln_invstd = l.bn_out = l.dy = None
        if l.ln is not None:
            return self._fwd_layer_ln(tag, l, cur, ld_cur, rows, training, p_drop, sk, planes_out, split_job, slabs_from)
        if l.bn is None and p_drop == 0 and sk == 1:
            self.gemm(NT, rows, l.n_out, l.n_in, cur, ld_cur, l.W, l.n_in, l.d, l.n_out, bias=l.b,
                      flags=RELU if l.relu else 0)
            if planes_out is not None:
                self._emit(self.lib.mmvae_split_planes_f32, rows, l.n_out, _p(l.d), l.n_out, *planes_out.args())
            return l.d
        if slabs_from is not None:
            assert tuple(slabs_from.shape) == (sk, rows, l.n_out) and slabs_from.is_contiguous()
            S = sk
        else:
            S = self.gemm_raw(NT, rows, l.n_out, l.n_in, cur, ld_cur, l.W, l.n_in)
        self._emit_col_fwd(l, rows, S, slabs_from, training, l.relu, l.mask, p_drop, l.a, l.d, planes_out, split_job)
        return l.d

    def _emit_col_fwd(self, l: _LayerRef, rows: int, S: int, slabs_from, training: bool, relu: bool, mask, p_drop: float,
                      a_out, d_out, planes_out=None, split_job=None):
        bnp = None
        if l.bn is not None:
            bn = l.bn
            bnp = _lib.BnParams(_p(bn.weight), _p(bn.bias), _p(bn.running_mean), _p(bn.running_var),
                                _p(bn.num_batches_tracked), float(bn.momentum), float(bn.eps))
            l._bnp = bnp
        plan = self
        d_planes = _lib.Planes(*planes_out.args()) if planes_out is not None else None

        def call():
            rc = plan.lib.mmvae_fc_epilogue_fwd(
                rows, l.n_out, slabs_from.data_ptr() if slabs_from is not None else plan.slab.data_ptr(), l.n_out, S, _p(l.b),
                bnp, int(training), int(relu), _p(mask), p_drop, _p(l.z), _p(a_out), _p(d_out), l.n_out, _p(l.mean),
                _p(l.invstd), plan.fcws.data_ptr(), plan.fcws.numel() * 4, d_planes, split_job, _s())
            if rc != 0:
                raise _lib.HipLibraryError(f"mmvae_fc_epilogue_fwd failed with code {rc}")

        self._cur.append(call)

    def _fwd_layer_ln(self, tag: str, l: _LayerRef, cur, ld_cur: int, rows: int, training: bool, p_drop: float, sk: int,
                      planes_out, split_job, slabs_from):
        eng = self.eng
        if slabs_from is not None:
            assert tuple(slabs_from.shape) == (sk, rows, l.n_out) and slabs_from.is_contiguous()
            S = sk
        else:
            S = self.gemm_raw(NT, rows, l.n_out, l.n_in, cur, ld_cur, l.W, l.n_in)
        l.y = eng.buf(f"{tag}.y", (rows, l.n_out)) if (training and (l.relu or p_drop > 0)) else None
        l.ln_invstd = eng.buf(f"{tag}.invstd.rows", (rows,)) if training else None
        if l.bn is not None:
            l.bn_out = eng.buf(f"{tag}.bn", (rows, l.n_out))
            l.dy = eng.buf(f"{tag}.dy", (rows, l.n_out)) if training else None
            self._emit_col_fwd(l, rows, S, slabs_from, training, False, None, 0.0, None, l.bn_out, None, split_job)
            S = 1
        plan, src, bias = self, l.bn_out, (l.b if l.bn is None else None)

        def call():
            in_ptr = _p(src) if src is not None else (slabs_from.data_ptr() if slabs_from is not None else plan.slab.data_ptr())
            rc = plan.lib.mmvae_fc_rowtail_fwd(rows, l.n_out, in_ptr, l.n_out, S, _p(bias), l.ln, int(training), int(l.relu),
                                               _p(l.mask), p_drop, _p(l.y), _p(l.a), _p(l.d), l.n_out, _p(l.ln_invstd), _s())
            if rc != 0:
                raise _lib.HipLibraryError(f"mmvae_fc_rowtail_fwd failed with code {rc}")

        self._cur.append(call)
        if planes_out is not None:
            self._emit(self.lib.mmvae_split_planes_f32, rows, l.n_out, _p(l.d), l.n_out, *planes_out.args())
        return l.d

    def bwd_layer(self, l: _LayerRef, din, S_in: int, addend=None, need_dx: str = "raw", dx_out=None, dx_flags=0,
                  dx_alpha=1.0, dz_planes: Optional[_PlaneBuf] = None, inp_planes: Optional[_PlaneBuf] = None,
                  row_scale=None):
        rows = l.rows
        dw_planes = (dz_planes, inp_planes) if (dz_planes is not None and (inp_planes is not None or self.x_fp32_dw1)) else None
        dz_pl = _lib.Planes(*dz_planes.args()) if dw_planes is not None else None
        plan = self
        relu_src = l.a if l.a is not None else l.d
        has_bn = l.bn is not None

        own_ws = None
        if not has_bn and l.gb is not None:
            own_ws = self._bias_partials(rows, l.n_out, l.gb)
        after_ln = l.ln is not None
        if after_ln:
            din, S_in, addend, row_scale = self._bwd_layer_ln(l, din, S_in, addend, row_scale, own_ws)

        def call():
            din_ptr = _p(din) if din is not None else plan.slab.data_ptr()
            ws = own_ws if own_ws is not None else plan.fcws
            mask, relu = (None, False) if after_ln else (l.mask, l.relu)
            rc = plan.lib.mmvae_fc_epilogue_bwd(
                rows, l.n_out, din_ptr, l.n_out, S_in, None, _p(addend), _p(row_scale), _p(mask), l.p, int(relu),
                _p(relu_src) if relu else None, _p(l.z), _p(l.bn.weight) if has_bn else None, _p(l.mean),
                _p(l.invstd), int(has_bn), _p(l.dz), l.n_out, _p(l.gb) if own_ws is None else None,
                _p(l.ggamma) if has_bn else None, _p(l.gbeta) if has_bn else None, ws.data_ptr(), ws.numel() * 4,
                dz_pl, _s())
            if rc != 0:
                raise _lib.HipLibraryError(f"mmvae_fc_epilogue_bwd failed with code {rc}")

        if has_bn or not after_ln:
            self._cur.append(call)
        k_rows = rows if (self.K > 1 and l.inp is self.z and rows != self.R) else self.kpad(rows)
        if self._defer_next_dw:
            self._deferred_dw = ((TN, l.n_out, l.n_in, k_rows, l.dz, l.n_out, l.inp, l.ld_inp, l.gW, l.n_in), dw_planes)
            self._defer_next_dw = False
        else:
            big_first = l is self.enc_layers[0] and 2.0 * l.n_out * l.n_in * k_rows >= 5e9
            self._probe_next = "enc_l1_dw" if big_first else None
            self.gemm(TN, l.n_out, l.n_in, k_rows, l.dz, l.n_out, l.inp, l.ld_inp, l.gW, l.n_in, side=True, planes=dw_planes)
            self._probe_next = None
        if need_dx == "raw":
            return self.gemm_raw(NN, rows, l.n_in, l.n_out, l.dz, l.n_out, l.W, l.n_in)
        if need_dx == "full":
            if not self._gemm_group([(NN, rows, l.n_in, l.n_out, l.dz, l.n_out, l.W, l.n_in, dx_out, l.n_in, None,
                                      dx_flags, dx_alpha)]):
                self.gemm(NN, rows, l.n_in, l.n_out, l.dz, l.n_out, l.W, l.n_in, dx_out, l.n_in, flags=dx_flags,
                          alpha=dx_alpha)
        return 0

    def _bwd_layer_ln(self, l: _LayerRef, din, S_in: int, addend, row_scale, own_ws):
        plan, rows, has_bn = self, l.rows, l.bn is not None
        out = l.dy if has_bn else l.dz
        act = (l.a if l.a is not None else l.d) if l.relu else None
        y = l.y if l.y is not None else l.d

        def call():
            din_ptr = _p(din) if din is not None else plan.slab.data_ptr()
            rc = plan.lib.mmvae_fc_rowtail_bwd(
                rows, l.n_out, din_ptr, l.n_out, S_in, _p(addend), _p(row_scale), _p(l.mask), l.p, int(l.relu), _p(act), _p(y),
                _p(l.ln_invstd), _p(out), l.n_out, None, _p(own_ws), own_ws.numel() * 4 if own_ws is not None else 0, _s())
            if rc != 0:
                raise _lib.HipLibraryError(f"mmvae_fc_rowtail_bwd failed with code {rc}")

        self._cur.append(call)
        return (l.dy, 1, None, None) if has_bn else (None, 0, None, None)

    def _bias_partials(self, rows, N, dbias):
        RC = (rows + 31) // 32
        nfl = max(self.lib.mmvae_fc_workspace_bytes(rows, N) // 4, RC * N)
        ws = self.eng.buf(f"biasparts.{self._next_defer_id()}", (nfl,))
        self._defer_sum(ws, RC, N, 1, N, N, dbias, N)
        return ws

    def _emit_colsum_pair(self, B, N, pair, dbias0, dbias1):
        plan = self
        rows = 2 * B
        RC = rows // 32
        self._fcws_bytes = max(self._fcws_bytes, self.lib.mmvae_fc_workspace_bytes(rows, N))
        ws = self.eng.buf(f"biasparts.{self._next_defer_id()}",
                          (max(self.lib.mmvae_fc_workspace_bytes(rows, N) // 4, RC * N),))
        self._defer_sum(ws, RC // 2, N, 1, N, N, dbias0, N)
        self._defer_sum(ws[(RC // 2) * N:], RC // 2, N, 1, N, N, dbias1, N)

        def call():
            rc = plan.lib.mmvae_fc_epilogue_bwd(rows, N, _p(pair), N, 1, None, None, None, None, 0.0, 0, None, None,
                                                None, None, None, 0, None, N, None, None, None, ws.data_ptr(),
                                                ws.numel() * 4, None, _s())
            if rc != 0:
                raise _lib.HipLibraryError(f"mmvae_fc_epilogue_bwd (stacked column sums) failed with code {rc}")

        self._cur.append(call)

    def _emit_fc_bwd(self, rows, N, din, addend, row_scale, dz_out, dbias):
        plan = self
        self._fcws_bytes = max(self._fcws_bytes, self.lib.mmvae_fc_workspace_bytes(rows, N))
        own_ws = self._bias_partials(rows, N, dbias) if dbias is not None else None

        def call():
            ws = own_ws if own_ws is not None else plan.fcws
            rc = plan.lib.mmvae_fc_epilogue_bwd(rows, N, _p(din), N, 1, _p(addend), None, _p(row_scale), None, 0.0, 0, None, None,
                                                None, None, None, 0, _p(dz_out), N, _p(dbias) if own_ws is None else None,
                                                None, None, ws.data_ptr(), ws.numel() * 4, None, _s())
            if rc != 0:
                raise _lib.HipLibraryError(f"mmvae_fc_epilogue_bwd (column sum) failed with code {rc}")

        self._cur.append(call)

    def optimizer(self, opt: HipAdam, max_norm: float, advance: bool = True, step: bool = True, exchange: str = "inline",
                  join: bool = True, tail_copy=None):
        if join:
            self._join()
        self._flush_sums()
# ... 102 lines not shown
```

Baseline: 577,800 cells/s.

## Fuse Philox dropout-mask and latent-noise generation into consumer kernels

Adds draw variants of the FC forward epilogue and reparameterisation kernels that generate dropout keep-masks and Gaussian eps in place from the Philox state, instead of running separate fill kernels beforehand. The RNG offset is advanced inside the reparam backward kernel, so the standalone noise-fill launches and the extra read of mask and eps buffers are dropped. This is enabled by default for single-GPU, non-adversarial, non-overlap training. The cost is recomputing a full Philox block per element, since each element uses only one of the four words, plus some risk of differing RNG stream semantics.

```diff
diff --git a/include/mmvae_hip.h b/include/mmvae_hip.h
--- a/include/mmvae_hip.h
+++ b/include/mmvae_hip.h
@@ -90,6 +90,14 @@
                           float* workspace, size_t workspace_bytes, const mmvae_planes* d_planes ,
                           const mmvae_split_job* split , mmvae_stream_t stream);
 
+int mmvae_fc_epilogue_fwd_draw(int B, int N, const float* in, int64_t ld_in, int n_slabs, const float* bias,
+                               const mmvae_bn_params* bn , int training, int relu,
+                               uint8_t* keep_mask_out , const uint64_t* rng_state, uint64_t stream_id,
+                               float dropout_p, float* z_out, float* a_out, float* d_out, int64_t ld_out,
+                               float* save_mean, float* save_invstd, float* workspace, size_t workspace_bytes,
+                               const mmvae_planes* d_planes , const mmvae_split_job* split ,
+                               mmvae_stream_t stream);
+
 int mmvae_fc_epilogue_bwd(int B, int N, const float* din, int64_t ld_in, int n_slabs, const float* addend,
                           const float* addend_a, const float* row_scale, const uint8_t* keep_mask, float dropout_p, int relu,
                           const float* a, const float* z, const float* gamma, const float* save_mean,
@@ -114,11 +122,18 @@
 
 int mmvae_reparam_kl_fwd(int B, int Z, int K, const float* mu, const float* a_raw, const float* eps, float var_eps,
                          float* std_out, float* z_out, float* kl_row, float* stat_row, mmvae_stream_t stream);
+int mmvae_reparam_kl_fwd_draw(int B, int Z, int K, const float* mu, const float* a_raw, float* eps_out,
+                              const uint64_t* rng_state, uint64_t stream_id, float var_eps, float* std_out, float* z_out,
+                              float* kl_row, float* stat_row, mmvae_stream_t stream);
 
 int mmvae_reparam_kl_bwd(int B, int Z, int K, const float* mu, const float* std, const float* eps, const float* dz,
                          const float* dmu_extra, const float* dstd_extra, const float* dkl_row,
                          const float* kl_scale_dev, float kl_scale_host, float var_eps, float* dmu, float* da_raw,
                          mmvae_stream_t stream);
+int mmvae_reparam_kl_bwd_advance(int B, int Z, int K, const float* mu, const float* std, const float* eps, const float* dz,
+                                 const float* dmu_extra, const float* dstd_extra, const float* dkl_row,
+                                 const float* kl_scale_dev, float kl_scale_host, float var_eps, float* dmu, float* da_raw,
+                                 uint64_t* rng_state, uint64_t advance_by, mmvae_stream_t stream);
 
 int mmvae_mse_sum_fwd_bwd(int B, int G, const float* xhat, int64_t ldxhat, const float* x, int64_t ldx, float* se_row,
                           float* dxhat, int64_t lddx, const float* gscale_dev, float gscale_host,
diff --git a/mmvae_amd/_lib.py b/mmvae_amd/_lib.py
--- a/mmvae_amd/_lib.py
+++ b/mmvae_amd/_lib.py
@@ -84,6 +84,11 @@
         [_i, _i, _p, _l, _i, _p, C.POINTER(BnParams), _i, _i, _p, _f, _p, _p, _p, _l, _p, _p, _p, _z,
          C.POINTER(Planes), C.POINTER(SplitJob), _p],
     ),
+    "mmvae_fc_epilogue_fwd_draw": (
+        _i,
+        [_i, _i, _p, _l, _i, _p, C.POINTER(BnParams), _i, _i, _p, _p, _u64, _f, _p, _p, _p, _l, _p, _p, _p, _z,
+         C.POINTER(Planes), C.POINTER(SplitJob), _p],
+    ),
     "mmvae_fc_epilogue_bwd": (
         _i,
         [_i, _i, _p, _l, _i, _p, _p, _p, _p, _f, _i, _p, _p, _p, _p, _p, _i, _p, _l, _p, _p, _p, _p, _z,
@@ -94,7 +99,9 @@
     "mmvae_fc_rowtail_fwd": (_i, [_i, _i, _p, _l, _i, _p, _f, _i, _i, _p, _f, _p, _p, _p, _l, _p, _p]),
     "mmvae_fc_rowtail_bwd": (_i, [_i, _i, _p, _l, _i, _p, _p, _p, _f, _i, _p, _p, _p, _p, _l, _p, _p, _z, _p]),
     "mmvae_reparam_kl_fwd": (_i, [_i, _i, _i, _p, _p, _p, _f, _p, _p, _p, _p, _p]),
+    "mmvae_reparam_kl_fwd_draw": (_i, [_i, _i, _i, _p, _p, _p, _p, _u64, _f, _p, _p, _p, _p, _p]),
     "mmvae_reparam_kl_bwd": (_i, [_i, _i, _i, _p, _p, _p, _p, _p, _p, _p, _p, _f, _f, _p, _p, _p]),
+    "mmvae_reparam_kl_bwd_advance": (_i, [_i, _i, _i, _p, _p, _p, _p, _p, _p, _p, _p, _f, _f, _p, _p, _p, _u64, _p]),
     "mmvae_mse_sum_fwd_bwd": (_i, [_i, _i, _p, _l, _p, _l, _p, _p, _l, _p, _f, _p]),
     "mmvae_elbo_finalize": (_i, [_i, _i, _i, _p, _p, _p, _i, _p, _f, _p, _p, _p, _p]),
     "mmvae_iwae_logratio": (_i, [_i, _i, _i, _p, _p, _p, _p, _p]),
diff --git a/mmvae_amd/csrc/elbo_optim.hip b/mmvae_amd/csrc/elbo_optim.hip
--- a/mmvae_amd/csrc/elbo_optim.hip
+++ b/mmvae_amd/csrc/elbo_optim.hip
@@ -1,15 +1,24 @@
 #include "common.h"
+#include "philox.h"
 
 namespace {
 
+template <bool DRAW>
 __global__ __launch_bounds__(256) void reparam_kl_fwd_kernel(int B, int Z, int K, const float* __restrict__ mu,
                                                              const float* __restrict__ a_raw,
                                                              const float* __restrict__ eps, float var_eps,
                                                              float* __restrict__ std_out, float* __restrict__ z_out,
-                                                             float* __restrict__ kl_row, float* __restrict__ stat_row) {
+                                                             float* __restrict__ kl_row, float* __restrict__ stat_row,
+                                                             const uint64_t* __restrict__ rng, uint64_t stream_id,
+                                                             float* __restrict__ eps_out) {
     const int lane = threadIdx.x & 63;
     const int b = blockIdx.x * 4 + (threadIdx.x >> 6);
     if (b >= B) return;
+    uint64_t seed = 0, off = 0;
+    if (DRAW) {
+        seed = rng[0];
+        off = rng[1];
+    }
     float kl = 0.f, smu = 0.f, svar = 0.f;
     for (int j = lane; j < Z; j += 64) {
         const int64_t o = (int64_t)b * Z + j;
@@ -24,7 +33,14 @@
         if (z_out)
             for (int k = 0; k < K; ++k) {
                 const int64_t ok = ((int64_t)k * B + b) * Z + j;
-                z_out[ok] = m + s * eps[ok];
+                float e;
+                if (DRAW) {
+                    e = philox_normal_elem(seed, off, stream_id, ok);
+                    eps_out[ok] = e;
+                } else {
+                    e = eps[ok];
+                }
+                z_out[ok] = m + s * e;
             }
     }
     kl = wave_sum(kl);
@@ -47,7 +63,9 @@
                                                              const float* __restrict__ dkl_row,
                                                              const float* __restrict__ kl_scale_dev, float kl_scale_host,
                                                              float var_eps, float* __restrict__ dmu,
-                                                             float* __restrict__ da_raw) {
+                                                             float* __restrict__ da_raw, uint64_t* rng_advance,
+                                                             uint64_t advance_by) {
+    if (rng_advance && blockIdx.x == 0 && threadIdx.x == 0) rng_advance[1] += advance_by;
     const int64_t n = (int64_t)B * Z;
     const float cs = (kl_scale_dev ? *kl_scale_dev : 1.f) * kl_scale_host;
     for (int64_t o = (int64_t)blockIdx.x * blockDim.x + threadIdx.x; o < n; o += (int64_t)gridDim.x * blockDim.x) {
@@ -780,32 +798,6 @@
     if (acc == -1.f && sink) sink[0] = acc;
 }
 
-struct u32x4 {
-    uint32_t x, y, z, w;
-};
-__device__ __forceinline__ u32x4 philox4x32_10(uint64_t counter, uint64_t stream_id, uint64_t seed) {
-    uint32_t c0 = (uint32_t)counter, c1 = (uint32_t)(counter >> 32), c2 = (uint32_t)stream_id,
-             c3 = (uint32_t)(stream_id >> 32);
-    uint32_t k0 = (uint32_t)seed, k1 = (uint32_t)(seed >> 32);
-#pragma unroll
-    for (int i = 0; i < 10; ++i) {
-        const uint64_t p0 = (uint64_t)0xD2511F53u * c0;
-        const uint64_t p1 = (uint64_t)0xCD9E8D57u * c2;
-        const uint32_t n0 = (uint32_t)(p1 >> 32) ^ c1 ^ k0;
-        const uint32_t n1 = (uint32_t)p1;
-        const uint32_t n2 = (uint32_t)(p0 >> 32) ^ c3 ^ k1;
-        const uint32_t n3 = (uint32_t)p0;
-        c0 = n0;
-        c1 = n1;
-        c2 = n2;
-        c3 = n3;
-        k0 += 0x9E3779B9u;
-        k1 += 0xBB67AE85u;
-    }
-    return {c0, c1, c2, c3};
-}
-__device__ __forceinline__ float u01(uint32_t x) { return ((float)(x >> 8) + 0.5f) * (1.0f / 16777216.0f); }
-
 __global__ __launch_bounds__(256) void philox_mask_kernel(int64_t n, float p_drop, uint8_t* __restrict__ mask,
                                                           const uint64_t* __restrict__ rng, uint64_t stream_id) {
     const uint64_t seed = rng[0], off = rng[1];
@@ -816,7 +808,7 @@
 #pragma unroll
         for (int j = 0; j < 4; ++j) {
             const int64_t i = q * 4 + j;
-            if (i < n) mask[i] = (u01(rv[j]) >= p_drop) ? 1 : 0;
+            if (i < n) mask[i] = philox_keep(rv[j], p_drop);
         }
     }
 }
@@ -827,12 +819,9 @@
     const int64_t nq = (n + 3) / 4;
     for (int64_t q = (int64_t)blockIdx.x * blockDim.x + threadIdx.x; q < nq; q += (int64_t)gridDim.x * blockDim.x) {
         const u32x4 r = philox4x32_10(off + (uint64_t)q, stream_id, seed);
-        const float u0 = u01(r.x), u1 = u01(r.y), u2 = u01(r.z), u3 = u01(r.w);
-        const float r0 = sqrtf(-2.f * logf(u0)), r1 = sqrtf(-2.f * logf(u2));
-        float s0, c0, s1, c1;
-        sincosf(6.283185307179586f * u1, &s0, &c0);
-        sincosf(6.283185307179586f * u3, &s1, &c1);
-        const float nv[4] = {r0 * c0, r0 * s0, r1 * c1, r1 * s1};
+        float nv[4];
+        philox_normal_pair(r.x, r.y, nv[0], nv[1]);
+        philox_normal_pair(r.z, r.w, nv[2], nv[3]);
 #pragma unroll
         for (int j = 0; j < 4; ++j) {
             const int64_t i = q * 4 + j;
@@ -856,16 +845,13 @@
 #pragma unroll
             for (int j = 0; j < 4; ++j) {
                 const int64_t i = q * 4 + j;
-                if (i < n) mask[i] = (u01(rv[j]) >= job.p_drop) ? 1 : 0;
+                if (i < n) mask[i] = philox_keep(rv[j], job.p_drop);
             }
         } else {
             float* out = static_cast<float*>(job.out);
-            const float u0 = u01(r.x), u1 = u01(r.y), u2 = u01(r.z), u3 = u01(r.w);
-            const float r0 = sqrtf(-2.f * logf(u0)), r1 = sqrtf(-2.f * logf(u2));
-            float s0, c0, s1, c1;
-            sincosf(6.283185307179586f * u1, &s0, &c0);
-            sincosf(6.283185307179586f * u3, &s1, &c1);
-            const float nv[4] = {r0 * c0, r0 * s0, r1 * c1, r1 * s1};
+            float nv[4];
+            philox_normal_pair(r.x, r.y, nv[0], nv[1]);
+            philox_normal_pair(r.z, r.w, nv[2], nv[3]);
 #pragma unroll
             for (int j = 0; j < 4; ++j) {
                 const int64_t i = q * 4 + j;
@@ -968,8 +954,20 @@
                                     mmvae_stream_t stream) {
     if (B <= 0 || Z <= 0 || K < 1 || !mu || !a_raw) return MMVAE_ERR_ARG;
     if (z_out && !eps) return MMVAE_ERR_ARG;
-    MMVAE_LAUNCH(reparam_kl_fwd_kernel, dim3(ceil_div_i(B, 4)), dim3(256), 0, (hipStream_t)stream, B, Z, K, mu,
-                       a_raw, eps, var_eps, std_out, z_out, kl_row, stat_row);
+    MMVAE_LAUNCH(reparam_kl_fwd_kernel<false>, dim3(ceil_div_i(B, 4)), dim3(256), 0, (hipStream_t)stream, B, Z, K, mu,
+                       a_raw, eps, var_eps, std_out, z_out, kl_row, stat_row,
+                       (const uint64_t*)nullptr, (uint64_t)0, (float*)nullptr);
+    MMVAE_LAUNCH_CHECK();
+    return MMVAE_OK;
+}
+
+extern "C" int mmvae_reparam_kl_fwd_draw(int B, int Z, int K, const float* mu, const float* a_raw, float* eps_out,
+                                         const uint64_t* rng_state, uint64_t stream_id, float var_eps, float* std_out,
+                                         float* z_out, float* kl_row, float* stat_row, mmvae_stream_t stream) {
+    if (B <= 0 || Z <= 0 || K < 1 || !mu || !a_raw || !eps_out || !rng_state || !z_out) return MMVAE_ERR_ARG;
+    MMVAE_LAUNCH(reparam_kl_fwd_kernel<true>, dim3(ceil_div_i(B, 4)), dim3(256), 0, (hipStream_t)stream, B, Z, K, mu,
+                       a_raw, (const float*)nullptr, var_eps, std_out, z_out, kl_row, stat_row, rng_state, stream_id,
+                       eps_out);
     MMVAE_LAUNCH_CHECK();
     return MMVAE_OK;
 }
@@ -983,7 +981,22 @@
     const int64_t n = (int64_t)B * Z;
     MMVAE_LAUNCH(reparam_kl_bwd_kernel, dim3(grid_for(n, 256, 2048)), dim3(256), 0, (hipStream_t)stream, B, Z, K,
                        mu, sd, eps, dz, dmu_extra, dstd_extra, dkl_row, kl_scale_dev, kl_scale_host, var_eps, dmu,
-                       da_raw);
+                       da_raw, (uint64_t*)nullptr, (uint64_t)0);
+    MMVAE_LAUNCH_CHECK();
+    return MMVAE_OK;
+}
+
+extern "C" int mmvae_reparam_kl_bwd_advance(int B, int Z, int K, const float* mu, const float* sd, const float* eps,
+                                            const float* dz, const float* dmu_extra, const float* dstd_extra,
+                                            const float* dkl_row, const float* kl_scale_dev, float kl_scale_host,
+                                            float var_eps, float* dmu, float* da_raw, uint64_t* rng_state,
+                                            uint64_t advance_by, mmvae_stream_t stream) {
+    if (B <= 0 || Z <= 0 || K < 1 || !mu || !sd || !dmu || !da_raw || !rng_state || advance_by == 0) return MMVAE_ERR_ARG;
+    if (dz && !eps) return MMVAE_ERR_ARG;
+    const int64_t n = (int64_t)B * Z;
+    MMVAE_LAUNCH(reparam_kl_bwd_kernel, dim3(grid_for(n, 256, 2048)), dim3(256), 0, (hipStream_t)stream, B, Z, K,
+                       mu, sd, eps, dz, dmu_extra, dstd_extra, dkl_row, kl_scale_dev, kl_scale_host, var_eps, dmu,
+                       da_raw, rng_state, advance_by);
     MMVAE_LAUNCH_CHECK();
     return MMVAE_OK;
 }
diff --git a/mmvae_amd/csrc/fc_epilogue.hip b/mmvae_amd/csrc/fc_epilogue.hip
--- a/mmvae_amd/csrc/fc_epilogue.hip
+++ b/mmvae_amd/csrc/fc_epilogue.hip
@@ -1,4 +1,5 @@
 #include "common.h"
+#include "philox.h"
 
 namespace {
 
@@ -35,6 +36,10 @@
     unsigned short* sp_planes;
     int64_t sp_ld_src, sp_ld, sp_pstride;
     int sp_rows, sp_groups, sp_cols;
+    const uint64_t* draw_rng;
+    uint64_t draw_stream;
+    float p_drop;
+    uint8_t* mask_w;
 };
 
 __device__ __forceinline__ void split_rows_job(const FwdArgs& a, int wg, int nwg) {
@@ -141,7 +146,7 @@
     }
 }
 
-template <bool HAS_BN>
+template <bool HAS_BN, bool DRAW>
 __global__ __launch_bounds__(CT) void fc_fwd_apply_kernel(const FwdArgs a) {
     if ((int)blockIdx.y >= a.RC) {
         split_rows_job(a, ((int)blockIdx.y - a.RC) * gridDim.x + blockIdx.x, ((int)gridDim.y - a.RC) * gridDim.x);
@@ -162,7 +167,13 @@
         for (int i = 0; i < RPW; ++i) {
             const int rc = min(r0 + i, a.B - 1);
             if (stats) zs[i] = a.z_out[(int64_t)rc * a.ld_out + c];
-            mk[i] = a.mask ? a.mask[(int64_t)rc * a.N + c] : (unsigned char)1;
+            if (!DRAW) mk[i] = a.mask ? a.mask[(int64_t)rc * a.N + c] : (unsigned char)1;
+        }
+        if (DRAW) {
+            const uint64_t seed = a.draw_rng[0], off = a.draw_rng[1];
+#pragma unroll
+            for (int i = 0; i < RPW; ++i)
+                mk[i] = philox_keep_elem(seed, off, a.draw_stream, (int64_t)min(r0 + i, a.B - 1) * a.N + c, a.p_drop);
         }
     }
     if (HAS_BN) {
@@ -227,6 +238,7 @@
         if (a.d_out) {
             float d = y;
             if (a.mask) d = mk[i] ? y * a.keep_scale : 0.f;
+            if (DRAW) a.mask_w[(int64_t)r * a.N + c] = mk[i];
             a.d_out[o] = d;
             if (a.d_planes) store_planes_lanepair(a.d_planes, a.ldp, a.pstride, r, c, d, lane);
         }
@@ -638,11 +650,12 @@
     return (size_t)3 * (size_t)ceil_div_i(B, RPC) * (size_t)N * sizeof(float);
 }
 
-extern "C" int mmvae_fc_epilogue_fwd(int B, int N, const float* in, int64_t ld_in, int n_slabs, const float* bias,
-                                     const mmvae_bn_params* bn, int training, int relu, const uint8_t* keep_mask,
-                                     float dropout_p, float* z_out, float* a_out, float* d_out, int64_t ld_out,
-                                     float* save_mean, float* save_invstd, float* workspace, size_t workspace_bytes,
-                                     const mmvae_planes* d_pl, const mmvae_split_job* split, mmvae_stream_t stream) {
+static int fc_epilogue_fwd_launch(int B, int N, const float* in, int64_t ld_in, int n_slabs, const float* bias,
+                                  const mmvae_bn_params* bn, int training, int relu, const uint8_t* keep_mask,
+                                  float dropout_p, float* z_out, float* a_out, float* d_out, int64_t ld_out,
+                                  float* save_mean, float* save_invstd, float* workspace, size_t workspace_bytes,
+                                  const mmvae_planes* d_pl, const mmvae_split_job* split, const uint64_t* draw_rng,
+                                  uint64_t draw_stream, uint8_t* mask_w, mmvae_stream_t stream) {
     if ((d_pl && d_pl->p && split) || (split && !split->planes.p)) return MMVAE_ERR_ARG;
     static const mmvae_planes no_planes = {nullptr, 0, 0};
     const mmvae_planes dp = d_pl ? *d_pl : no_planes, sp = split ? split->planes : no_planes;
@@ -682,6 +695,10 @@
     a.relu = relu;
     a.mask = keep_mask;
     a.keep_scale = keep_mask ? 1.0f / (1.0f - dropout_p) : 1.f;
+    a.draw_rng = draw_rng;
+    a.draw_stream = draw_stream;
+    a.p_drop = dropout_p;
+    a.mask_w = mask_w;
     a.z_out = z_out;
     a.a_out = a_out;
     a.d_out = d_out;
@@ -713,12 +730,40 @@
         MMVAE_LAUNCH(fc_fwd_stats_kernel, grid, dim3(CT), 0, s, a);
         MMVAE_LAUNCH_CHECK();
     }
-    if (bn)
-        MMVAE_LAUNCH(fc_fwd_apply_kernel<true>, grid_apply, dim3(CT), 0, s, a);
-    else
-        MMVAE_LAUNCH(fc_fwd_apply_kernel<false>, grid_apply, dim3(CT), 0, s, a);
+    if (draw_rng) {
+        if (bn)
+            MMVAE_LAUNCH((fc_fwd_apply_kernel<true, true>), grid_apply, dim3(CT), 0, s, a);
+        else
+            MMVAE_LAUNCH((fc_fwd_apply_kernel<false, true>), grid_apply, dim3(CT), 0, s, a);
+    } else if (bn) {
+        MMVAE_LAUNCH((fc_fwd_apply_kernel<true, false>), grid_apply, dim3(CT), 0, s, a);
+    } else {
+        MMVAE_LAUNCH((fc_fwd_apply_kernel<false, false>), grid_apply, dim3(CT), 0, s, a);
+    }
     MMVAE_LAUNCH_CHECK();
     return MMVAE_OK;
+}
+
+extern "C" int mmvae_fc_epilogue_fwd(int B, int N, const float* in, int64_t ld_in, int n_slabs, const float* bias,
+                                     const mmvae_bn_params* bn, int training, int relu, const uint8_t* keep_mask,
+                                     float dropout_p, float* z_out, float* a_out, float* d_out, int64_t ld_out,
+                                     float* save_mean, float* save_invstd, float* workspace, size_t workspace_bytes,
+                                     const mmvae_planes* d_pl, const mmvae_split_job* split, mmvae_stream_t stream) {
+    return fc_epilogue_fwd_launch(B, N, in, ld_in, n_slabs, bias, bn, training, relu, keep_mask, dropout_p, z_out, a_out,
+                                  d_out, ld_out, save_mean, save_invstd, workspace, workspace_bytes, d_pl, split, nullptr, 0,
+                                  nullptr, stream);
+}
+
+extern "C" int mmvae_fc_epilogue_fwd_draw(int B, int N, const float* in, int64_t ld_in, int n_slabs, const float* bias,
+                                          const mmvae_bn_params* bn, int training, int relu, uint8_t* keep_mask_out,
+                                          const uint64_t* rng_state, uint64_t stream_id, float dropout_p, float* z_out,
+                                          float* a_out, float* d_out, int64_t ld_out, float* save_mean,
+                                          float* save_invstd, float* workspace, size_t workspace_bytes,
+                                          const mmvae_planes* d_pl, const mmvae_split_job* split, mmvae_stream_t stream) {
+    if (!keep_mask_out || !rng_state) return MMVAE_ERR_ARG;
+    return fc_epilogue_fwd_launch(B, N, in, ld_in, n_slabs, bias, bn, training, relu, keep_mask_out, dropout_p, z_out, a_out,
+                                  d_out, ld_out, save_mean, save_invstd, workspace, workspace_bytes, d_pl, split, rng_state,
+                                  stream_id, keep_mask_out, stream);
 }
 
 extern "C" int mmvae_fc_epilogue_bwd(int B, int N, const float* din, int64_t ld_in, int n_slabs, const float* addend,
diff --git a/mmvae_amd/csrc/philox.h b/mmvae_amd/csrc/philox.h
--- /dev/null
+++ b/mmvae_amd/csrc/philox.h
@@ -0,0 +1,56 @@
+#pragma once
+#include "common.h"
+
+namespace {
+
+struct u32x4 {
+    uint32_t x, y, z, w;
+};
+__device__ __forceinline__ u32x4 philox4x32_10(uint64_t counter, uint64_t stream_id, uint64_t seed) {
+    uint32_t c0 = (uint32_t)counter, c1 = (uint32_t)(counter >> 32), c2 = (uint32_t)stream_id,
+             c3 = (uint32_t)(stream_id >> 32);
+    uint32_t k0 = (uint32_t)seed, k1 = (uint32_t)(seed >> 32);
+#pragma unroll
+    for (int i = 0; i < 10; ++i) {
+        const uint64_t p0 = (uint64_t)0xD2511F53u * c0;
+        const uint64_t p1 = (uint64_t)0xCD9E8D57u * c2;
+        const uint32_t n0 = (uint32_t)(p1 >> 32) ^ c1 ^ k0;
+        const uint32_t n1 = (uint32_t)p1;
+        const uint32_t n2 = (uint32_t)(p0 >> 32) ^ c3 ^ k1;
+        const uint32_t n3 = (uint32_t)p0;
+        c0 = n0;
+        c1 = n1;
+        c2 = n2;
+        c3 = n3;
+        k0 += 0x9E3779B9u;
+        k1 += 0xBB67AE85u;
+    }
+    return {c0, c1, c2, c3};
+}
+__device__ __forceinline__ float u01(uint32_t x) { return ((float)(x >> 8) + 0.5f) * (1.0f / 16777216.0f); }
+
+__device__ __forceinline__ uint8_t philox_keep(uint32_t word, float p_drop) { return (u01(word) >= p_drop) ? 1 : 0; }
+
+__device__ __forceinline__ void philox_normal_pair(uint32_t wa, uint32_t wb, float& n0, float& n1) {
+    const float ua = u01(wa), ub = u01(wb);
+    const float r = sqrtf(-2.f * logf(ua));
+    float s, c;
+    sincosf(6.283185307179586f * ub, &s, &c);
+    n0 = r * c;
+    n1 = r * s;
+}
+
+__device__ __forceinline__ uint8_t philox_keep_elem(uint64_t seed, uint64_t off, uint64_t stream_id, int64_t i,
+                                                    float p_drop) {
+    const u32x4 r = philox4x32_10(off + (uint64_t)(i >> 2), stream_id, seed);
+    const int j = (int)(i & 3);
+    return philox_keep(j == 0 ? r.x : j == 1 ? r.y : j == 2 ? r.z : r.w, p_drop);
+}
+__device__ __forceinline__ float philox_normal_elem(uint64_t seed, uint64_t off, uint64_t stream_id, int64_t i) {
+    const u32x4 r = philox4x32_10(off + (uint64_t)(i >> 2), stream_id, seed);
+    float n0, n1;
+    philox_normal_pair((i & 2) ? r.z : r.x, (i & 2) ? r.w : r.y, n0, n1);
+    return (i & 1) ? n1 : n0;
+}
+
+}
diff --git a/mmvae_amd/engine.py b/mmvae_amd/engine.py
--- a/mmvae_amd/engine.py
+++ b/mmvae_amd/engine.py
@@ -40,6 +40,7 @@
     dp_kernels: str = "auto"
     dp_sim_world: int = 0
     dp_autotune_force: bool = False
+    fused_noise: bool = True
     stamps: bool = False
 
     @staticmethod
@@ -59,7 +60,7 @@
             adv_aside=int(e("MMVAE_ADV_ASIDE", "2")),
             dp_overlap=None if ov == "" else ov != "0", dp_shard=e("MMVAE_DP_SHARD", "1") != "0", dp_kernels=kernels,
             dp_sim_world=int(e("MMVAE_DP_SIM_WORLD", "0")), dp_autotune_force=e("MMVAE_DP_AUTOTUNE_FORCE", "0") != "0",
-            stamps=e("MMVAE_STAMPS", "0") == "1")
+            fused_noise=e("MMVAE_FUSED_NOISE", "1") != "0", stamps=e("MMVAE_STAMPS", "0") == "1")
 
 
 FORK_VALIDATED_RUNTIMES = ("7.0.",)
@@ -113,6 +114,7 @@
     prefetch: bool
     prefetch_cap: int
     prefetch_side2: bool
+    fused_noise: bool = False
 
 
 def plan_layout(st: EngineSettings, *, fork_ok: bool, side_stream: bool, side_stream2: bool, lane_stream: bool,
@@ -139,7 +141,8 @@
         adv_aside=adv_aside, adv_dw2=bool(adv_aside and side_stream2 and st.adv_aside >= 2),
         adv_lane=bool(adv_fused and adv_dp and st.adv_aside and lane_stream and K == 1 and not has_cond), dp_dw=dp_dw,
         prefetch=bool(train and (side_dw or adv_forks)),
-        prefetch_cap=st.prefetch_adv if adv_forks else st.prefetch, prefetch_side2=adv_forks)
+        prefetch_cap=st.prefetch_adv if adv_forks else st.prefetch, prefetch_side2=adv_forks,
+        fused_noise=bool(st.fused_noise and train and not overlap and world == 1 and not has_adv and not has_cond))
 
 
 def _key_pointer(key: tuple) -> int:
@@ -781,6 +784,8 @@
             world=eng.world, mode=mode, B=B, K=K, R=self.R, G=self.G, n_in_last=self.dec_layers[-1].n_in, iwae=self.iwae,
             has_adv=self.has_adv, has_cond=self.cond is not None,
             adv_reducer=any(o.reducer is not None for o in self.opt_adv))
+        self.fused_noise = bool(self.layout.fused_noise and not self.explicit and not self.has_adv and not any(
+            l.ln is not None and l.p > 0 for l in self.enc_layers + self.dec_layers[:-1]))
         self._build()
 
     def _layer_refs(self, block: FCBlock) -> list:
@@ -888,8 +893,13 @@
                 (NT, B, Z, HV, q, HV, self.var_enc.weight, HV, self.a_raw, Z, self.var_enc.bias, 0, 1.0)]):
             self.gemm(NT, B, Z, HV, q, HV, self.mean_enc.weight, HV, self.mu, Z, bias=self.mean_enc.bias)
             self.gemm(NT, B, Z, HV, q, HV, self.var_enc.weight, HV, self.a_raw, Z, bias=self.var_enc.bias)
-        self._emit(lib.mmvae_reparam_kl_fwd, B, Z, K, _p(self.mu), _p(self.a_raw), _p(self.eps), self.var_eps,
-                   _p(self.std), _p(self.z), _p(self.kl_row), _p(self.stat))
+        if self.fused_noise:
+            self._emit(lib.mmvae_reparam_kl_fwd_draw, B, Z, K, _p(self.mu), _p(self.a_raw), _p(self.eps),
+                       _p(self.rng_state), rng.STREAM_NORMAL, self.var_eps, _p(self.std), _p(self.z), _p(self.kl_row),
+                       _p(self.stat))
+        else:
+            self._emit(lib.mmvae_reparam_kl_fwd, B, Z, K, _p(self.mu), _p(self.a_raw), _p(self.eps), self.var_eps,
+                       _p(self.std), _p(self.z), _p(self.kl_row), _p(self.stat))
         self._mark("reparameterised (fork point)")
         if self.iwae:
             self.logratio = eng.buf("iwae.logratio", (K, B))
@@ -1134,15 +1144,19 @@
         self.dmu, self.da = dm[0], dm[1]
         dq2 = eng.buf("dq", (2, B, HV))
         self.dq = dq2[0]
+        bwd, adv = lib.mmvae_reparam_kl_bwd, ()
+        if self.fused_noise:
+            n_max = max([K * B * Z] + [l.mask.numel() for l, _ in self._mask_layers])
+            bwd, adv = lib.mmvae_reparam_kl_bwd_advance, (_p(self.rng_state), (n_max + 3) // 4)
         if self.iwae:
             self.dstd_extra = eng.buf("iwae.dstd", (B, Z))
             self._emit(lib.mmvae_iwae_bwd_terms, B, Z, K, _p(eng.klw_dev), 1.0, _p(self.w), _p(self.z), _p(self.std),
                        _p(self.dz_lat), _p(self.dstd_extra))
-            self._emit(lib.mmvae_reparam_kl_bwd, B, Z, K, _p(self.mu), _p(self.std), _p(self.eps), _p(self.dz_lat), None,
-                       _p(self.dstd_extra), None, _p(eng.klw_dev), 0.0, self.var_eps, _p(self.dmu), _p(self.da))
+            self._emit(bwd, B, Z, K, _p(self.mu), _p(self.std), _p(self.eps), _p(self.dz_lat), None,
+                       _p(self.dstd_extra), None, _p(eng.klw_dev), 0.0, self.var_eps, _p(self.dmu), _p(self.da), *adv)
         else:
-            self._emit(lib.mmvae_reparam_kl_bwd, B, Z, K, _p(self.mu), _p(self.std), _p(self.eps), _p(self.dz_lat), None,
-                       None, None, _p(eng.klw_dev), 1.0 / B, self.var_eps, _p(self.dmu), _p(self.da))
+            self._emit(bwd, B, Z, K, _p(self.mu), _p(self.std), _p(self.eps), _p(self.dz_lat), None,
+                       None, None, _p(eng.klw_dev), 1.0 / B, self.var_eps, _p(self.dmu), _p(self.da), *adv)
         if B % 32 == 0:
             self._emit_colsum_pair(B, Z, dm, eng.grad_of(self.mean_enc.bias), eng.grad_of(self.var_enc.bias))
         else:
@@ -1226,7 +1240,7 @@
         eng, lib = self.eng, self.lib
         self.segments.append(self._cur)
         self._cur = []
-        if not self.explicit:
+        if not self.explicit and not self.fused_noise:
             n_max = self.K * self.B * self.Z
             fills = []
             for l, stream in masks:
diff --git a/mmvae_amd/engine_emit.py b/mmvae_amd/engine_emit.py
--- a/mmvae_amd/engine_emit.py
+++ b/mmvae_amd/engine_emit.py
@@ -5,7 +5,7 @@
 
 import torch
 
-from . import _lib, dist as mdist
+from . import _lib, dist as mdist, rng
 from .engine_common import ACC, NN, NT, RAW, RELU, SLACK, SQ_FUSED_SLOTS, TN, _LayerRef, _NOPL, _PlaneBuf, _p, _planes_desc, _s
 from .optim import HipAdam
 
@@ -317,6 +317,7 @@
         l.mask = eng.buf(f"{mask_tag or tag}.mask", (rows, l.n_out), torch.uint8) if (l.p > 0 and training) else None
         if l.mask is not None:
             self._mask_layers.append((l, mask_stream if mask_stream is not None else len(self._mask_layers)))
+            l.mask_stream = self._mask_layers[-1][1]
         l.a = eng.buf(f"{tag}.a", (rows, l.n_out)) if (l.p > 0 and l.return_hidden and training) else None
         l.dz = eng.buf(f"{tag}.dz", (rows, l.n_out)) if training else None
         p_drop = l.p if training else 0.0
@@ -349,6 +350,20 @@
             l._bnp = bnp
         plan = self
         d_planes = _lib.Planes(*planes_out.args()) if planes_out is not None else None
+        if mask is not None and self.fused_noise:
+            rng_ptr, sid = _p(self.rng_state), rng.STREAM_DROPOUT + l.mask_stream
+
+            def call_draw():
+                rc = plan.lib.mmvae_fc_epilogue_fwd_draw(
+                    rows, l.n_out, slabs_from.data_ptr() if slabs_from is not None else plan.slab.data_ptr(), l.n_out, S,
+                    _p(l.b), bnp, int(training), int(relu), _p(mask), rng_ptr, sid, p_drop, _p(l.z), _p(a_out), _p(d_out),
+                    l.n_out, _p(l.mean), _p(l.invstd), plan.fcws.data_ptr(), plan.fcws.numel() * 4, d_planes, split_job,
+                    _s())
+                if rc != 0:
+                    raise _lib.HipLibraryError(f"mmvae_fc_epilogue_fwd_draw failed with code {rc}")
+
+            self._cur.append(call_draw)
+            return
 
         def call():
             rc = plan.lib.mmvae_fc_epilogue_fwd(
```

After: 580,400 cells/s (median of 4 runs). Within noise of the previous version (+0.4%).
